# ruolin/strawberry

Hardware: NVIDIA B200
Metric: fragments*EM-iters/sec (higher is better)
Workload: dtype f64

## Files before the change

### include/sbq.h

```cpp
#ifndef SBQ_H_
#define SBQ_H_
#include <stddef.h>
#include <stdint.h>

#ifdef __cplusplus
extern "C" {
#endif

#define SBQ_ABI_VERSION 2

typedef enum {
   SBQ_SUCCESS = 0,
   SBQ_ERR_INVALID = -1,
   SBQ_ERR_NO_DEVICE = -2,
   SBQ_ERR_CUDA = -3,
   SBQ_ERR_NOMEM = -4,
   SBQ_ERR_STATE = -5,
   SBQ_ERR_UNSUPPORTED = -6
} sbq_error;

typedef enum { SBQ_LOCUS_OK = 0, SBQ_LOCUS_ITER_CAP = 1, SBQ_LOCUS_ZERO_DENOM = 2, SBQ_LOCUS_NO_ROWS = 3 } sbq_locus_status;

#define SBQ_MAX_ISO 3600

typedef struct {
   int32_t device;
   int32_t max_iter;
   double  theta_tol;
   double  row_eps;
   double  min_iso_frac;
   int32_t effective_len_norm;
   double  insert_mean;
   int32_t bias_mode;
   int32_t max_out_it;
   int32_t max_theta_it;
   int32_t max_bias_it;
   double  bias_tol;
   int32_t n_gpus;
} sbq_config;

typedef struct {
   int32_t n_iso;
   int32_t n_row;
   const int64_t* row_ptr;
   const int32_t* col;
   const double*  alpha;
   const int32_t* count;
   const int32_t* iso_len;
} sbq_locus;

typedef struct sbq_ctx sbq_ctx;

typedef struct {
   int64_t n_loci, n_row, n_iso, nnz;
   int64_t loci_warp, loci_cta, loci_grid;
   int64_t kernel_launches;
   int64_t h2d_bytes, d2h_bytes;
   double  upload_ms, solve_ms, download_ms;
   double  em_ms;
   double  grid_em_ms;
   int64_t em_iters_total;
   int64_t frag_iters;
   int64_t alg_bytes;
   int64_t grid_alg_bytes;
   double  weights_ms;
} sbq_stats;

int  sbq_abi_version(void);
const char* sbq_error_string(int err);
const char* sbq_last_error(const sbq_ctx*);

void sbq_config_default(sbq_config* cfg);

int  sbq_create(const sbq_config* cfg, sbq_ctx** out);
void sbq_destroy(sbq_ctx*);

int  sbq_submit(sbq_ctx*, const sbq_locus* loci, int64_t n_loci);

int  sbq_submit_flat(sbq_ctx*, int64_t n_loci, const int64_t* loc_row_off, const int64_t* loc_iso_off,
                     const int64_t* row_ptr, const int32_t* col, const double* alpha,
                     const int32_t* count, const int32_t* iso_len);

int  sbq_clear(sbq_ctx*);

int  sbq_validate(sbq_ctx*);

void* sbq_host_alloc(size_t bytes);
void  sbq_host_free(void* p);

int  sbq_upload(sbq_ctx*);
int  sbq_upload_begin(sbq_ctx*);
int  sbq_solve(sbq_ctx*, int64_t total_mapped_reads);
int  sbq_download(sbq_ctx*);

int  sbq_run(sbq_ctx*, int64_t total_mapped_reads);

int  sbq_fpkm_sum(sbq_ctx*, double* local_sum);
int  sbq_fpkm_sum_to_device(sbq_ctx*, void* dev_double);
int  sbq_finalize_tpm(sbq_ctx*, double global_fpkm_sum);

int  sbq_results(sbq_ctx*, double* theta, double* fpkm, double* frac, double* tpm, int32_t* keep,
                 int32_t* iters, int32_t* status);

int  sbq_get_stats(const sbq_ctx*, sbq_stats* out);
// ... 44 lines not shown
```

### strawberry_b200/api.py

```python
import ctypes
import os
import weakref

os.environ.setdefault("CUDA_DEVICE_MAX_CONNECTIONS", "32")

import numpy as np

_HERE = os.path.dirname(os.path.abspath(__file__))
LIB_PATH = os.environ.get("SBQ_LIB_PATH", os.path.join(_HERE, "libsbq.so"))

SBQ_SUCCESS, SBQ_ERR_INVALID, SBQ_ERR_NO_DEVICE, SBQ_ERR_CUDA, SBQ_ERR_NOMEM, SBQ_ERR_STATE, SBQ_ERR_UNSUPPORTED = 0, -1, -2, -3, -4, -5, -6
LOCUS_OK, LOCUS_ITER_CAP, LOCUS_ZERO_DENOM, LOCUS_NO_ROWS = 0, 1, 2, 3

ABI_SYMBOLS = [
    "sbq_abi_version", "sbq_error_string", "sbq_last_error", "sbq_config_default", "sbq_create", "sbq_destroy",
    "sbq_submit", "sbq_submit_flat", "sbq_clear", "sbq_validate", "sbq_host_alloc", "sbq_host_free",
    "sbq_upload", "sbq_upload_begin", "sbq_solve", "sbq_download", "sbq_run", "sbq_fpkm_sum", "sbq_fpkm_sum_to_device",
    "sbq_finalize_tpm", "sbq_results", "sbq_get_stats", "sbq_get_launch_stats", "sbq_em_solve", "sbq_set_plan",
    "sbq_set_covariates", "sbq_bias_results", "sbq_partition_lpt", "sbq_locus_devices", "sbq_synth_giant", "sbq_fetch_batch",
]


class SbqError(RuntimeError):
    def __init__(self, code, msg):
        super().__init__(f"sbq error {code}: {msg}")
        self.code = code


class Config(ctypes.Structure):
    _fields_ = [("device", ctypes.c_int32), ("max_iter", ctypes.c_int32), ("theta_tol", ctypes.c_double),
                ("row_eps", ctypes.c_double), ("min_iso_frac", ctypes.c_double),
                ("effective_len_norm", ctypes.c_int32), ("insert_mean", ctypes.c_double),
                ("bias_mode", ctypes.c_int32), ("max_out_it", ctypes.c_int32), ("max_theta_it", ctypes.c_int32),
                ("max_bias_it", ctypes.c_int32), ("bias_tol", ctypes.c_double), ("n_gpus", ctypes.c_int32)]


class Locus(ctypes.Structure):
    _fields_ = [("n_iso", ctypes.c_int32), ("n_row", ctypes.c_int32), ("row_ptr", ctypes.c_void_p),
                ("col", ctypes.c_void_p), ("alpha", ctypes.c_void_p), ("count", ctypes.c_void_p),
                ("iso_len", ctypes.c_void_p)]


class SynthGiantSpec(ctypes.Structure):
    _fields_ = [("seed", ctypes.c_uint64), ("n_loci", ctypes.c_int32), ("locus_ids", ctypes.c_void_p), ("rows_per_locus", ctypes.c_int64),
                ("iso_lo", ctypes.c_int32), ("iso_hi", ctypes.c_int32), ("mean_extra", ctypes.c_double)]


class Stats(ctypes.Structure):
    _fields_ = [(n, ctypes.c_int64) for n in ("n_loci", "n_row", "n_iso", "nnz", "loci_warp", "loci_cta", "loci_grid",
                                              "kernel_launches", "h2d_bytes", "d2h_bytes")] + \
               [(n, ctypes.c_double) for n in ("upload_ms", "solve_ms", "download_ms", "em_ms", "grid_em_ms")] + \
               [(n, ctypes.c_int64) for n in ("em_iters_total", "frag_iters", "alg_bytes", "grid_alg_bytes")] + \
               [("weights_ms", ctypes.c_double)]

    def as_dict(self):
        return {n: getattr(self, n) for n, _ in self._fields_}


class LaunchStat(ctypes.Structure):
    _fields_ = [("kind", ctypes.c_int32), ("cluster_size", ctypes.c_int32), ("lanes_per_row", ctypes.c_int32),
                ("variant", ctypes.c_int32), ("n_loci", ctypes.c_int64), ("nnz", ctypes.c_int64), ("ms", ctypes.c_double),
                ("alg_bytes", ctypes.c_int64), ("frag_iters", ctypes.c_int64), ("max_iters", ctypes.c_int64), ("start_ms", ctypes.c_double)]


_lib = None


def lib():
    global _lib
    if _lib is None:
        if not os.path.exists(LIB_PATH):
            raise RuntimeError(f"{LIB_PATH} is missing: build the CUDA extension first "
                               "(python -m strawberry_b200.build or __graft_entry__.build()); there is no CPU fallback")
        L = ctypes.CDLL(LIB_PATH)
        L.sbq_error_string.restype = ctypes.c_char_p
        L.sbq_last_error.restype = ctypes.c_char_p
        L.sbq_last_error.argtypes = [ctypes.c_void_p]
        L.sbq_host_alloc.restype = ctypes.c_void_p
        L.sbq_host_alloc.argtypes = [ctypes.c_size_t]
        L.sbq_host_free.argtypes = [ctypes.c_void_p]
        L.sbq_config_default.argtypes = [ctypes.POINTER(Config)]
        L.sbq_create.argtypes = [ctypes.POINTER(Config), ctypes.POINTER(ctypes.c_void_p)]
        L.sbq_destroy.argtypes = [ctypes.c_void_p]
        for name in ("sbq_clear", "sbq_validate", "sbq_upload", "sbq_upload_begin", "sbq_download"):
            getattr(L, name).argtypes = [ctypes.c_void_p]
        L.sbq_submit.argtypes = [ctypes.c_void_p, ctypes.POINTER(Locus), ctypes.c_int64]
        L.sbq_submit_flat.argtypes = [ctypes.c_void_p, ctypes.c_int64] + [ctypes.c_void_p] * 7
        L.sbq_solve.argtypes = [ctypes.c_void_p, ctypes.c_int64]
        L.sbq_run.argtypes = [ctypes.c_void_p, ctypes.c_int64]
        L.sbq_fpkm_sum.argtypes = [ctypes.c_void_p, ctypes.POINTER(ctypes.c_double)]
        L.sbq_fpkm_sum_to_device.argtypes = [ctypes.c_void_p, ctypes.c_void_p]
        L.sbq_finalize_tpm.argtypes = [ctypes.c_void_p, ctypes.c_double]
        L.sbq_results.argtypes = [ctypes.c_void_p] + [ctypes.c_void_p] * 7
        L.sbq_get_stats.argtypes = [ctypes.c_void_p, ctypes.POINTER(Stats)]
        L.sbq_get_launch_stats.argtypes = [ctypes.c_void_p, ctypes.POINTER(LaunchStat), ctypes.c_int]
# ... 98 lines not shown

    def submit(self, loci):
        arr, keep = [], []
        for n_iso, row_ptr, col, alpha, count, iso_len in loci:
            rp, c, a = _c(row_ptr, np.int64), _c(col, np.int32), _c(alpha, np.float64)
            n, il = _c(count, np.int32), _c(iso_len, np.int32)
            keep.append((rp, c, a, n, il))
            arr.append(Locus(int(n_iso), len(n), rp.ctypes.data, c.ctypes.data, a.ctypes.data, n.ctypes.data, il.ctypes.data))
        buf = (Locus * len(arr))(*arr)
        self._chk(self._L.sbq_submit(self._h, buf, len(arr)))

    def set_covariates(self, x):
        x = _c(x, np.float64)
        self._n_cov = x.shape[1] if x.ndim == 2 else 0
        self._chk(self._L.sbq_set_covariates(self._h, _ptr(x) if x.size else None, x.shape[0], self._n_cov))

    def bias_results(self):
        nl = self.stats()["n_loci"]
        beta = np.zeros((nl, max(self._n_cov, 1)))
        outer = np.zeros(nl, np.int32)
        self._chk(self._L.sbq_bias_results(self._h, _ptr(beta), _ptr(outer)))
        return beta[:, :self._n_cov], outer

    def set_insert_model(self, model, read_len):
        from . import builder
        builder._lib()
        self._model = model
        self._chk(self._L.sbq_set_insert_model(self._h, ctypes.byref(model.struct), int(read_len)))

    def submit_deferred(self, tables):
        from . import builder
        builder._lib()
        arr = (ctypes.c_void_p * len(tables))(*[t.handle for t in tables])
        self._keepalive.append(tables)
        self._chk(self._L.sbq_submit_deferred(self._h, arr, len(tables)))

    def fetch_alpha(self):
        out = np.empty(self.stats()["nnz"])
        self._chk(self._L.sbq_fetch_alpha(self._h, _ptr(out)))
        return out

    def validate(self):
        self._chk(self._L.sbq_validate(self._h))

    def upload(self):
        self._chk(self._L.sbq_upload(self._h))

    def upload_begin(self):
        self._chk(self._L.sbq_upload_begin(self._h))

    def solve(self, total_mapped_reads):
        self._chk(self._L.sbq_solve(self._h, int(total_mapped_reads)))

    def download(self):
        self._chk(self._L.sbq_download(self._h))

    def run(self, total_mapped_reads):
        self._chk(self._L.sbq_run(self._h, int(total_mapped_reads)))

    def fpkm_sum(self):
        s = ctypes.c_double(0)
        self._chk(self._L.sbq_fpkm_sum(self._h, ctypes.byref(s)))
        return s.value

    def fpkm_sum_to_device(self, dev_ptr):
        self._chk(self._L.sbq_fpkm_sum_to_device(self._h, ctypes.c_void_p(dev_ptr)))

    def finalize_tpm(self, global_fpkm_sum):
        self._chk(self._L.sbq_finalize_tpm(self._h, float(global_fpkm_sum)))

    def stats(self):
        s = Stats()
        self._chk(self._L.sbq_get_stats(self._h, ctypes.byref(s)))
        return s.as_dict()

    def launch_stats(self):
        cap = 32 * max(1, int(self.cfg.n_gpus))
        buf = (LaunchStat * cap)()
        n = self._chk(self._L.sbq_get_launch_stats(self._h, buf, cap))
        names = {1: "em_warp_kernel", 2: "em_cluster_kernel", 3: "em_grid_kernel"}
        grid = {1: "em_grid_kernel", 2: "em_grid_tma_kernel", 3: "em_grid_dual_kernel"}
        return [dict(kernel=grid.get(buf[i].variant, names[buf[i].kind]) if buf[i].kind == 3 else names[buf[i].kind], cluster_size=buf[i].cluster_size, lanes_per_row=buf[i].lanes_per_row,
                     n_loci=buf[i].n_loci, nnz=buf[i].nnz, ms=buf[i].ms, alg_bytes=buf[i].alg_bytes,
                     frag_iters=buf[i].frag_iters, max_iters=buf[i].max_iters, start_ms=buf[i].start_ms, threads=buf[i].lanes_per_row) for i in range(min(n, cap))]

    def synth_giant(self, locus_ids, rows_per_locus, seed=4, iso_lo=500, iso_hi=800, mean_extra=47.0):
        ids = _c(locus_ids, np.int32)
        spec = SynthGiantSpec(int(seed), len(ids), ids.ctypes.data, int(rows_per_locus), int(iso_lo), int(iso_hi), float(mean_extra))
        self._keepalive = []
        self._chk(self._L.sbq_synth_giant(self._h, ctypes.byref(spec)))

    def fetch_batch(self):
        st = self.stats()
        out = dict(loc_row_off=np.empty(st["n_loci"] + 1, np.int64), loc_iso_off=np.empty(st["n_loci"] + 1, np.int64),
                   row_ptr=np.empty(st["n_row"] + 1, np.int64), col=np.empty(st["nnz"], np.int32), alpha=np.empty(st["nnz"]),
                   count=np.empty(st["n_row"], np.int32), iso_len=np.empty(st["n_iso"], np.int32))
        self._chk(self._L.sbq_fetch_batch(self._h, *[_ptr(out[k]) for k in ("loc_row_off", "loc_iso_off", "row_ptr", "col", "alpha", "count", "iso_len")]))
        out["total_mapped_reads"] = int(out["count"].sum())
        return out

    def locus_devices(self):
        out = np.empty(self.stats()["n_loci"], np.int32)
        self._chk(self._L.sbq_locus_devices(self._h, _ptr(out)))
        return out

    def results(self):
        st = self.stats()
        ni, nl = st["n_iso"], st["n_loci"]
        out = dict(theta=np.empty(ni), fpkm=np.empty(ni), frac=np.empty(ni), tpm=np.empty(ni),
                   keep=np.empty(ni, np.int32), iters=np.empty(nl, np.int32), status=np.empty(nl, np.int32))
        self._chk(self._L.sbq_results(self._h, *[_ptr(out[k]) for k in ("theta", "fpkm", "frac", "tpm", "keep", "iters", "status")]))
        return out

    def em_solve(self, n_iso, row_ptr, col, alpha, count):
        rp, c, a, n = _c(row_ptr, np.int64), _c(col, np.int32), _c(alpha, np.float64), _c(count, np.int32)
        il = np.full(n_iso, 1000, np.int32)
        loc = Locus(int(n_iso), len(n), rp.ctypes.data, c.ctypes.data, a.ctypes.data, n.ctypes.data, il.ctypes.data)
        theta = np.empty(n_iso)
        iters = ctypes.c_int32(0)
        st = self._chk(self._L.sbq_em_solve(self._h, ctypes.byref(loc), _ptr(theta), ctypes.byref(iters)))
        return st, theta, iters.value


class EmSolver:

    def __init__(self, quantifier=None):
        self._q = quantifier or Quantifier()
        self._theta = []
        self._status = None
        self.iters = 0

    def init(self, num_iso, count, model):
        model = np.asarray(model, dtype=np.float64).reshape(len(count), num_iso)
        rows, cols = np.nonzero(model)
        row_ptr = np.zeros(len(count) + 1, np.int64)
        np.cumsum(np.bincount(rows, minlength=len(count)), out=row_ptr[1:])
        st, theta, it = self._q.em_solve(num_iso, row_ptr, cols.astype(np.int32), model[rows, cols], count)
        self._status, self._theta, self.iters = st, list(theta), it
        return st != LOCUS_NO_ROWS

    def run(self):
        if self._status is None or self._status == LOCUS_NO_ROWS:
            return False
        return self._status != LOCUS_ZERO_DENOM
```

### strawberry_b200/csrc/sbq.cu

```cuda
#include <algorithm>
#include <chrono>
#include <cstdarg>
#include <cstdio>
#include <cstdlib>
#include <cstring>
#include <dlfcn.h>
#include <mutex>
#include <string>
#include <thread>
#include <vector>

#include <nccl.h>

#include "../../include/sbq.h"
#include "../../include/sbq_builder.h"
#include "sbq_kernels.cuh"
#include "sbq_grid.cuh"
#include "sbq_grid_tma.cuh"
#include "sbq_grid_dual.cuh"
#include "sbq_bias.cuh"
#include "sbq_weights.cuh"
#include "sbq_synth.cuh"
#include "sbq_rawbuild.cuh"

using namespace sbq;

namespace {

constexpr size_t SMEM_CAP = CL_SMEM_CAP;
constexpr int N_SIDE_STREAMS = 12;
#ifndef SBQ_DEFAULT_WARP_CTAS
#define SBQ_DEFAULT_WARP_CTAS 0
#endif
#ifndef SBQ_DEFAULT_ORDER
#define SBQ_DEFAULT_ORDER 0
#endif

template <typename T>
struct PinnedVec {
   T* p = nullptr;
   size_t n = 0, cap = 0;
   bool reserve(size_t want) {
      if (want <= cap) return true;
      size_t ncap = std::max(want, cap + cap / 2 + 1024);
      T* q = nullptr;
      if (cudaMallocHost((void**)&q, ncap * sizeof(T)) != cudaSuccess) return false;
      if (n) memcpy(q, p, n * sizeof(T));
      if (p) cudaFreeHost(p);
      p = q;
      cap = ncap;
      return true;
   }
   bool append(const T* src, size_t k) {
      if (!reserve(n + k)) return false;
      if (k) memcpy(p + n, src, k * sizeof(T));
      n += k;
      return true;
   }
   void clear() { n = 0; }
   void release() {
      if (p) cudaFreeHost(p);
      p = nullptr;
      n = cap = 0;
   }
};

struct DevBuf {
   void* p = nullptr;
   size_t cap = 0;
   bool reserve(size_t bytes) {
      if (bytes <= cap) return true;
      if (p) cudaFree(p);
      p = nullptr;
      cap = 0;
      size_t want = bytes + bytes / 8 + 4096;
      if (cudaMalloc(&p, want) != cudaSuccess) return false;
      cap = want;
      return true;
   }
   void release() {
      if (p) cudaFree(p);
      p = nullptr;
      cap = 0;
   }
};

struct LaunchClass {
   int cs, lpr;
   std::vector<int32_t> loci;
   int max_iso = 0;
   size_t max_slice = 0;
   size_t list_off = 0;
   size_t smem = 0;
};

struct BiasClass {
   int cs = 1, max_iso = 1;
   size_t off = 0, n = 0;
};

struct LaunchTimer {
   cudaEvent_t e0 = nullptr, e1 = nullptr;
   bool used = false;
};

}

struct MultiState;

struct sbq_ctx {
   sbq_config cfg;
   MultiState* multi = nullptr;
   int device = 0;
   cudaDeviceProp prop;
   cudaStream_t stream = nullptr;
   cudaStream_t copy_st = nullptr;
   cudaEvent_t ev_class_ready[N_SIDE_STREAMS] = {};
   cudaEvent_t ev_grid_ready = nullptr;
   bool class_ready[N_SIDE_STREAMS] = {};
   bool grid_ready = false;
   bool upload_pending = false;
   cudaStream_t side[N_SIDE_STREAMS] = {};
   cudaEvent_t ev[10] = {};
   cudaEvent_t ev_fork = nullptr, ev_join[N_SIDE_STREAMS] = {};
   LaunchTimer lt[N_SIDE_STREAMS + 2];
   std::vector<sbq_launch_stat> launch_stats;
   std::vector<int32_t> locus_launch;
   std::mutex mu;
   std::string err;

   PinnedVec<int64_t> h_loc_row_off, h_loc_iso_off, h_row_ptr;
   PinnedVec<int32_t> h_col, h_count, h_iso_len;
   PinnedVec<double> h_alpha;
   bool borrowed = false;
   const int64_t *b_loc_row_off = nullptr, *b_loc_iso_off = nullptr, *b_row_ptr = nullptr;
   const int32_t *b_col = nullptr, *b_count = nullptr, *b_iso_len = nullptr;
   const double* b_alpha = nullptr;
   int64_t n_loci = 0, n_row = 0, n_iso = 0, nnz = 0;
   bool host_released = false;
   struct LocusMeta { int64_t nnz, frags; int32_t R, T; };
   std::vector<LocusMeta> meta;

   PinnedVec<double> h_cov;
   int n_cov = 0;
   bool have_cov = false;
   DevBuf d_bias;
   int32_t* d_bias_list = nullptr;
   std::vector<int32_t> bias_list;
   BiasClass bias_cls[6];
   int* d_bias_queue = nullptr;
   BiasParams bpar{};
   PinnedVec<double> r_beta;
   PinnedVec<int32_t> r_outer;
   int max_iso_all = 1;

   int deferred = 0;
   PinnedVec<int64_t> h_wseg, h_wpool_off;
   PinnedVec<uint8_t> h_wn;
   PinnedVec<uint32_t> h_wmask, h_wpool;
   PinnedVec<int32_t> h_wlen;
   std::vector<double> model_emp;
   sbq_insert_model model{};
   int model_read_len = 0;
   bool have_model = false;
   DevBuf d_weights;
   double weights_ms = 0.0;

   struct RawStage {
      std::vector<int32_t> hit_locus, hit_ref, iso_seg;
      std::vector<int64_t> hit_feat_ptr{0}, iso_feat_ptr{0}, loc_hit_off{0}, loc_seg_off{0}, iso_seg_ptr{0};
      std::vector<uint32_t> hf_off, hf_len, if_off, if_len, seg_left, seg_right;
      std::vector<uint8_t> hf_code, if_code;
      std::vector<float> hit_mass;
      int long_read = 0;
      void clear() { *this = RawStage(); }
   } raw;
   bool raw_mode = false;
   DevBuf d_raw, d_raw2;
   RawBatch rb{};

   int force_tier = 0, force_cluster = 0;
   std::vector<int32_t> warp_list, grid_list;
   std::vector<LaunchClass> classes;
   int warp_max_iso = 1;
   PinnedVec<int32_t> h_lists;
   size_t warp_list_off = 0, grid_list_off = 0;

   DevBuf d_in, d_out, d_lists, d_grid_scratch, d_col16, d_rowrec, d_csc, d_synth, d_pk;
   bool col16_ready = false, grid_tma_ok = false, grid_dual_ok = false;
   std::vector<int32_t> sgrid_list;
   std::vector<int64_t> sgrid_rec_off;
   size_t sgrid_list_off = 0, sgrid_n_dual = 0;
   int sgrid_max_iso = 1, sgrid_max_iso_dual = 1, sgrid_variant = 0;
   bool sgrid_tma_ok = false;
   DevBuf d_sgrid_scratch, d_srowrec, d_spk;
   cudaStream_t sgrid_st = nullptr;
   cudaEvent_t ev_sgrid_join = nullptr;
   LaunchTimer lt_sgrid;
   std::vector<int64_t> grid_rec_off;
   size_t grid_n_dual = 0;
   int grid_max_iso_dual = 1;
   int grid_max_iso = 1;
   int grid_variant = 0;
   DevParams dp{};
   double* d_tpm = nullptr;
   double* d_fpkm_sum = nullptr;
   int32_t* d_lists_p = nullptr;
   bool resident = false, solved = false, downloaded = false;

   PinnedVec<double> r_theta, r_fpkm, r_frac, r_tpm, r_locus_fpkm;
   PinnedVec<int32_t> r_keep, r_iters, r_status;
   PinnedVec<long long> r_frags;
   DevBuf d_frags;
   double r_fpkm_sum = 0.0;

   sbq_stats stats{};
   bool stats_stale = false;
};

namespace {

int fail(sbq_ctx* c, int code, const char* fmt, ...) {
   if (c) {
      char buf[512];
      va_list ap;
      va_start(ap, fmt);
      vsnprintf(buf, sizeof buf, fmt, ap);
      va_end(ap);
      c->err = buf;
   }
   return code;
}

#define CU(call)                                                                                   \
   do {                                                                                            \
      cudaError_t e_ = (call);                                                                     \
      if (e_ != cudaSuccess)                                                                       \
         return fail(c, SBQ_ERR_CUDA, "%s failed: %s (%s:%d)", #call, cudaGetErrorString(e_), __FILE__, __LINE__); \
   } while (0)

const int64_t* loc_row_off(const sbq_ctx* c) { return c->borrowed ? c->b_loc_row_off : c->h_loc_row_off.p; }
const int64_t* loc_iso_off(const sbq_ctx* c) { return c->borrowed ? c->b_loc_iso_off : c->h_loc_iso_off.p; }
const int64_t* row_ptr(const sbq_ctx* c) { return c->borrowed ? c->b_row_ptr : c->h_row_ptr.p; }
const int32_t* colp(const sbq_ctx* c) { return c->borrowed ? c->b_col : c->h_col.p; }
const int32_t* countp(const sbq_ctx* c) { return c->borrowed ? c->b_count : c->h_count.p; }
const int32_t* iso_lenp(const sbq_ctx* c) { return c->borrowed ? c->b_iso_len : c->h_iso_len.p; }
const double* alphap(const sbq_ctx* c) { return c->borrowed ? c->b_alpha : c->h_alpha.p; }

bool is_pinned(const void* p) {
   cudaPointerAttributes a;
   if (cudaPointerGetAttributes(&a, p) != cudaSuccess) {
      cudaGetLastError();
      return false;
   }
   return a.type == cudaMemoryTypeHost;
}

int materialise(sbq_ctx* c) {
   if (!c->borrowed) return SBQ_SUCCESS;
   if (c->host_released) return fail(c, SBQ_ERR_STATE, "the borrowed batch was released by sbq_upload: sbq_clear and submit again");
   bool ok = true;
   c->h_loc_row_off.clear(); c->h_loc_iso_off.clear(); c->h_row_ptr.clear();
   c->h_col.clear(); c->h_count.clear(); c->h_iso_len.clear(); c->h_alpha.clear();
   ok &= c->h_loc_row_off.append(c->b_loc_row_off, c->n_loci + 1);
   ok &= c->h_loc_iso_off.append(c->b_loc_iso_off, c->n_loci + 1);
   ok &= c->h_row_ptr.append(c->b_row_ptr, c->n_row + 1);
   ok &= c->h_col.append(c->b_col, c->nnz);
   ok &= c->h_alpha.append(c->b_alpha, c->nnz);
   ok &= c->h_count.append(c->b_count, c->n_row);
   ok &= c->h_iso_len.append(c->b_iso_len, c->n_iso);
   c->borrowed = false;
   return ok ? SBQ_SUCCESS : fail(c, SBQ_ERR_NOMEM, "pinned staging allocation failed");
}

void reset_batch(sbq_ctx* c) {
   c->borrowed = false;
   c->host_released = false;
   c->meta.clear();
   c->h_loc_row_off.clear(); c->h_loc_iso_off.clear(); c->h_row_ptr.clear();
   c->h_col.clear(); c->h_count.clear(); c->h_iso_len.clear(); c->h_alpha.clear();
   c->n_loci = c->n_row = c->n_iso = c->nnz = 0;
   c->have_cov = false;
   c->h_cov.clear();
   c->deferred = 0;
   c->raw.clear();
   c->raw_mode = false;
   c->h_wseg.clear(); c->h_wn.clear(); c->h_wmask.clear(); c->h_wpool.clear(); c->h_wlen.clear(); c->h_wpool_off.clear();
   c->resident = c->solved = c->downloaded = false;
}

int ensure_origin(sbq_ctx* c) {
   if (c->h_loc_row_off.n == 0) {
      int64_t z = 0;
      if (!c->h_loc_row_off.append(&z, 1) || !c->h_loc_iso_off.append(&z, 1) || !c->h_row_ptr.append(&z, 1))
         return fail(c, SBQ_ERR_NOMEM, "pinned staging allocation failed");
   }
   return SBQ_SUCCESS;
}

constexpr int N_BUCKETS = 5;
const int BUCKET_NT[N_BUCKETS] = {64, 128, 512, 512, 512};
int smem_bucket(size_t bytes) { return bytes <= 12 * 1024 ? 0 : bytes <= 24 * 1024 ? 1 : bytes <= 56 * 1024 ? 2 : bytes <= 112 * 1024 ? 3 : 4; }

constexpr int64_t SGRID_MAX_NNZ = 1000 * 1000;
constexpr int SGRID_CTAS_DEFAULT = 32;
inline int sgrid_ctas() {
   static const int v = getenv("SBQ_SGRID_CTAS") ? std::max(1, atoi(getenv("SBQ_SGRID_CTAS"))) : SGRID_CTAS_DEFAULT;
   return v;
}
#define SGRID_CTAS sgrid_ctas()

int cluster_size_for(int64_t nnz) {
   static int64_t th[4] = {16 * 1024, 32 * 1024, 64 * 1024, 150 * 1024};
   static bool init = false;
   if (!init) {
      init = true;
      if (const char* e = std::getenv("SBQ_CS_THRESH")) {
         long long a, b, c2, d;
         if (std::sscanf(e, "%lld,%lld,%lld,%lld", &a, &b, &c2, &d) == 4) { th[0] = a * 1024; th[1] = b * 1024; th[2] = c2 * 1024; th[3] = d * 1024; }
      }
   }
   if (nnz <= th[0]) return 1;
   if (nnz <= th[1]) return 2;
   if (nnz <= th[2]) return 4;
   if (nnz <= th[3]) return 8;
   return 16;
}

void capture_meta_host(sbq_ctx* c) {
   const int64_t *lro = loc_row_off(c), *lio = loc_iso_off(c), *rp = row_ptr(c);
   c->meta.resize((size_t)c->n_loci);
   for (int64_t l = 0; l < c->n_loci; ++l)
      c->meta[l] = {rp[lro[l + 1]] - rp[lro[l]], 0, (int32_t)(lro[l + 1] - lro[l]), (int32_t)(lio[l + 1] - lio[l])};
}

int plan(sbq_ctx* c) {
   c->warp_list.clear();
   c->grid_list.clear();
   c->sgrid_list.clear();
   c->sgrid_max_iso = c->sgrid_max_iso_dual = 1;
   c->sgrid_tma_ok = true;
   c->classes.clear();
   c->warp_max_iso = 1;
   c->max_iso_all = 1;
   c->grid_max_iso = 1;
   c->grid_max_iso_dual = 1;
   c->grid_tma_ok = true;
   c->grid_dual_ok = !getenv("SBQ_GRID_NO_DUAL");
   const bool force_dual = getenv("SBQ_GRID_DUAL") != nullptr;
   static const bool sgrid_enabled = !getenv("SBQ_NO_SGRID");
   std::vector<char> dual_locus(c->n_loci, 0);
   std::vector<int64_t> nnz_of(c->n_loci);
   LaunchClass* slot[5][N_BUCKETS] = {};
   std::vector<LaunchClass> tmp;
   tmp.reserve(20);
   static const int64_t grid_min_nnz = getenv("SBQ_GRID_MIN_NNZ") ? atoll(getenv("SBQ_GRID_MIN_NNZ")) : 300 * 1000;
   for (int64_t l = 0; l < c->n_loci; ++l) {
      const int64_t R = c->meta[l].R, T = c->meta[l].T, nnz = c->meta[l].nnz;
      nnz_of[l] = nnz;
      c->max_iso_all = std::max(c->max_iso_all, (int)T);
      if (T > SBQ_MAX_ISO) return fail(c, SBQ_ERR_UNSUPPORTED, "locus %lld has %lld isoforms (> SBQ_MAX_ISO)", (long long)l, (long long)T);
      int tier;
      if (c->force_tier) tier = c->force_tier;
      else if (T <= WT_MAX_ISO && R <= WT_MAX_ROWS && nnz <= WT_MAX_NNZ) tier = 1;
      else if (nnz >= grid_min_nnz) tier = 3;
      else tier = 2;
      if (tier == 1 && T > WT_MAX_ISO) tier = 2;
      if (tier == 3 && !grid_tier_supports((int)T)) tier = 2;
      if (tier == 2 && cluster_stream_groups((int)T, SMEM_CAP, CL_NT, 1, 0) <= 0) {
         if (!grid_tier_supports((int)T)) return fail(c, SBQ_ERR_UNSUPPORTED, "locus %lld: %lld isoforms fit no tier", (long long)l, (long long)T);
         tier = 3;
      }
      if (tier == 1) {
         c->warp_list.push_back((int32_t)l);
         c->warp_max_iso = std::max(c->warp_max_iso, (int)T);
      } else if (tier == 3) {
         const bool small = !c->force_tier && sgrid_enabled && nnz < SGRID_MAX_NNZ;
         (small ? c->sgrid_list : c->grid_list).push_back((int32_t)l);
         const bool dual = c->grid_dual_ok && (grid_dual_supports_iso((int)T) || (force_dual && grid_dual_possible((int)T))) &&
                           nnz < (1LL << 32) && nnz <= 56 * R;
         dual_locus[l] = dual;
         int& mx_dual = small ? c->sgrid_max_iso_dual : c->grid_max_iso_dual;
         int& mx_rest = small ? c->sgrid_max_iso : c->grid_max_iso;
         bool& tma_ok = small ? c->sgrid_tma_ok : c->grid_tma_ok;
         if (dual) {
            mx_dual = std::max(mx_dual, (int)T);
         } else {
            mx_rest = std::max(mx_rest, (int)T);
            if (!grid_tma_supports((int)T, (long long)R, small ? SGRID_CTAS : c->prop.multiProcessorCount)) tma_ok = false;
         }
      } else {
         int cs = c->force_cluster ? c->force_cluster : cluster_size_for(nnz);
         int csi = cs == 1 ? 0 : cs == 2 ? 1 : cs == 4 ? 2 : cs == 8 ? 3 : 4;
         const size_t slice = cluster_slice_estimate(nnz, R, (int)T, cs);
         const int bucket = cs == 1 ? smem_bucket(cluster_fixed_doubles((int)T, 1, slice) * sizeof(double) + slice + 256) : N_BUCKETS - 1;
         if (!slot[csi][bucket]) {
            tmp.push_back(LaunchClass{cs, BUCKET_NT[bucket], {}, 0, 0, 0, 0});
            slot[csi][bucket] = &tmp.back();
         }
         LaunchClass* lc = slot[csi][bucket];
         lc->loci.push_back((int32_t)l);
         lc->max_iso = std::max(lc->max_iso, (int)T);
         lc->max_slice = std::max(lc->max_slice, slice);
         lc->smem = std::max(lc->smem, cluster_class_smem((int)T, slice, lc->lpr, cs));
      }
   }
   auto by_size = [&](int32_t a, int32_t b) { return nnz_of[a] != nnz_of[b] ? nnz_of[a] > nnz_of[b] : a < b; };
   {
      bool small_keys = true;
      for (int32_t l : c->warp_list) small_keys &= nnz_of[l] <= WT_MAX_NNZ;
      if (small_keys) {
         std::vector<int32_t> first(WT_MAX_NNZ + 2, 0), sorted(c->warp_list.size());
         for (int32_t l : c->warp_list) ++first[WT_MAX_NNZ - (int)nnz_of[l] + 1];
         for (int k = 1; k <= WT_MAX_NNZ + 1; ++k) first[k] += first[k - 1];
         for (int32_t l : c->warp_list) sorted[first[WT_MAX_NNZ - (int)nnz_of[l]]++] = l;
         c->warp_list.swap(sorted);
      } else {
         std::sort(c->warp_list.begin(), c->warp_list.end(), by_size);
      }
   }
   auto order_grid = [&](std::vector<int32_t>& list, size_t& n_dual, std::vector<int64_t>& rec_off) {
      std::sort(list.begin(), list.end(), [&](int32_t a, int32_t b) {
         if (dual_locus[a] != dual_locus[b]) return dual_locus[a] > dual_locus[b];
         if (dual_locus[a]) {
            const int na = grid_dual_nc(c->meta[a].T), nb_ = grid_dual_nc(c->meta[b].T);
            if (na != nb_) return na > nb_;
         }
         return by_size(a, b);
      });
      n_dual = 0;
      for (int32_t l : list) n_dual += dual_locus[l];
      rec_off.assign(n_dual + 1, 0);
      for (size_t i = 0; i < n_dual; ++i) rec_off[i + 1] = rec_off[i] + c->meta[list[i]].R + 1;
   };
   order_grid(c->grid_list, c->grid_n_dual, c->grid_rec_off);
   order_grid(c->sgrid_list, c->sgrid_n_dual, c->sgrid_rec_off);
   for (auto& lc : tmp) {
      std::sort(lc.loci.begin(), lc.loci.end(), by_size);
      if (cluster_stream_groups(lc.max_iso, SMEM_CAP, lc.lpr, 1, 0) <= 0)
         return fail(c, SBQ_ERR_UNSUPPORTED, "locus with %d isoforms does not fit the cluster tier", lc.max_iso);
      c->classes.push_back(std::move(lc));
   }
   std::sort(c->classes.begin(), c->classes.end(), [](const LaunchClass& a, const LaunchClass& b) { return a.cs != b.cs ? a.cs > b.cs : a.max_slice > b.max_slice; });

   c->h_lists.clear();
   c->warp_list_off = 0;
   if (!c->h_lists.append(c->warp_list.data(), c->warp_list.size())) return fail(c, SBQ_ERR_NOMEM, "list staging");
   c->grid_list_off = c->h_lists.n;
   if (!c->h_lists.append(c->grid_list.data(), c->grid_list.size())) return fail(c, SBQ_ERR_NOMEM, "list staging");
   c->sgrid_list_off = c->h_lists.n;
   if (!c->h_lists.append(c->sgrid_list.data(), c->sgrid_list.size())) return fail(c, SBQ_ERR_NOMEM, "list staging");
   for (auto& lc : c->classes) {
      lc.list_off = c->h_lists.n;
      if (!c->h_lists.append(lc.loci.data(), lc.loci.size())) return fail(c, SBQ_ERR_NOMEM, "list staging");
   }
   c->stats.loci_warp = (int64_t)c->warp_list.size();
   c->stats.loci_grid = (int64_t)(c->grid_list.size() + c->sgrid_list.size());
   c->stats.loci_cta = c->n_loci - c->stats.loci_warp - c->stats.loci_grid;
   return SBQ_SUCCESS;
}

size_t align_up(size_t x, size_t a = 256) { return (x + a - 1) / a * a; }

int alloc_device(sbq_ctx* c) {
   const size_t sz_lro = align_up((c->n_loci + 1) * sizeof(int64_t)), sz_rp = align_up((c->n_row + 1) * sizeof(int64_t) + 64);
   const size_t sz_col = align_up(c->nnz * sizeof(int32_t) + 64), sz_al = align_up(c->nnz * sizeof(double) + 64);
   const size_t sz_cnt = align_up(c->n_row * sizeof(int32_t) + 64), sz_il = align_up(c->n_iso * sizeof(int32_t));
   const size_t in_bytes = 2 * sz_lro + sz_rp + sz_col + sz_al + 2 * sz_cnt + sz_il;
   const size_t sz_iso_d = align_up(c->n_iso * sizeof(double)), sz_iso_i = align_up(c->n_iso * sizeof(int32_t));
   const size_t sz_loc_i = align_up(c->n_loci * sizeof(int32_t)), sz_loc_d = align_up(c->n_loci * sizeof(double));
   const size_t out_bytes = 4 * sz_iso_d + sz_iso_i + 2 * sz_loc_i + sz_loc_d + 256;
   if (!c->d_in.reserve(in_bytes) || !c->d_out.reserve(out_bytes) || !c->d_lists.reserve(align_up((size_t)c->n_loci * sizeof(int32_t)) + 256))
      return fail(c, SBQ_ERR_NOMEM, "device allocation failed (%zu MB)", (in_bytes + out_bytes) >> 20);

   char* p = (char*)c->d_in.p;
   DevParams& dp = c->dp;
   auto carve = [&](size_t bytes) { char* q = p; p += bytes; return q; };
   int64_t* d_lro = (int64_t*)carve(sz_lro);
   int64_t* d_lio = (int64_t*)carve(sz_lro);
   int64_t* d_rp = (int64_t*)carve(sz_rp);
   int32_t* d_col = (int32_t*)carve(sz_col);
   double* d_al = (double*)carve(sz_al);
   int32_t* d_cnt = (int32_t*)carve(sz_cnt);
   dp.neff = (int32_t*)carve(sz_cnt);
   int32_t* d_il = (int32_t*)carve(sz_il);
   dp.csc = nullptr;
   dp.loc_row_off = d_lro; dp.loc_iso_off = d_lio; dp.row_ptr = d_rp; dp.col = d_col; dp.alpha = d_al;
   dp.count = d_cnt; dp.iso_len = d_il;
   p = (char*)c->d_out.p;
   dp.theta = (double*)carve(sz_iso_d);
   dp.fpkm = (double*)carve(sz_iso_d);
   dp.frac = (double*)carve(sz_iso_d);
   c->d_tpm = (double*)carve(sz_iso_d);
   dp.keep = (int32_t*)carve(sz_iso_i);
   dp.iters = (int32_t*)carve(sz_loc_i);
   dp.status = (int32_t*)carve(sz_loc_i);
   dp.locus_fpkm = (double*)carve(sz_loc_d);
   c->d_fpkm_sum = (double*)carve(256);
   c->d_lists_p = (int32_t*)c->d_lists.p;
   return SBQ_SUCCESS;
}

template <typename K>
int set_kernel_attrs(sbq_ctx* c, K kernel, size_t smem, bool nonportable) {
   CU(cudaFuncSetAttribute(kernel, cudaFuncAttributeMaxDynamicSharedMemorySize, (int)smem));
   if (nonportable) CU(cudaFuncSetAttribute(kernel, cudaFuncAttributeNonPortableClusterSizeAllowed, 1));
   return SBQ_SUCCESS;
}

template <int NT, int NCACHE, int MINB>
int launch_cluster_class_nt(sbq_ctx* c, const LaunchClass& lc, cudaStream_t st) {
   auto kernel = em_cluster_kernel<NT, NCACHE, MINB>;
   int rc = set_kernel_attrs(c, kernel, lc.smem, lc.cs > 8);
   if (rc) return rc;
   cudaLaunchConfig_t cfg{};
   cfg.gridDim = dim3((unsigned)(lc.loci.size() * lc.cs));
   cfg.blockDim = dim3(NT);
   cfg.dynamicSmemBytes = lc.smem;
   cfg.stream = st;
   cudaLaunchAttribute attr[1];
   attr[0].id = cudaLaunchAttributeClusterDimension;
   attr[0].val.clusterDim.x = (unsigned)lc.cs;
   attr[0].val.clusterDim.y = 1;
   attr[0].val.clusterDim.z = 1;
   cfg.attrs = attr;
   cfg.numAttrs = 1;
   const int32_t* list = c->d_lists_p + lc.list_off;
   CU(cudaLaunchKernelEx(&cfg, kernel, c->dp, list, (int)lc.loci.size(), (unsigned)lc.smem));
   return SBQ_SUCCESS;
}

struct StagingMark {
   size_t lro, lio, rp, col, al, cnt, il, wseg, wn, wmask, wlen, wpool, wpoff;
   int64_t n_loci, n_row, n_iso, nnz;
   explicit StagingMark(const sbq_ctx* c)
       : lro(c->h_loc_row_off.n), lio(c->h_loc_iso_off.n), rp(c->h_row_ptr.n), col(c->h_col.n), al(c->h_alpha.n), cnt(c->h_count.n), il(c->h_iso_len.n),
         wseg(c->h_wseg.n), wn(c->h_wn.n), wmask(c->h_wmask.n), wlen(c->h_wlen.n), wpool(c->h_wpool.n), wpoff(c->h_wpool_off.n),
         n_loci(c->n_loci), n_row(c->n_row), n_iso(c->n_iso), nnz(c->nnz) {}
   void restore(sbq_ctx* c) const {
      c->h_loc_row_off.n = lro; c->h_loc_iso_off.n = lio; c->h_row_ptr.n = rp; c->h_col.n = col; c->h_alpha.n = al; c->h_count.n = cnt; c->h_iso_len.n = il;
      c->h_wseg.n = wseg; c->h_wn.n = wn; c->h_wmask.n = wmask; c->h_wlen.n = wlen; c->h_wpool.n = wpool; c->h_wpool_off.n = wpoff;
      c->n_loci = n_loci; c->n_row = n_row; c->n_iso = n_iso; c->nnz = nnz;
   }
};

int submit_locked(sbq_ctx* c, const sbq_locus* loci, int64_t n_loci) {
   if (c->host_released) return fail(c, SBQ_ERR_STATE, "the borrowed batch was released by sbq_upload: sbq_clear and submit again");
   for (int64_t l = 0; l < n_loci; ++l) {
      const sbq_locus& L = loci[l];
      if (L.n_iso < 1 || L.n_row < 0 || !L.row_ptr || !L.iso_len || (L.n_row > 0 && !L.count))
         return fail(c, SBQ_ERR_INVALID, "locus %lld: bad shape or null pointer", (long long)l);
      if (L.n_iso > SBQ_MAX_ISO) return fail(c, SBQ_ERR_UNSUPPORTED, "locus %lld: %d isoforms > SBQ_MAX_ISO", (long long)l, L.n_iso);
      for (int32_t i = 1; i <= L.n_row; ++i)
         if (L.row_ptr[i] < L.row_ptr[i - 1]) return fail(c, SBQ_ERR_INVALID, "locus %lld: row_ptr not monotone", (long long)l);
      if (L.row_ptr[L.n_row] > L.row_ptr[0] && (!L.col || !L.alpha)) return fail(c, SBQ_ERR_INVALID, "locus %lld: null col / alpha", (long long)l);
   }
   cudaSetDevice(c->device);
   int rc = materialise(c);
   if (rc) return rc;
   if ((rc = ensure_origin(c))) return rc;
   const StagingMark mark(c);
   for (int64_t l = 0; l < n_loci; ++l) {
      const sbq_locus& L = loci[l];
      const int64_t k0 = L.row_ptr[0], k1 = L.row_ptr[L.n_row];
      const int64_t base = c->nnz - k0;
      bool ok = c->h_row_ptr.reserve(c->h_row_ptr.n + L.n_row);
      if (ok) {
         for (int32_t i = 1; i <= L.n_row; ++i) c->h_row_ptr.p[c->h_row_ptr.n++] = L.row_ptr[i] + base;
         ok = c->h_col.append(L.col + k0, k1 - k0) && c->h_alpha.append(L.alpha + k0, k1 - k0) &&
              c->h_count.append(L.count, L.n_row) && c->h_iso_len.append(L.iso_len, L.n_iso);
      }
      c->nnz += k1 - k0;
      c->n_row += L.n_row;
      c->n_iso += L.n_iso;
      c->n_loci += 1;
      ok = ok && c->h_loc_row_off.append(&c->n_row, 1) && c->h_loc_iso_off.append(&c->n_iso, 1);
      if (!ok) {
         mark.restore(c);
         return fail(c, SBQ_ERR_NOMEM, "pinned staging");
      }
   }
   c->resident = c->solved = c->downloaded = false;
   return SBQ_SUCCESS;
}

}

#include "sbq_multi.cuh"

extern "C" {

int sbq_abi_version(void) { return SBQ_ABI_VERSION; }

const char* sbq_error_string(int err) {
   switch (err) {
      case SBQ_SUCCESS: return "success";
      case SBQ_ERR_INVALID: return "invalid argument";
      case SBQ_ERR_NO_DEVICE: return "no CUDA device (libsbq has no CPU path)";
      case SBQ_ERR_CUDA: return "CUDA runtime error";
      case SBQ_ERR_NOMEM: return "out of memory";
      case SBQ_ERR_STATE: return "invalid call sequence";
      case SBQ_ERR_UNSUPPORTED: return "shape outside supported limits";
      default: return "unknown error";
   }
}

const char* sbq_last_error(const sbq_ctx* c) { return c ? c->err.c_str() : ""; }

void sbq_config_default(sbq_config* cfg) {
   if (!cfg) return;
   memset(cfg, 0, sizeof *cfg);
   cfg->device = -1;
   cfg->max_iter = 1000;
   cfg->theta_tol = 1e-2;
   cfg->row_eps = 1e-5;
   cfg->min_iso_frac = 0.0;
   cfg->effective_len_norm = 0;
   cfg->insert_mean = 0.0;
   cfg->bias_mode = 0;
   cfg->max_out_it = 100;
   cfg->max_theta_it = 5000;
   cfg->max_bias_it = 10;
   cfg->bias_tol = 1e-2;
   cfg->n_gpus = 1;
}

int sbq_create(const sbq_config* cfg, sbq_ctx** out) {
   if (!cfg || !out) return SBQ_ERR_INVALID;
   *out = nullptr;
   if (cfg->max_iter < 1 || !(cfg->theta_tol >= 0) || cfg->bias_mode < 0 || cfg->bias_mode > 1) return SBQ_ERR_INVALID;
   if (cfg->bias_mode == 1 && (cfg->max_out_it < 1 || cfg->max_theta_it < 1 || cfg->max_bias_it < 1 || !(cfg->bias_tol >= 0))) return SBQ_ERR_INVALID;
   if (cfg->n_gpus < 0 || cfg->n_gpus > 64) return SBQ_ERR_INVALID;
   setenv("CUDA_DEVICE_MAX_CONNECTIONS", "32", 0);
   int ndev = 0;
   if (cudaGetDeviceCount(&ndev) != cudaSuccess || ndev == 0) {
      cudaGetLastError();
      return SBQ_ERR_NO_DEVICE;
   }
   int dev = cfg->device;
   if (dev < 0) {
      if (cfg->n_gpus > 1) dev = 0;
      else if (cudaGetDevice(&dev) != cudaSuccess) return SBQ_ERR_NO_DEVICE;
   }
   if (dev >= ndev) return SBQ_ERR_INVALID;
   if (cfg->n_gpus > 1 && dev + cfg->n_gpus > ndev) return SBQ_ERR_NO_DEVICE;
   sbq_ctx* c = new sbq_ctx();
   c->cfg = *cfg;
   c->device = dev;
   auto bail = [&](int code) { sbq_destroy(c); return code; };
   if (cudaSetDevice(dev) != cudaSuccess) return bail(SBQ_ERR_CUDA);
   if (cudaGetDeviceProperties(&c->prop, dev) != cudaSuccess) return bail(SBQ_ERR_CUDA);
   if (c->prop.major < 10) return bail(SBQ_ERR_NO_DEVICE);
   if (cudaStreamCreateWithFlags(&c->stream, cudaStreamNonBlocking) != cudaSuccess) return bail(SBQ_ERR_CUDA);
   if (cudaStreamCreateWithFlags(&c->copy_st, cudaStreamNonBlocking) != cudaSuccess) return bail(SBQ_ERR_CUDA);
   if (cudaEventCreateWithFlags(&c->ev_grid_ready, cudaEventDisableTiming) != cudaSuccess) return bail(SBQ_ERR_CUDA);
   for (auto& e : c->ev_class_ready)
      if (cudaEventCreateWithFlags(&e, cudaEventDisableTiming) != cudaSuccess) return bail(SBQ_ERR_CUDA);
   for (auto& s : c->side)
      if (cudaStreamCreateWithFlags(&s, cudaStreamNonBlocking) != cudaSuccess) return bail(SBQ_ERR_CUDA);
   for (auto& e : c->ev)
      if (cudaEventCreate(&e) != cudaSuccess) return bail(SBQ_ERR_CUDA);
   if (cudaEventCreateWithFlags(&c->ev_fork, cudaEventDisableTiming) != cudaSuccess) return bail(SBQ_ERR_CUDA);
   for (auto& e : c->ev_join)
      if (cudaEventCreateWithFlags(&e, cudaEventDisableTiming) != cudaSuccess) return bail(SBQ_ERR_CUDA);
   for (auto& t : c->lt)
      if (cudaEventCreate(&t.e0) != cudaSuccess || cudaEventCreate(&t.e1) != cudaSuccess) return bail(SBQ_ERR_CUDA);
   if (cudaStreamCreateWithFlags(&c->sgrid_st, cudaStreamNonBlocking) != cudaSuccess) return bail(SBQ_ERR_CUDA);
   if (cudaEventCreateWithFlags(&c->ev_sgrid_join, cudaEventDisableTiming) != cudaSuccess) return bail(SBQ_ERR_CUDA);
   if (cudaEventCreate(&c->lt_sgrid.e0) != cudaSuccess || cudaEventCreate(&c->lt_sgrid.e1) != cudaSuccess) return bail(SBQ_ERR_CUDA);
   if (cfg->n_gpus > 1) {
      const int rc = multi_create(c, ndev);
      if (rc) {
         fprintf(stderr, "libsbq: %s\n", c->err.c_str());
         return bail(rc);
      }
   }
   *out = c;
   return SBQ_SUCCESS;
}

void sbq_destroy(sbq_ctx* c) {
   if (!c) return;
   multi_destroy(c);
   cudaSetDevice(c->device);
   if (c->copy_st) cudaStreamSynchronize(c->copy_st);
   if (c->stream) cudaStreamSynchronize(c->stream);
   c->h_loc_row_off.release(); c->h_loc_iso_off.release(); c->h_row_ptr.release();
   c->h_col.release(); c->h_count.release(); c->h_iso_len.release(); c->h_alpha.release();
   c->h_lists.release();
   c->r_theta.release(); c->r_fpkm.release(); c->r_frac.release(); c->r_tpm.release();
   c->r_locus_fpkm.release(); c->r_keep.release(); c->r_iters.release(); c->r_status.release(); c->r_frags.release(); c->d_frags.release();
   c->d_in.release(); c->d_out.release(); c->d_lists.release(); c->d_grid_scratch.release(); c->d_col16.release(); c->d_rowrec.release(); c->d_csc.release(); c->d_synth.release(); c->d_pk.release(); c->d_raw.release(); c->d_raw2.release(); c->d_bias.release();
   c->d_sgrid_scratch.release(); c->d_srowrec.release(); c->d_spk.release();
   c->h_cov.release(); c->r_beta.release(); c->r_outer.release();
   c->h_wseg.release(); c->h_wn.release(); c->h_wmask.release(); c->h_wpool.release(); c->h_wlen.release(); c->h_wpool_off.release(); c->d_weights.release();
   for (auto& e : c->ev) if (e) cudaEventDestroy(e);
   if (c->ev_fork) cudaEventDestroy(c->ev_fork);
   for (auto& e : c->ev_join) if (e) cudaEventDestroy(e);
   for (auto& t : c->lt) { if (t.e0) cudaEventDestroy(t.e0); if (t.e1) cudaEventDestroy(t.e1); }
   for (auto& s : c->side) if (s) cudaStreamDestroy(s);
   if (c->lt_sgrid.e0) cudaEventDestroy(c->lt_sgrid.e0);
   if (c->lt_sgrid.e1) cudaEventDestroy(c->lt_sgrid.e1);
   if (c->ev_sgrid_join) cudaEventDestroy(c->ev_sgrid_join);
   if (c->sgrid_st) cudaStreamSynchronize(c->sgrid_st), cudaStreamDestroy(c->sgrid_st);
   if (c->ev_grid_ready) cudaEventDestroy(c->ev_grid_ready);
   for (auto& e : c->ev_class_ready) if (e) cudaEventDestroy(e);
   if (c->copy_st) cudaStreamDestroy(c->copy_st);
   if (c->stream) cudaStreamDestroy(c->stream);
   delete c;
}

int sbq_set_plan(sbq_ctx* c, int force_tier, int force_cluster) {
   if (!c) return SBQ_ERR_INVALID;
   if (force_tier < 0 || force_tier > 3) return fail(c, SBQ_ERR_INVALID, "force_tier must be 0..3");
   if (force_cluster != 0 && force_cluster != 1 && force_cluster != 2 && force_cluster != 4 && force_cluster != 8 && force_cluster != 16)
      return fail(c, SBQ_ERR_INVALID, "force_cluster must be 0, 1, 2, 4, 8 or 16");
   if (c->force_tier != force_tier || c->force_cluster != force_cluster) c->resident = c->solved = c->downloaded = false;
   c->force_tier = force_tier;
   c->force_cluster = force_cluster;
   return SBQ_SUCCESS;
}

int sbq_clear(sbq_ctx* c) {
   if (!c) return SBQ_ERR_INVALID;
   std::lock_guard<std::mutex> lk(c->mu);
   if (c->upload_pending) {
      cudaSetDevice(c->device);
      cudaStreamSynchronize(c->copy_st);
      c->upload_pending = false;
   }
   if (c->multi && c->raw_mode)
      for (sbq_ctx* ch : c->multi->child) sbq_clear(ch);
   reset_batch(c);
   return SBQ_SUCCESS;
}

int sbq_submit(sbq_ctx* c, const sbq_locus* loci, int64_t n_loci) {
   if (!c || (!loci && n_loci > 0) || n_loci < 0) return SBQ_ERR_INVALID;
   std::lock_guard<std::mutex> lk(c->mu);
   if (c->deferred == 1) return fail(c, SBQ_ERR_STATE, "a batch is either all deferred-weight or all host-weighted");
   const int rc = submit_locked(c, loci, n_loci);
   if (rc == SBQ_SUCCESS && n_loci > 0) c->deferred = 2;
   return rc;
}

int sbq_submit_flat(sbq_ctx* c, int64_t n_loci, const int64_t* lro, const int64_t* lio, const int64_t* rp,
                    const int32_t* col, const double* alpha, const int32_t* count, const int32_t* iso_len) {
   if (!c || n_loci < 0) return SBQ_ERR_INVALID;
   if (n_loci == 0) return SBQ_SUCCESS;
   if (!lro || !lio || !rp || !iso_len) return fail(c, SBQ_ERR_INVALID, "null offset array");
   std::lock_guard<std::mutex> lk(c->mu);
   cudaSetDevice(c->device);
   if (c->deferred == 1) return fail(c, SBQ_ERR_STATE, "a batch is either all deferred-weight or all host-weighted");
   const int64_t rows = lro[n_loci] - lro[0], isos = lio[n_loci] - lio[0];
   if (rows < 0 || isos < n_loci) return fail(c, SBQ_ERR_INVALID, "bad locus offsets");
   const int64_t k0 = rp[lro[0]], k1 = rp[lro[n_loci]];
   if (k1 < k0 || (k1 > k0 && (!col || !alpha)) || (rows > 0 && !count)) return fail(c, SBQ_ERR_INVALID, "bad CSR arrays");
   for (int64_t l = 0; l < n_loci; ++l) {
      const int64_t T = lio[l + 1] - lio[l];
      if (lro[l + 1] < lro[l] || T < 1) return fail(c, SBQ_ERR_INVALID, "locus %lld: bad shape", (long long)l);
      if (T > SBQ_MAX_ISO) return fail(c, SBQ_ERR_UNSUPPORTED, "locus %lld: %lld isoforms > SBQ_MAX_ISO", (long long)l, (long long)T);
   }
   if (c->n_loci == 0 && lro[0] == 0 && lio[0] == 0 && k0 == 0 && is_pinned(lro) && is_pinned(lio) && is_pinned(rp) &&
       is_pinned(iso_len) && (rows == 0 || is_pinned(count)) && (k1 == 0 || (is_pinned(col) && is_pinned(alpha)))) {
      c->borrowed = true;
      c->b_loc_row_off = lro; c->b_loc_iso_off = lio; c->b_row_ptr = rp;
      c->b_col = col; c->b_alpha = alpha; c->b_count = count; c->b_iso_len = iso_len;
      c->n_loci = n_loci; c->n_row = rows; c->n_iso = isos; c->nnz = k1;
      c->deferred = 2;
      c->resident = c->solved = c->downloaded = false;
      return SBQ_SUCCESS;
   }
   if (c->host_released) return fail(c, SBQ_ERR_STATE, "the borrowed batch was released by sbq_upload: sbq_clear and submit again");
   for (int64_t i = lro[0]; i < lro[n_loci]; ++i)
      if (rp[i + 1] < rp[i]) return fail(c, SBQ_ERR_INVALID, "row %lld: row_ptr not monotone", (long long)i);
   int rc = materialise(c);
   if (rc) return rc;
   if ((rc = ensure_origin(c))) return rc;
   const bool ok = c->h_loc_row_off.reserve(c->h_loc_row_off.n + n_loci) && c->h_loc_iso_off.reserve(c->h_loc_iso_off.n + n_loci) &&
                   c->h_row_ptr.reserve(c->h_row_ptr.n + rows) && c->h_col.reserve(c->h_col.n + (k1 - k0)) && c->h_alpha.reserve(c->h_alpha.n + (k1 - k0)) &&
                   c->h_count.reserve(c->h_count.n + rows) && c->h_iso_len.reserve(c->h_iso_len.n + isos);
   if (!ok) return fail(c, SBQ_ERR_NOMEM, "pinned staging");
   for (int64_t l = 1; l <= n_loci; ++l) {
      c->h_loc_row_off.p[c->h_loc_row_off.n++] = c->n_row + (lro[l] - lro[0]);
      c->h_loc_iso_off.p[c->h_loc_iso_off.n++] = c->n_iso + (lio[l] - lio[0]);
   }
   const int64_t base = c->nnz - k0;
   for (int64_t i = 1; i <= rows; ++i) c->h_row_ptr.p[c->h_row_ptr.n++] = rp[lro[0] + i] + base;
   c->h_col.append(col + k0, k1 - k0);
   c->h_alpha.append(alpha + k0, k1 - k0);
   c->h_count.append(count + lro[0], rows);
   c->h_iso_len.append(iso_len + lio[0], isos);
   c->n_loci += n_loci; c->n_row += rows; c->n_iso += isos; c->nnz += k1 - k0;
   c->deferred = 2;
   c->resident = c->solved = c->downloaded = false;
   return SBQ_SUCCESS;
}

int sbq_validate(sbq_ctx* c) {
   if (!c) return SBQ_ERR_INVALID;
   std::lock_guard<std::mutex> lk(c->mu);
   if (c->host_released) return fail(c, SBQ_ERR_STATE, "the borrowed batch was released by sbq_upload");
   const int64_t *lro = loc_row_off(c), *lio = loc_iso_off(c), *rp = row_ptr(c);
   const int32_t* col = colp(c);
   for (int64_t l = 0; l < c->n_loci; ++l) {
      const int64_t T = lio[l + 1] - lio[l];
      for (int64_t i = lro[l]; i < lro[l + 1]; ++i) {
         if (rp[i + 1] < rp[i]) return fail(c, SBQ_ERR_INVALID, "locus %lld row %lld: row_ptr not monotone", (long long)l, (long long)(i - lro[l]));
         for (int64_t k = rp[i]; k < rp[i + 1]; ++k) {
            if (col[k] < 0 || col[k] >= T) return fail(c, SBQ_ERR_INVALID, "locus %lld: column %d out of range", (long long)l, col[k]);
            if (k > rp[i] && col[k] <= col[k - 1]) return fail(c, SBQ_ERR_INVALID, "locus %lld row %lld: columns not strictly ascending", (long long)l, (long long)(i - lro[l]));
         }
      }
   }
   return SBQ_SUCCESS;
}

}

static int raw_upload(sbq_ctx* c);

static int upload_begin(sbq_ctx* c) {
   CU(cudaSetDevice(c->device));
   if (c->upload_pending) {
      CU(cudaStreamSynchronize(c->copy_st));
      c->upload_pending = false;
   }
   if (c->n_loci == 0) return fail(c, SBQ_ERR_STATE, "nothing submitted");
   if (c->host_released) return fail(c, SBQ_ERR_STATE, "the borrowed batch was released by the previous sbq_upload: sbq_clear and submit again");
   {
      const int rc = alloc_device(c);
      if (rc) return rc;
   }
   DevParams& dp = c->dp;
   int64_t *d_lro = const_cast<int64_t*>(dp.loc_row_off), *d_lio = const_cast<int64_t*>(dp.loc_iso_off), *d_rp = const_cast<int64_t*>(dp.row_ptr);
   int32_t *d_col = const_cast<int32_t*>(dp.col), *d_cnt = const_cast<int32_t*>(dp.count), *d_il = const_cast<int32_t*>(dp.iso_len);
   double* d_al = const_cast<double*>(dp.alpha);

   cudaStream_t st = c->copy_st;
   c->upload_pending = true;
   c->resident = c->solved = c->downloaded = false;
   CU(cudaEventRecord(c->ev[0], st));
   CU(cudaMemcpyAsync(d_lro, loc_row_off(c), (c->n_loci + 1) * sizeof(int64_t), cudaMemcpyHostToDevice, st));
   CU(cudaMemcpyAsync(d_lio, loc_iso_off(c), (c->n_loci + 1) * sizeof(int64_t), cudaMemcpyHostToDevice, st));
   CU(cudaMemcpyAsync(d_rp, row_ptr(c), (c->n_row + 1) * sizeof(int64_t), cudaMemcpyHostToDevice, st));
   if (c->n_row) CU(cudaMemcpyAsync(d_cnt, countp(c), c->n_row * sizeof(int32_t), cudaMemcpyHostToDevice, st));
   CU(cudaMemcpyAsync(d_il, iso_lenp(c), c->n_iso * sizeof(int32_t), cudaMemcpyHostToDevice, st));
   if (!c->r_frags.reserve((size_t)c->n_loci) || !c->d_frags.reserve(align_up((size_t)c->n_loci * 8))) return fail(c, SBQ_ERR_NOMEM, "fragment-total buffers");
   locus_frags_kernel<<<std::max(1, std::min<int>((int)((c->n_loci + 7) / 8), c->prop.multiProcessorCount * 8)), 256, 0, st>>>(d_lro, d_cnt, c->n_loci, (long long*)c->d_frags.p);
   CU(cudaGetLastError());
   CU(cudaMemcpyAsync(c->r_frags.p, c->d_frags.p, (size_t)c->n_loci * 8, cudaMemcpyDeviceToHost, st));
   if (c->nnz) CU(cudaMemcpyAsync(d_col, colp(c), c->nnz * sizeof(int32_t), cudaMemcpyHostToDevice, st));
   const bool timing = getenv("SBQ_TIMING") != nullptr;
   const auto t_plan0 = std::chrono::steady_clock::now();
   {
      capture_meta_host(c);
      const int rc = plan(c);
      if (rc) {
         cudaStreamSynchronize(st);
         c->upload_pending = false;
         return rc;
      }
   }
   if (timing) fprintf(stderr, "SBQ_TIMING plan_ms %.3f\n", std::chrono::duration<double, std::milli>(std::chrono::steady_clock::now() - t_plan0).count());
   if (c->h_lists.n) CU(cudaMemcpyAsync(c->d_lists_p, c->h_lists.p, c->h_lists.n * sizeof(int32_t), cudaMemcpyHostToDevice, st));
   const int64_t* lro = loc_row_off(c);
   const int64_t* rp = row_ptr(c);
   const double* al = alphap(c);
   std::vector<std::pair<int64_t, int64_t>> done;
   auto copy_loci = [&](const std::vector<int32_t>& loci) -> int {
      for (int32_t l : loci) {
         const int64_t k0 = rp[lro[l]], k1 = rp[lro[l + 1]];
         if (k1 > k0) {
            CU(cudaMemcpyAsync(d_al + k0, al + k0, (size_t)(k1 - k0) * sizeof(double), cudaMemcpyHostToDevice, st));
            done.emplace_back(k0, k1);
         }
      }
      return SBQ_SUCCESS;
   };
   for (auto& r : c->class_ready) r = false;
   c->grid_ready = false;
   if (!(c->grid_list.empty() && c->sgrid_list.empty()) && c->grid_list.size() + c->sgrid_list.size() <= 16) {
      int rc = copy_loci(c->grid_list);
      if (rc) return rc;
      rc = copy_loci(c->sgrid_list);
      if (rc) return rc;
      CU(cudaEventRecord(c->ev_grid_ready, st));
      c->grid_ready = true;
   }
   size_t n_prio = 0;
   for (size_t i = 0; i < c->classes.size() && i < (size_t)N_SIDE_STREAMS; ++i) {
      if (c->classes[i].cs < 8 || n_prio + c->classes[i].loci.size() > 48) continue;
      n_prio += c->classes[i].loci.size();
      const int rc = copy_loci(c->classes[i].loci);
      if (rc) return rc;
      CU(cudaEventRecord(c->ev_class_ready[i], st));
      c->class_ready[i] = true;
   }
   std::sort(done.begin(), done.end());
   int64_t pos = 0;
   for (size_t i = 0; i <= done.size(); ++i) {
      const int64_t end = i < done.size() ? done[i].first : c->nnz;
      if (end > pos) CU(cudaMemcpyAsync(d_al + pos, al + pos, (size_t)(end - pos) * sizeof(double), cudaMemcpyHostToDevice, st));
      if (i < done.size()) pos = std::max(pos, done[i].second);
   }
   CU(cudaEventRecord(c->ev[1], st));
   if (!c->classes.empty()) {
      if (!c->d_csc.reserve(align_up(c->nnz * 4 + 16))) return fail(c, SBQ_ERR_NOMEM, "device allocation failed (transposed-index scratch)");
      dp.csc = (unsigned*)c->d_csc.p;
   }
   c->stats.h2d_bytes = 2 * (c->n_loci + 1) * 8 + (c->n_row + 1) * 8 + c->nnz * 12 + c->n_row * 4 + c->n_iso * 4 + (int64_t)c->h_lists.n * 4;
   c->stats.n_loci = c->n_loci; c->stats.n_row = c->n_row; c->stats.n_iso = c->n_iso; c->stats.nnz = c->nnz;
   c->stats.weights_ms = 0.0;
   c->col16_ready = false;
   c->resident = true;
   return SBQ_SUCCESS;
}

static int upload_wait(sbq_ctx* c) {
   if (!c->upload_pending) return SBQ_SUCCESS;
   CU(cudaSetDevice(c->device));
   CU(cudaStreamSynchronize(c->copy_st));
   c->upload_pending = false;
   if (c->borrowed) c->host_released = true;
   for (size_t l = 0; l < c->meta.size(); ++l) c->meta[l].frags = c->r_frags.p[l];
   float ms = 0;
   CU(cudaEventElapsedTime(&ms, c->ev[0], c->ev[1]));
   c->stats.upload_ms = ms;
   return SBQ_SUCCESS;
}

extern "C" {

int sbq_upload_begin(sbq_ctx* c) {
   if (!c) return SBQ_ERR_INVALID;
   if (c->multi || c->deferred == 1 || c->raw_mode || c->cfg.bias_mode == 1) return sbq_upload(c);
   std::lock_guard<std::mutex> lk(c->mu);
   return upload_begin(c);
}

int sbq_upload(sbq_ctx* c) {
   if (!c) return SBQ_ERR_INVALID;
   if (c->multi) return multi_upload(c);
   std::lock_guard<std::mutex> lk(c->mu);
   if (c->raw_mode) {
      if (c->n_loci == 0) return fail(c, SBQ_ERR_STATE, "nothing submitted");
      return raw_upload(c);
   }
   {
      int rc = upload_begin(c);
      if (!rc) rc = upload_wait(c);
      if (rc) return rc;
   }
   if (c->deferred == 1) {
      if (!c->have_model) return fail(c, SBQ_ERR_STATE, "deferred weights need sbq_set_insert_model()");
      if ((int64_t)c->h_wseg.n != c->nnz) return fail(c, SBQ_ERR_STATE, "deferred-weight descriptors do not cover the batch");
      const size_t b_seg = align_up(c->nnz * 8 + 8), b_n = align_up(c->nnz + 8), b_m = align_up(c->nnz * 4 + 8), b_l = align_up(c->nnz * 4 + 8);
      const size_t b_pool = align_up(c->h_wpool.n * 4 + 8), b_emp = align_up(c->model_emp.size() * 8 + 8);
      if (!c->d_weights.reserve(b_seg + b_n + b_m + b_l + b_pool + b_emp)) return fail(c, SBQ_ERR_NOMEM, "device allocation failed (weight descriptors)");
      char* q = (char*)c->d_weights.p;
      int64_t* d_seg = (int64_t*)q; q += b_seg;
      uint8_t* d_n = (uint8_t*)q; q += b_n;
      uint32_t* d_m = (uint32_t*)q; q += b_m;
      int32_t* d_l = (int32_t*)q; q += b_l;
      uint32_t* d_pool = (uint32_t*)q; q += b_pool;
      double* d_emp = (double*)q;
      cudaStream_t st = c->stream;
      CU(cudaEventRecord(c->ev[5], st));
      CU(cudaMemcpyAsync(d_seg, c->h_wseg.p, c->nnz * 8, cudaMemcpyHostToDevice, st));
      CU(cudaMemcpyAsync(d_n, c->h_wn.p, c->nnz, cudaMemcpyHostToDevice, st));
      CU(cudaMemcpyAsync(d_m, c->h_wmask.p, c->nnz * 4, cudaMemcpyHostToDevice, st));
      CU(cudaMemcpyAsync(d_l, c->h_wlen.p, c->nnz * 4, cudaMemcpyHostToDevice, st));
      if (c->h_wpool.n) CU(cudaMemcpyAsync(d_pool, c->h_wpool.p, c->h_wpool.n * 4, cudaMemcpyHostToDevice, st));
      if (!c->model_emp.empty()) CU(cudaMemcpyAsync(d_emp, c->model_emp.data(), c->model_emp.size() * 8, cudaMemcpyHostToDevice, st));
      WeightModel wm{c->model.use_emp, c->model.start_offset, c->model.end_offset, c->model.total_reads, d_emp, c->model.mean, c->model.sd, c->model_read_len};
      const int blocks = std::max(1, std::min<int>((int)((c->nnz + 7) / 8), c->prop.multiProcessorCount * 16));
      weights_kernel<<<blocks, 256, 0, st>>>(c->nnz, d_seg, d_n, d_m, d_l, d_pool, wm, const_cast<double*>(c->dp.alpha));
      CU(cudaGetLastError());
      CU(cudaEventRecord(c->ev[6], st));
      CU(cudaStreamSynchronize(st));
      float wms = 0;
      CU(cudaEventElapsedTime(&wms, c->ev[5], c->ev[6]));
      c->weights_ms = wms;
      c->stats.weights_ms = wms;
      c->stats.h2d_bytes += (int64_t)(c->nnz * 17 + c->h_wpool.n * 4 + c->model_emp.size() * 8);
   }
   if (c->cfg.bias_mode == 1) {
      if (!c->have_cov) return fail(c, SBQ_ERR_STATE, "bias_mode = 1 needs sbq_set_covariates() after the last submit");
      const size_t K = (size_t)c->n_cov;
      const size_t bx = align_up(c->n_row * K * 8 + 8), bw = align_up(c->n_row * 8 + 8), bb = align_up(c->n_loci * K * 8 + 8), bo = align_up(c->n_loci * 4 + 8);
      if (!c->d_bias.reserve(bx + 2 * bw + bb + 2 * bo + 64)) return fail(c, SBQ_ERR_NOMEM, "device allocation failed (bias scratch)");
      char* q = (char*)c->d_bias.p;
      c->bpar.x = (const double*)q; q += bx;
// ... 44 lines not shown
   dp.max_iter = c->cfg.max_iter;
   dp.tol = c->cfg.theta_tol;
   dp.row_eps = c->cfg.row_eps;
   dp.min_frac = c->cfg.min_iso_frac;
   dp.eff_len_norm = c->cfg.effective_len_norm;
   dp.insert_mean = c->cfg.insert_mean;
   dp.rpm = 1e6 / (double)(int)total_mapped_reads;

   cudaStream_t st = c->stream;
   int64_t launches = 0;
   if (c->cfg.bias_mode == 1) {
      const size_t smem = bias_smem_bytes(c->max_iso_all);
      if (smem > SMEM_CAP) return fail(c, SBQ_ERR_UNSUPPORTED, "bias mode supports up to %d isoforms per locus", (int)((SMEM_CAP / 8 - 8) / (5 + BI_W)));
      c->bpar.max_out_it = c->cfg.max_out_it;
      c->bpar.max_theta_it = c->cfg.max_theta_it;
      c->bpar.max_bias_it = c->cfg.max_bias_it;
      c->bpar.bias_tol = c->cfg.bias_tol;
      int rc_attr = set_kernel_attrs(c, em_bias_kernel, smem, c->bias_cls[0].n > 0);
      if (rc_attr) return rc_attr;
      CU(cudaEventRecord(c->ev[2], st));
      CU(cudaEventRecord(c->ev_fork, st));
      int n_side = 0;
      if (c->bias_cls[5].n) {
         const BiasClass& bc = c->bias_cls[5];
         cudaStream_t ss = c->side[n_side];
         CU(cudaStreamWaitEvent(ss, c->ev_fork, 0));
         ++n_side;
         const size_t wsmem = bias_warp_smem_bytes();
         CU(cudaFuncSetAttribute(em_bias_warp_kernel, cudaFuncAttributeMaxDynamicSharedMemorySize, (int)wsmem));
         int occ = 1;
         CU(cudaOccupancyMaxActiveBlocksPerMultiprocessor(&occ, em_bias_warp_kernel, BW_WARPS * 32, wsmem));
         const long long want = ((long long)bc.n + BW_WARPS - 1) / BW_WARPS;
         const unsigned grid = (unsigned)std::max(1LL, std::min(want, (long long)c->prop.multiProcessorCount * std::max(1, occ)));
         CU(cudaMemsetAsync(c->d_bias_queue, 0, sizeof(int), ss));
         em_bias_warp_kernel<<<grid, BW_WARPS * 32, wsmem, ss>>>(c->dp, c->bpar, (const int32_t*)(c->d_bias_list + bc.off), (int)bc.n, c->d_bias_queue);
         CU(cudaGetLastError());
         ++launches;
      }
      for (int k = 0; k < 5; ++k) {
         const BiasClass& bc = c->bias_cls[k];
         if (!bc.n) continue;
         cudaStream_t ss = c->side[n_side % N_SIDE_STREAMS];
         if (n_side < N_SIDE_STREAMS) CU(cudaStreamWaitEvent(ss, c->ev_fork, 0));
         ++n_side;
         cudaLaunchConfig_t cfg{};
         cfg.gridDim = dim3((unsigned)(bc.n * bc.cs));
         cfg.blockDim = dim3(BI_NT);
         cfg.dynamicSmemBytes = bias_smem_bytes(bc.max_iso);
         cfg.stream = ss;
         cudaLaunchAttribute attr[1];
         attr[0].id = cudaLaunchAttributeClusterDimension;
         attr[0].val.clusterDim.x = (unsigned)bc.cs;
         attr[0].val.clusterDim.y = 1;
         attr[0].val.clusterDim.z = 1;
         cfg.attrs = attr;
         cfg.numAttrs = 1;
         CU(cudaLaunchKernelEx(&cfg, em_bias_kernel, c->dp, c->bpar, (const int32_t*)(c->d_bias_list + bc.off), (int)bc.n));
         ++launches;
      }
      for (int i = 0; i < std::min(n_side, N_SIDE_STREAMS); ++i) {
         CU(cudaEventRecord(c->ev_join[i], c->side[i]));
         CU(cudaStreamWaitEvent(st, c->ev_join[i], 0));
      }
      CU(cudaEventRecord(c->ev[3], st));
      fpkm_sum_kernel<<<1, 1024, 0, st>>>(dp.locus_fpkm, c->n_loci, c->d_fpkm_sum);
      CU(cudaGetLastError());
      CU(cudaEventRecord(c->ev[4], st));
      CU(cudaStreamSynchronize(st));
      float ms_ = 0;
      CU(cudaEventElapsedTime(&ms_, c->ev[2], c->ev[4]));
      c->stats.solve_ms = ms_;
      CU(cudaEventElapsedTime(&ms_, c->ev[2], c->ev[3]));
      c->stats.em_ms = ms_;
      c->stats.grid_em_ms = 0;
      c->stats.kernel_launches = launches + 1;
      c->launch_stats.clear();
      c->locus_launch.assign(c->n_loci, -1);
      c->solved = true;
      c->downloaded = false;
      return SBQ_SUCCESS;
   }
   CU(cudaEventRecord(c->ev[2], st));
   CU(cudaEventRecord(c->ev_fork, st));
   int used_side = 0;
   c->stats.grid_em_ms = 0;
   for (auto& t : c->lt) t.used = false;
   const bool pending = c->upload_pending;
   auto launch_grid_part = [&](const std::vector<int32_t>& list, size_t list_off, size_t n_dual_, const std::vector<int64_t>& rec_off, int max_iso_rest,
                               bool tma_ok, const cudaDeviceProp& prop_, DevBuf& scratch, DevBuf& rowrec, DevBuf& pkbuf, cudaStream_t gs_, int& variant,
                               int& n_launch) -> int {
      int rc = 0;
      variant = 0;
      const int32_t* d_grid = c->d_lists_p + list_off;
      const int n_dual = (int)n_dual_, n_rest = (int)list.size() - n_dual;
      if (n_dual) {
         GridDualBufs bf{&scratch.p, &scratch.cap, &c->d_col16.p, &c->d_col16.cap, &rowrec.p, &rowrec.cap, &pkbuf.p, &pkbuf.cap};
         int nl = 0;
         std::vector<int> h_iso((size_t)n_dual);
         for (int i = 0; i < n_dual; ++i) h_iso[i] = c->meta[list[i]].T;
         rc = grid_dual_launch(c->dp, c->nnz, d_grid, n_dual, h_iso.data(), rec_off.data(), prop_, bf, c->col16_ready, gs_, &nl);
         n_launch += nl;
         variant = 3;
      }
      if (rc == 0 && n_rest) {
         int nl = 0;
         if (tma_ok && !getenv("SBQ_GRID_NO_TMA")) {
            if (!variant) variant = 2;
            rc = grid_tma_launch(c->dp, c->nnz, d_grid + n_dual, n_rest, max_iso_rest, prop_, &scratch.p, &scratch.cap,
                                 &c->d_col16.p, &c->d_col16.cap, c->col16_ready, gs_, &nl);
         } else {
            if (!variant) variant = 1;
            rc = grid_tier_launch(c->dp, d_grid + n_dual, n_rest, prop_, &scratch.p, &scratch.cap, gs_, &nl);
         }
         n_launch += nl;
      }
      return rc;
   };
   auto grid_failed = [&](int rc) -> int {
      c->resident = false;
      c->col16_ready = false;
      return fail(c, rc < -6 ? SBQ_ERR_CUDA : rc, "grid tier launch failed: %s", cudaGetErrorString(cudaGetLastError()));
   };
   if (!(c->grid_list.empty() && c->sgrid_list.empty())) {
      const size_t need16 = (size_t)c->nnz * 2 + 256;
      if (need16 > c->d_col16.cap) {
         if (!c->d_col16.reserve(need16)) return fail(c, SBQ_ERR_NOMEM, "device allocation failed (16-bit slots)");
         c->col16_ready = false;
      }
   }
   if (!c->grid_list.empty()) {
      if (pending) CU(cudaStreamWaitEvent(st, c->grid_ready ? c->ev_grid_ready : c->ev[1], 0));
      CU(cudaEventRecord(c->ev[6], st));
      int n_launch = 0;
      const int rc = launch_grid_part(c->grid_list, c->grid_list_off, c->grid_n_dual, c->grid_rec_off, c->grid_max_iso, c->grid_tma_ok, c->prop,
                                      c->d_grid_scratch, c->d_rowrec, c->d_pk, st, c->grid_variant, n_launch);
      if (rc != 0) return grid_failed(rc);
      launches += n_launch;
      CU(cudaEventRecord(c->ev[7], st));
   }
   c->lt_sgrid.used = false;
   if (!c->sgrid_list.empty()) {
      cudaDeviceProp prop_sg = c->prop;
      prop_sg.multiProcessorCount = std::min(SGRID_CTAS, c->prop.multiProcessorCount);
      cudaStream_t gs_ = c->sgrid_st;
      CU(cudaStreamWaitEvent(gs_, c->ev_fork, 0));
      if (pending) CU(cudaStreamWaitEvent(gs_, c->grid_ready ? c->ev_grid_ready : c->ev[1], 0));
      if (!c->grid_list.empty()) {
         CU(cudaStreamWaitEvent(gs_, c->ev[7], 0));
      }
      CU(cudaEventRecord(c->lt_sgrid.e0, gs_));
      int n_launch = 0;
      const int rc = launch_grid_part(c->sgrid_list, c->sgrid_list_off, c->sgrid_n_dual, c->sgrid_rec_off, c->sgrid_max_iso, c->sgrid_tma_ok, prop_sg,
                                      c->d_sgrid_scratch, c->d_srowrec, c->d_spk, gs_, c->sgrid_variant, n_launch);
      if (rc != 0) return grid_failed(rc);
      launches += n_launch;
      CU(cudaEventRecord(c->lt_sgrid.e1, gs_));
      CU(cudaEventRecord(c->ev_sgrid_join, gs_));
      c->lt_sgrid.used = true;
   }
   if (!(c->grid_list.empty() && c->sgrid_list.empty())) c->col16_ready = true;
   const bool serialize = getenv("SBQ_SERIALIZE") != nullptr;
   static const int order_mode = getenv("SBQ_ORDER") ? atoi(getenv("SBQ_ORDER")) : SBQ_DEFAULT_ORDER;
   const int ncls = (int)c->classes.size();
   std::vector<int> ord;
   int warp_pos = ncls;
   {
      std::vector<int> big, small, rest;
      for (int i = 0; i < ncls; ++i) {
         const LaunchClass& lc = c->classes[i];
         if (lc.lpr < CL_NT) small.push_back(i);
         else if (lc.cs >= (order_mode == 3 ? 16 : 8)) big.push_back(i);
         else rest.push_back(i);
      }
      if (order_mode == 1) { ord = small; ord.insert(ord.end(), big.begin(), big.end()); ord.insert(ord.end(), rest.begin(), rest.end()); warp_pos = 0; }
      else if (order_mode == 2 || order_mode == 3) { ord = big; warp_pos = (int)ord.size(); ord.insert(ord.end(), small.begin(), small.end()); ord.insert(ord.end(), rest.begin(), rest.end()); }
      else { for (int i = 0; i < ncls; ++i) ord.push_back(i); }
   }
   auto launch_warp = [&]() -> int {
      if (c->warp_list.empty()) return SBQ_SUCCESS;
      const size_t smem = warp_tier_smem_bytes(c->warp_max_iso);
      CU(cudaFuncSetAttribute(em_warp_kernel, cudaFuncAttributeMaxDynamicSharedMemorySize, (int)smem));
      const int n = (int)c->warp_list.size();
      int per_sm = 1;
      CU(cudaOccupancyMaxActiveBlocksPerMultiprocessor(&per_sm, em_warp_kernel, WT_WARPS * 32, smem));
      int grid = std::max(1, std::min((n + WT_WARPS - 1) / WT_WARPS, per_sm * c->prop.multiProcessorCount));
      static const int warp_cta_cap = getenv("SBQ_WARP_CTAS") ? atoi(getenv("SBQ_WARP_CTAS")) : SBQ_DEFAULT_WARP_CTAS;
      if (warp_cta_cap > 0) grid = std::min(grid, warp_cta_cap);
      int* queue = (int*)((char*)c->d_fpkm_sum + 64);
      if (pending) CU(cudaStreamWaitEvent(st, c->ev[1], 0));
      CU(cudaMemsetAsync(queue, 0, sizeof(int), st));
      CU(cudaEventRecord(c->lt[0].e0, st));
      em_warp_kernel<<<grid, WT_WARPS * 32, smem, st>>>(c->dp, c->d_lists_p + c->warp_list_off, n, c->warp_max_iso, queue);
      CU(cudaGetLastError());
      CU(cudaEventRecord(c->lt[0].e1, st));
      c->lt[0].used = true;
      ++launches;
      return SBQ_SUCCESS;
   };
   for (int pos = 0; pos <= ncls; ++pos) {
      if (pos == warp_pos) {
         const int rcw = launch_warp();
         if (rcw) return rcw;
      }
      if (pos == ncls) break;
      const int i = ord[pos];
      const LaunchClass& lc = c->classes[i];
      cudaStream_t ss = serialize ? st : c->side[i % N_SIDE_STREAMS];
      if (!serialize && i < N_SIDE_STREAMS) CU(cudaStreamWaitEvent(ss, c->ev_fork, 0));
      if (pending) CU(cudaStreamWaitEvent(ss, (i < N_SIDE_STREAMS && c->class_ready[i]) ? c->ev_class_ready[i] : c->ev[1], 0));
      LaunchTimer& t = c->lt[2 + i % N_SIDE_STREAMS];
      CU(cudaEventRecord(t.e0, ss));
      int rc = lc.lpr == 64 ? launch_cluster_class_nt<64, 0, 8>(c, lc, ss) : lc.lpr == 128 ? launch_cluster_class_nt<128, 0, 4>(c, lc, ss) :
               lc.lpr == 256 ? launch_cluster_class_nt<256, 0, 2>(c, lc, ss) : launch_cluster_class_nt<CL_NT, 0, 1>(c, lc, ss);
      if (rc) return rc;
      CU(cudaEventRecord(t.e1, ss));
      t.used = true;
      ++launches;
   }
   used_side = ncls;
   for (int i = 0; i < std::min(used_side, N_SIDE_STREAMS) && !serialize; ++i) {
      CU(cudaEventRecord(c->ev_join[i], c->side[i]));
      CU(cudaStreamWaitEvent(st, c->ev_join[i], 0));
   }
   if (c->lt_sgrid.used) CU(cudaStreamWaitEvent(st, c->ev_sgrid_join, 0));
   CU(cudaEventRecord(c->ev[3], st));
   fpkm_sum_kernel<<<1, 1024, 0, st>>>(dp.locus_fpkm, c->n_loci, c->d_fpkm_sum);
   CU(cudaGetLastError());
   ++launches;
   CU(cudaEventRecord(c->ev[4], st));
   CU(cudaStreamSynchronize(st));
   if (pending) {
      const int rcw = upload_wait(c);
      if (rcw) return rcw;
   }
   float ms = 0;
   CU(cudaEventElapsedTime(&ms, c->ev[2], c->ev[4]));
   c->stats.solve_ms = ms;
   CU(cudaEventElapsedTime(&ms, c->ev[2], c->ev[3]));
   c->stats.em_ms = ms;
   if (!c->grid_list.empty()) {
      CU(cudaEventElapsedTime(&ms, c->ev[6], c->ev[7]));
      c->stats.grid_em_ms = ms;
   }
   c->launch_stats.clear();
   c->locus_launch.assign(c->n_loci, -1);
   auto add_stat = [&](int kind, int cs, int lpr, const std::vector<int32_t>& loci, double ms_, cudaEvent_t e0 = nullptr) {
      sbq_launch_stat ls{};
      ls.kind = kind; ls.cluster_size = cs; ls.lanes_per_row = lpr; ls.n_loci = (int64_t)loci.size(); ls.ms = ms_;
      float st_ms = 0;
      if (e0 && cudaEventElapsedTime(&st_ms, c->ev[2], e0) == cudaSuccess) ls.start_ms = st_ms;
      for (int32_t l : loci) c->locus_launch[l] = (int32_t)c->launch_stats.size();
      c->launch_stats.push_back(ls);
   };
   if (c->lt[0].used) { CU(cudaEventElapsedTime(&ms, c->lt[0].e0, c->lt[0].e1)); add_stat(1, 1, 1, c->warp_list, ms, c->lt[0].e0); }
   if (!c->grid_list.empty()) { add_stat(3, 0, 32, c->grid_list, c->stats.grid_em_ms, c->ev[6]); c->launch_stats.back().variant = c->grid_variant; }
   if (c->lt_sgrid.used) {
      CU(cudaEventElapsedTime(&ms, c->lt_sgrid.e0, c->lt_sgrid.e1));
      add_stat(3, std::min(SGRID_CTAS, c->prop.multiProcessorCount), 32, c->sgrid_list, ms, c->lt_sgrid.e0);
      c->launch_stats.back().variant = c->sgrid_variant;
   }
   for (size_t i = 0; i < c->classes.size(); ++i) {
      LaunchTimer& t = c->lt[2 + i % N_SIDE_STREAMS];
      CU(cudaEventElapsedTime(&ms, t.e0, t.e1));
      add_stat(2, c->classes[i].cs, c->classes[i].lpr, c->classes[i].loci, ms, t.e0);
   }
   c->stats.kernel_launches = launches;
   c->solved = true;
   c->downloaded = false;
   return SBQ_SUCCESS;
}

int sbq_fpkm_sum(sbq_ctx* c, double* local_sum) {
   if (!c || !local_sum) return SBQ_ERR_INVALID;
   if (c->multi) {
      std::lock_guard<std::mutex> lk(c->mu);
      if (!c->solved) return fail(c, SBQ_ERR_STATE, "sbq_fpkm_sum before sbq_solve");
      const int rc = multi_allreduce_locked(c);
      if (!rc) *local_sum = c->multi->global_sum;
      return rc;
   }
   std::lock_guard<std::mutex> lk(c->mu);
   CU(cudaSetDevice(c->device));
   if (!c->solved) return fail(c, SBQ_ERR_STATE, "sbq_fpkm_sum before sbq_solve");
   CU(cudaMemcpyAsync(local_sum, c->d_fpkm_sum, sizeof(double), cudaMemcpyDeviceToHost, c->stream));
   CU(cudaStreamSynchronize(c->stream));
   return SBQ_SUCCESS;
}

int sbq_fpkm_sum_to_device(sbq_ctx* c, void* dev_double) {
   if (!c || !dev_double) return SBQ_ERR_INVALID;
   if (c->multi) {
      std::lock_guard<std::mutex> lk(c->mu);
      if (!c->solved) return fail(c, SBQ_ERR_STATE, "sbq_fpkm_sum_to_device before sbq_solve");
      const int rc = multi_allreduce_locked(c);
      if (rc) return rc;
      CU(cudaMemcpy(dev_double, c->multi->d_sum[0] + 1, sizeof(double), cudaMemcpyDefault));
      return SBQ_SUCCESS;
   }
   std::lock_guard<std::mutex> lk(c->mu);
   CU(cudaSetDevice(c->device));
   if (!c->solved) return fail(c, SBQ_ERR_STATE, "sbq_fpkm_sum_to_device before sbq_solve");
   CU(cudaMemcpyAsync(dev_double, c->d_fpkm_sum, sizeof(double), cudaMemcpyDeviceToDevice, c->stream));
   CU(cudaStreamSynchronize(c->stream));
   return SBQ_SUCCESS;
}

int sbq_finalize_tpm(sbq_ctx* c, double global_fpkm_sum) {
   if (!c) return SBQ_ERR_INVALID;
   if (c->multi) return multi_finalize_tpm(c, global_fpkm_sum);
   std::lock_guard<std::mutex> lk(c->mu);
   CU(cudaSetDevice(c->device));
   if (!c->solved) return fail(c, SBQ_ERR_STATE, "sbq_finalize_tpm before sbq_solve");
   const int64_t n = c->n_iso;
   tpm_kernel<<<(unsigned)((n + 255) / 256), 256, 0, c->stream>>>(c->dp.fpkm, c->d_tpm, n, global_fpkm_sum);
   CU(cudaGetLastError());
   c->stats.kernel_launches += 1;
   c->downloaded = false;
   return SBQ_SUCCESS;
}

int sbq_download(sbq_ctx* c) {
   if (!c) return SBQ_ERR_INVALID;
   if (c->multi) return multi_download(c);
   std::lock_guard<std::mutex> lk(c->mu);
   CU(cudaSetDevice(c->device));
   if (!c->solved) return fail(c, SBQ_ERR_STATE, "sbq_download before sbq_solve");
   const size_t ni = c->n_iso, nl = c->n_loci;
   bool ok = c->r_theta.reserve(ni) && c->r_fpkm.reserve(ni) && c->r_frac.reserve(ni) && c->r_tpm.reserve(ni) &&
             c->r_keep.reserve(ni) && c->r_iters.reserve(nl) && c->r_status.reserve(nl) && c->r_locus_fpkm.reserve(nl);
   if (!ok) return fail(c, SBQ_ERR_NOMEM, "pinned result buffers");
   cudaStream_t st = c->stream;
   CU(cudaEventRecord(c->ev[8], st));
   CU(cudaMemcpyAsync(c->r_theta.p, c->dp.theta, ni * 8, cudaMemcpyDeviceToHost, st));
   CU(cudaMemcpyAsync(c->r_fpkm.p, c->dp.fpkm, ni * 8, cudaMemcpyDeviceToHost, st));
   CU(cudaMemcpyAsync(c->r_frac.p, c->dp.frac, ni * 8, cudaMemcpyDeviceToHost, st));
   CU(cudaMemcpyAsync(c->r_tpm.p, c->d_tpm, ni * 8, cudaMemcpyDeviceToHost, st));
   CU(cudaMemcpyAsync(c->r_keep.p, c->dp.keep, ni * 4, cudaMemcpyDeviceToHost, st));
   CU(cudaMemcpyAsync(c->r_iters.p, c->dp.iters, nl * 4, cudaMemcpyDeviceToHost, st));
   CU(cudaMemcpyAsync(c->r_status.p, c->dp.status, nl * 4, cudaMemcpyDeviceToHost, st));
   CU(cudaMemcpyAsync(&c->r_fpkm_sum, c->d_fpkm_sum, 8, cudaMemcpyDeviceToHost, st));
   CU(cudaEventRecord(c->ev[9], st));
   CU(cudaStreamSynchronize(st));
   float ms = 0;
   CU(cudaEventElapsedTime(&ms, c->ev[8], c->ev[9]));
   c->stats.download_ms = ms;
   c->stats.d2h_bytes = (int64_t)ni * 36 + (int64_t)nl * 8 + 8;

   c->stats_stale = true;
   c->downloaded = true;
   return SBQ_SUCCESS;
}

int sbq_run(sbq_ctx* c, int64_t total_mapped_reads) {
   int rc = sbq_upload_begin(c);
   if (rc) return rc;
   if ((rc = sbq_solve(c, total_mapped_reads))) return rc;
   if (c->multi) {
      if ((rc = multi_tpm(c))) return rc;
      return sbq_download(c);
   }
   double s = 0.0;
   if ((rc = sbq_fpkm_sum(c, &s))) return rc;
   if ((rc = sbq_finalize_tpm(c, s))) return rc;
   return sbq_download(c);
}

}

static void account(sbq_ctx* c) {
   if (!c->stats_stale || !c->downloaded) return;
   const size_t nl = (size_t)c->n_loci;
   std::vector<char> is_grid(nl, 0);
   for (int32_t l : c->grid_list) is_grid[l] = 1;
   int64_t it_total = 0, frag_iters = 0, alg = 0, galg = 0;
   for (auto& ls : c->launch_stats) ls.nnz = ls.alg_bytes = ls.frag_iters = ls.max_iters = 0;
   for (size_t l = 0; l < nl && l < c->meta.size(); ++l) {
      const int64_t it = c->r_iters.p[l];
      const sbq_ctx::LocusMeta& m = c->meta[l];
      it_total += it;
      frag_iters += m.frags * it;
      const int64_t b = (12 * m.nnz + 12 * (int64_t)m.R + 16 * (int64_t)m.T) * it;
      alg += b;
      if (is_grid[l]) galg += b;
      const int32_t li = l < c->locus_launch.size() ? c->locus_launch[l] : -1;
      if (li >= 0) {
         c->launch_stats[li].nnz += m.nnz;
         c->launch_stats[li].alg_bytes += b;
         c->launch_stats[li].frag_iters += m.frags * it;
         c->launch_stats[li].max_iters = std::max<int64_t>(c->launch_stats[li].max_iters, it);
      }
   }
   c->stats.em_iters_total = it_total;
   c->stats.frag_iters = frag_iters;
   c->stats.alg_bytes = alg;
   c->stats.grid_alg_bytes = galg;
   c->stats_stale = false;
}

extern "C" {

int sbq_results(sbq_ctx* c, double* theta, double* fpkm, double* frac, double* tpm, int32_t* keep, int32_t* iters, int32_t* status) {
   if (!c) return SBQ_ERR_INVALID;
   std::lock_guard<std::mutex> lk(c->mu);
   if (!c->downloaded) return fail(c, SBQ_ERR_STATE, "sbq_results before sbq_download / sbq_run");
   const size_t ni = c->n_iso, nl = c->n_loci;
   if (theta) memcpy(theta, c->r_theta.p, ni * 8);
   if (fpkm) memcpy(fpkm, c->r_fpkm.p, ni * 8);
   if (frac) memcpy(frac, c->r_frac.p, ni * 8);
   if (tpm) memcpy(tpm, c->r_tpm.p, ni * 8);
   if (keep) memcpy(keep, c->r_keep.p, ni * 4);
   if (iters) memcpy(iters, c->r_iters.p, nl * 4);
   if (status) memcpy(status, c->r_status.p, nl * 4);
   return SBQ_SUCCESS;
}

int sbq_get_stats(const sbq_ctx* cc, sbq_stats* out) {
   if (!cc || !out) return SBQ_ERR_INVALID;
   sbq_ctx* c = const_cast<sbq_ctx*>(cc);
   std::lock_guard<std::mutex> lk(c->mu);
   if (c->multi) {
      multi_stats(c, out);
      return SBQ_SUCCESS;
   }
   account(c);
   *out = c->stats;
   return SBQ_SUCCESS;
}

int sbq_set_insert_model(sbq_ctx* c, const sbq_insert_model* model, int32_t read_len) {
   if (!c || !model || read_len < 1) return SBQ_ERR_INVALID;
   std::lock_guard<std::mutex> lk(c->mu);
   c->model = *model;
// ... 204 lines not shown
   }
   if (rb_scan(st, b.is_rep, H, d_bs, b.cls_prefix)) return fail(c, SBQ_ERR_CUDA, "scan failed");
   rb_gather_kernel<<<(unsigned)((L + 1 + 255) / 256), 256, 0, st>>>(b.cls_prefix, b.loc_hit_off, L + 1, d_gather);
   std::vector<int64_t> cls_off(L + 1);
   CU(cudaMemcpyAsync(cls_off.data(), d_gather, (L + 1) * 8, cudaMemcpyDeviceToHost, st));
   if ((rc = check_flags("hits"))) return rc;
   const int64_t R = cls_off[L];
   std::vector<int64_t> cmask_off(L + 1, 0);
   std::vector<int32_t> class_locus((size_t)R);
   for (int64_t l = 0; l < L; ++l) {
      const int64_t W = (lio[l + 1] - lio[l] + 31) / 32;
      cmask_off[l + 1] = cmask_off[l] + (cls_off[l + 1] - cls_off[l]) * W;
      for (int64_t x = cls_off[l]; x < cls_off[l + 1]; ++x) class_locus[x] = (int32_t)l;
   }
   size_t need2 = 0;
   auto sz2 = [&](size_t bytes) { const size_t o = need2; need2 += align_up(bytes + 16); return o; };
   const int n_scan2 = (int)((std::max<int64_t>(R, 1) + RB_SCAN_BLOCK - 1) / RB_SCAN_BLOCK);
   const size_t p_co = sz2((L + 1) * 8), p_mo = sz2((L + 1) * 8), p_cl = sz2(R * 4), p_rep = sz2(R * 8), p_ms = sz2(R * 4), p_nf = sz2(R * 4), p_cmk = sz2(cmask_off[L] * 4),
                p_nz = sz2(R * 4), p_rp = sz2((R + 1) * 8), p_bs = sz2((size_t)n_scan2 * 8 + 8), p_g = sz2((L + 1) * 8);
   if (!c->d_raw2.reserve(need2)) return fail(c, SBQ_ERR_NOMEM, "device allocation failed (class arrays)");
   char* base2 = (char*)c->d_raw2.p;
   CU(cudaMemcpyAsync(base2 + p_co, cls_off.data(), (L + 1) * 8, cudaMemcpyHostToDevice, st));
   CU(cudaMemcpyAsync(base2 + p_mo, cmask_off.data(), (L + 1) * 8, cudaMemcpyHostToDevice, st));
   if (R) CU(cudaMemcpyAsync(base2 + p_cl, class_locus.data(), R * 4, cudaMemcpyHostToDevice, st));
   CU(cudaMemsetAsync(base2 + p_ms, 0, align_up(R * 4 + 16), st));
   CU(cudaMemsetAsync(base2 + p_nf, 0, align_up(R * 4 + 16), st));
   CU(cudaMemsetAsync(base2 + p_cmk, 0, align_up(cmask_off[L] * 4 + 16), st));
   b.loc_cls_off = (const int64_t*)(base2 + p_co); b.loc_cmask_off = (const int64_t*)(base2 + p_mo); b.class_rep = (int64_t*)(base2 + p_rep);
   b.class_mass = (float*)(base2 + p_ms); b.class_nfrag = (int32_t*)(base2 + p_nf); b.cmask = (uint32_t*)(base2 + p_cmk); b.class_nnz = (int32_t*)(base2 + p_nz);
   const int32_t* d_class_locus = (const int32_t*)(base2 + p_cl);
   int64_t* d_rp_tmp = (int64_t*)(base2 + p_rp);
   const int nbc = std::max(1, std::min<int>((int)((R + 127) / 128), c->prop.multiProcessorCount * 16));
   if (H) {
      raw_member_kernel<<<nbk, 256, 0, st>>>(b);
      raw_mass_kernel<<<nbk, 256, 0, st>>>(b);
   }
   if (R) raw_nnz_kernel<<<nbc, 256, 0, st>>>(b, R, d_class_locus);
   CU(cudaGetLastError());
   if (rb_scan(st, b.class_nnz, R, (long long*)(base2 + p_bs), d_rp_tmp)) return fail(c, SBQ_ERR_CUDA, "scan failed");
   rb_gather_kernel<<<(unsigned)((L + 1 + 255) / 256), 256, 0, st>>>(d_rp_tmp, b.loc_cls_off, L + 1, (int64_t*)(base2 + p_g));
   std::vector<int64_t> nz_off(L + 1);
   CU(cudaMemcpyAsync(nz_off.data(), base2 + p_g, (L + 1) * 8, cudaMemcpyDeviceToHost, st));
   if ((rc = check_flags("classes"))) return rc;
   c->n_row = R;
   c->nnz = nz_off[L];
   if ((rc = alloc_device(c))) return rc;
   DevParams& dp = c->dp;
   CU(cudaMemcpyAsync(const_cast<int64_t*>(dp.loc_row_off), cls_off.data(), (L + 1) * 8, cudaMemcpyHostToDevice, st));
   CU(cudaMemcpyAsync(const_cast<int64_t*>(dp.loc_iso_off), lio, (L + 1) * 8, cudaMemcpyHostToDevice, st));
   CU(cudaMemcpyAsync(const_cast<int64_t*>(dp.row_ptr), d_rp_tmp, (R + 1) * 8, cudaMemcpyDeviceToDevice, st));
   CU(cudaMemcpyAsync(const_cast<int32_t*>(dp.iso_len), c->h_iso_len.p, T * 4, cudaMemcpyHostToDevice, st));
   const int64_t nnz = c->nnz;
   const size_t b_seg = align_up(nnz * 8 + 8), b_n = align_up(nnz + 8), b_m = align_up(nnz * 4 + 8), b_l = align_up(nnz * 4 + 8), b_pool = align_up((size_t)nnz * RB_POOL * 4 + 8),
                b_emp = align_up(c->model_emp.size() * 8 + 8);
   if (!c->d_weights.reserve(b_seg + b_n + b_m + b_l + b_pool + b_emp)) return fail(c, SBQ_ERR_NOMEM, "device allocation failed (weight descriptors)");
   char* q = (char*)c->d_weights.p;
   int64_t* d_seg = (int64_t*)q; q += b_seg;
   uint8_t* d_n = (uint8_t*)q; q += b_n;
   uint32_t* d_m = (uint32_t*)q; q += b_m;
   int32_t* d_l = (int32_t*)q; q += b_l;
   uint32_t* d_pool = (uint32_t*)q; q += b_pool;
   double* d_emp = (double*)q;
   if (R) raw_fill_kernel<<<nbc, 128, 0, st>>>(b, R, d_class_locus, dp.row_ptr, const_cast<int32_t*>(dp.col), const_cast<double*>(dp.alpha), const_cast<int32_t*>(dp.count),
                                               d_seg, d_n, d_m, d_l, d_pool);
   CU(cudaGetLastError());
   if ((rc = check_flags("weights"))) return rc;
   CU(cudaEventRecord(c->ev[5], st));
   if (!r.long_read && nnz) {
      if (!c->model_emp.empty()) CU(cudaMemcpyAsync(d_emp, c->model_emp.data(), c->model_emp.size() * 8, cudaMemcpyHostToDevice, st));
      WeightModel wm{c->model.use_emp, c->model.start_offset, c->model.end_offset, c->model.total_reads, d_emp, c->model.mean, c->model.sd, c->model_read_len};
      const int blocks = std::max(1, std::min<int>((int)((nnz + 7) / 8), c->prop.multiProcessorCount * 16));
      weights_kernel<<<blocks, 256, 0, st>>>(nnz, d_seg, d_n, d_m, d_l, d_pool, wm, const_cast<double*>(dp.alpha));
      CU(cudaGetLastError());
   }
   CU(cudaEventRecord(c->ev[6], st));
   if (!c->r_frags.reserve((size_t)L) || !c->d_frags.reserve(align_up((size_t)L * 8))) return fail(c, SBQ_ERR_NOMEM, "fragment-total buffers");
   locus_frags_kernel<<<std::max(1, std::min<int>((int)((L + 7) / 8), c->prop.multiProcessorCount * 8)), 256, 0, st>>>(dp.loc_row_off, dp.count, L, (long long*)c->d_frags.p);
   CU(cudaMemcpyAsync(c->r_frags.p, c->d_frags.p, (size_t)L * 8, cudaMemcpyDeviceToHost, st));
   CU(cudaStreamSynchronize(st));
   c->meta.resize((size_t)L);
   for (int64_t l = 0; l < L; ++l) c->meta[l] = {nz_off[l + 1] - nz_off[l], c->r_frags.p[l], (int32_t)(cls_off[l + 1] - cls_off[l]), (int32_t)(lio[l + 1] - lio[l])};
   if ((rc = plan(c))) return rc;
   if (c->h_lists.n) CU(cudaMemcpyAsync(c->d_lists_p, c->h_lists.p, c->h_lists.n * sizeof(int32_t), cudaMemcpyHostToDevice, st));
   if (!c->classes.empty()) {
      if (!c->d_csc.reserve(align_up(c->nnz * 4 + 16))) return fail(c, SBQ_ERR_NOMEM, "device allocation failed (transposed-index scratch)");
      dp.csc = (unsigned*)c->d_csc.p;
   }
   CU(cudaEventRecord(c->ev[1], st));
   CU(cudaStreamSynchronize(st));
   float ms = 0;
   CU(cudaEventElapsedTime(&ms, c->ev[0], c->ev[1]));
   c->stats.upload_ms = ms;
   CU(cudaEventElapsedTime(&ms, c->ev[5], c->ev[6]));
   c->stats.weights_ms = ms;
   c->weights_ms = ms;
   c->stats.h2d_bytes = (int64_t)(H * 20 + r.hf_off.size() * 9 + r.if_off.size() * 9 + S * 8 + r.iso_seg.size() * 4 + T * 20 + L * 40);
   c->stats.n_loci = c->n_loci; c->stats.n_row = c->n_row; c->stats.n_iso = c->n_iso; c->stats.nnz = c->nnz;
   c->resident = true;
   c->col16_ready = false;
   c->solved = c->downloaded = false;
   return SBQ_SUCCESS;
}

extern "C" {

int sbq_fetch_raw_classes(sbq_ctx* c, int32_t* hit_class, uint8_t* hit_ncoord, uint16_t* hit_coords, int64_t* class_rep, float* class_mass, int32_t* class_nfrag) {
   if (!c) return SBQ_ERR_INVALID;
   std::lock_guard<std::mutex> lk(c->mu);
   if (c->multi) return fail(c, SBQ_ERR_UNSUPPORTED, "sbq_fetch_raw_classes is single-device (a test aid)");
   CU(cudaSetDevice(c->device));
   if (!c->resident || !c->raw_mode) return fail(c, SBQ_ERR_STATE, "sbq_fetch_raw_classes needs an uploaded raw batch");
   const RawBatch& b = c->rb;
   cudaStream_t st = c->stream;
   if (hit_class && b.n_hit) CU(cudaMemcpyAsync(hit_class, b.hit_class, b.n_hit * 4, cudaMemcpyDeviceToHost, st));
   if (hit_ncoord && b.n_hit) CU(cudaMemcpyAsync(hit_ncoord, b.ncoord, b.n_hit, cudaMemcpyDeviceToHost, st));
   if (hit_coords && b.n_hit) CU(cudaMemcpyAsync(hit_coords, b.coords, b.n_hit * RB_MAXC * 2, cudaMemcpyDeviceToHost, st));
   if (class_rep && c->n_row) CU(cudaMemcpyAsync(class_rep, b.class_rep, c->n_row * 8, cudaMemcpyDeviceToHost, st));
   if (class_mass && c->n_row) CU(cudaMemcpyAsync(class_mass, b.class_mass, c->n_row * 4, cudaMemcpyDeviceToHost, st));
   if (class_nfrag && c->n_row) CU(cudaMemcpyAsync(class_nfrag, b.class_nfrag, c->n_row * 4, cudaMemcpyDeviceToHost, st));
   CU(cudaStreamSynchronize(st));
   return SBQ_SUCCESS;
}

int sbq_synth_giant(sbq_ctx* c, const sbq_synth_giant_spec* sp) {
   if (!c || !sp || sp->n_loci < 1 || sp->rows_per_locus < 1 || sp->iso_lo < 1 || sp->iso_hi < sp->iso_lo || sp->iso_hi > SBQ_MAX_ISO ||
       !(sp->mean_extra >= 0) || sp->mean_extra > 200.0)
      return SBQ_ERR_INVALID;
   if (c->multi) return fail(c, SBQ_ERR_UNSUPPORTED, "sbq_synth_giant is per device: give every device of a partition its own locus ids");
   if (c->cfg.bias_mode) return fail(c, SBQ_ERR_UNSUPPORTED, "sbq_synth_giant generates no covariates");
   std::lock_guard<std::mutex> lk(c->mu);
   CU(cudaSetDevice(c->device));
   reset_batch(c);
   const int L = sp->n_loci;
   const int64_t rows = sp->rows_per_locus, n_row = (int64_t)L * rows;
   std::vector<SynthLocus> hl((size_t)L);
   std::vector<int64_t> h_lro((size_t)L + 1), h_lio((size_t)L + 1, 0);
   for (int l = 0; l < L; ++l) {
      const uint64_t id = sp->locus_ids ? (uint64_t)(uint32_t)sp->locus_ids[l] : (uint64_t)l;
      hl[l].key_deg = synth_key(sp->seed, id, 1);
      hl[l].key_ent = synth_key(sp->seed, id, 2);
      hl[l].key_len = synth_key(sp->seed, id, 3);
      hl[l].T = sp->iso_lo + (int32_t)(sm64(synth_key(sp->seed, id, 0)) % (uint64_t)(sp->iso_hi - sp->iso_lo + 1));
      hl[l].pad = 0;
      h_lro[l] = (int64_t)l * rows;
      h_lio[l + 1] = h_lio[l] + hl[l].T;
   }
   h_lro[L] = n_row;
   double cdf[SYN_CDF];
   {
      double pk = std::exp(-sp->mean_extra);
      cdf[0] = pk;
      for (int k = 1; k < SYN_CDF; ++k) {
         pk = pk * (sp->mean_extra / (double)k);
         cdf[k] = cdf[k - 1] + pk;
      }
   }
   const int n_scan = (int)((n_row + SYN_SCAN_BLOCK - 1) / SYN_SCAN_BLOCK);
   const size_t b_loci = align_up(L * sizeof(SynthLocus)), b_cdf = align_up(sizeof cdf), b_deg = align_up((size_t)n_row), b_sum = align_up((size_t)n_scan * 8 + 8);
   if (!c->d_synth.reserve(b_loci + b_cdf + b_deg + b_sum + 256)) return fail(c, SBQ_ERR_NOMEM, "device allocation failed (generator scratch)");
   char* q = (char*)c->d_synth.p;
   SynthLocus* d_loci = (SynthLocus*)q; q += b_loci;
   double* d_cdf = (double*)q; q += b_cdf;
   unsigned char* d_deg = (unsigned char*)q; q += b_deg;
   long long* d_bsum = (long long*)q; q += b_sum;
   unsigned long long* d_total = (unsigned long long*)q;
   cudaStream_t st = c->stream;
   CU(cudaEventRecord(c->ev[0], st));
   CU(cudaMemcpyAsync(d_loci, hl.data(), L * sizeof(SynthLocus), cudaMemcpyHostToDevice, st));
   CU(cudaMemcpyAsync(d_cdf, cdf, sizeof cdf, cudaMemcpyHostToDevice, st));
   CU(cudaMemsetAsync(d_total, 0, 8, st));
   const int nb = c->prop.multiProcessorCount * 8;
   synth_degree_kernel<<<nb, 256, 0, st>>>(d_loci, L, rows, d_cdf, d_deg, d_total);
   CU(cudaGetLastError());
   unsigned long long total = 0;
   CU(cudaMemcpyAsync(&total, d_total, 8, cudaMemcpyDeviceToHost, st));
   CU(cudaStreamSynchronize(st));
   c->n_loci = L; c->n_row = n_row; c->n_iso = h_lio[L]; c->nnz = (int64_t)total;
   {
      const int rc = alloc_device(c);
      if (rc) { reset_batch(c); return rc; }
   }
   DevParams& dp = c->dp;
   CU(cudaMemcpyAsync(const_cast<int64_t*>(dp.loc_row_off), h_lro.data(), (L + 1) * 8, cudaMemcpyHostToDevice, st));
   CU(cudaMemcpyAsync(const_cast<int64_t*>(dp.loc_iso_off), h_lio.data(), (L + 1) * 8, cudaMemcpyHostToDevice, st));
   synth_scan_sums_kernel<<<n_scan, 1024, 0, st>>>(d_deg, n_row, d_bsum);
   synth_scan_blocks_kernel<<<1, 1024, 0, st>>>(d_bsum, n_scan);
   synth_scan_fill_kernel<<<n_scan, 1024, 0, st>>>(d_deg, n_row, d_bsum, const_cast<int64_t*>(dp.row_ptr), const_cast<int32_t*>(dp.count));
   synth_fill_kernel<<<nb, 256, 0, st>>>(d_loci, L, rows, dp.row_ptr, const_cast<int32_t*>(dp.col), const_cast<double*>(dp.alpha));
   synth_len_kernel<<<std::min(L, 1024), 256, 0, st>>>(d_loci, L, dp.loc_iso_off, const_cast<int32_t*>(dp.iso_len));
   CU(cudaGetLastError());
   std::vector<int64_t> bound((size_t)L + 1);
   CU(cudaMemcpy2DAsync(bound.data(), 8, dp.row_ptr, (size_t)rows * 8, 8, (size_t)L + 1, cudaMemcpyDeviceToHost, st));
   CU(cudaStreamSynchronize(st));
   c->meta.resize((size_t)L);
   for (int l = 0; l < L; ++l) c->meta[l] = {bound[l + 1] - bound[l], rows, (int32_t)rows, hl[l].T};
   if (rows > INT32_MAX) return fail(c, SBQ_ERR_INVALID, "rows_per_locus too large");
   {
      const int rc = plan(c);
      if (rc) { reset_batch(c); return rc; }
   }
   if (c->h_lists.n) CU(cudaMemcpyAsync(c->d_lists_p, c->h_lists.p, c->h_lists.n * sizeof(int32_t), cudaMemcpyHostToDevice, st));
   if (!c->classes.empty()) {
      if (!c->d_csc.reserve(align_up(c->nnz * 4 + 16))) return fail(c, SBQ_ERR_NOMEM, "device allocation failed (transposed-index scratch)");
      dp.csc = (unsigned*)c->d_csc.p;
   }
   CU(cudaEventRecord(c->ev[1], st));
   CU(cudaStreamSynchronize(st));
   float ms = 0;
   CU(cudaEventElapsedTime(&ms, c->ev[0], c->ev[1]));
   c->stats.upload_ms = ms;
   c->stats.h2d_bytes = 0;
   c->stats.n_loci = c->n_loci; c->stats.n_row = c->n_row; c->stats.n_iso = c->n_iso; c->stats.nnz = c->nnz;
   c->stats.weights_ms = 0.0;
   c->deferred = 2;
   c->host_released = true;
   c->resident = true;
   c->col16_ready = false;
   c->solved = c->downloaded = false;
   return SBQ_SUCCESS;
}

int sbq_fetch_batch(sbq_ctx* c, int64_t* loc_row_off_, int64_t* loc_iso_off_, int64_t* row_ptr_, int32_t* col, double* alpha, int32_t* count, int32_t* iso_len) {
   if (!c) return SBQ_ERR_INVALID;
   if (c->multi) return fail(c, SBQ_ERR_UNSUPPORTED, "sbq_fetch_batch is single-device");
   std::lock_guard<std::mutex> lk(c->mu);
   CU(cudaSetDevice(c->device));
   if (!c->resident) return fail(c, SBQ_ERR_STATE, "sbq_fetch_batch before sbq_upload / sbq_synth_giant");
   { const int rcw = upload_wait(c); if (rcw) return rcw; }
   cudaStream_t st = c->stream;
   if (loc_row_off_) CU(cudaMemcpyAsync(loc_row_off_, c->dp.loc_row_off, (c->n_loci + 1) * 8, cudaMemcpyDeviceToHost, st));
   if (loc_iso_off_) CU(cudaMemcpyAsync(loc_iso_off_, c->dp.loc_iso_off, (c->n_loci + 1) * 8, cudaMemcpyDeviceToHost, st));
   if (row_ptr_) CU(cudaMemcpyAsync(row_ptr_, c->dp.row_ptr, (c->n_row + 1) * 8, cudaMemcpyDeviceToHost, st));
   if (col) CU(cudaMemcpyAsync(col, c->dp.col, c->nnz * 4, cudaMemcpyDeviceToHost, st));
   if (alpha) CU(cudaMemcpyAsync(alpha, c->dp.alpha, c->nnz * 8, cudaMemcpyDeviceToHost, st));
   if (count) CU(cudaMemcpyAsync(count, c->dp.count, c->n_row * 4, cudaMemcpyDeviceToHost, st));
   if (iso_len) CU(cudaMemcpyAsync(iso_len, c->dp.iso_len, c->n_iso * 4, cudaMemcpyDeviceToHost, st));
   CU(cudaStreamSynchronize(st));
   return SBQ_SUCCESS;
}

int sbq_fetch_alpha(sbq_ctx* c, double* alpha) {
   if (!c || !alpha) return SBQ_ERR_INVALID;
   if (c->multi) return fail(c, SBQ_ERR_UNSUPPORTED, "sbq_fetch_alpha is single-device");
   std::lock_guard<std::mutex> lk(c->mu);
   CU(cudaSetDevice(c->device));
   if (!c->resident) return fail(c, SBQ_ERR_STATE, "sbq_fetch_alpha before sbq_upload");
   { const int rcw = upload_wait(c); if (rcw) return rcw; }
   CU(cudaMemcpyAsync(alpha, c->dp.alpha, c->nnz * 8, cudaMemcpyDeviceToHost, c->stream));
   CU(cudaStreamSynchronize(c->stream));
   return SBQ_SUCCESS;
}

int sbq_set_covariates(sbq_ctx* c, const double* x, int64_t n_row, int32_t n_cov) {
   if (!c || n_cov < 0 || n_cov > BI_MAX_COV || (n_cov > 0 && !x)) return SBQ_ERR_INVALID;
   std::lock_guard<std::mutex> lk(c->mu);
   if (n_row != c->n_row) return fail(c, SBQ_ERR_INVALID, "covariates for %lld rows, %lld rows queued", (long long)n_row, (long long)c->n_row);
   cudaSetDevice(c->device);
   c->h_cov.clear();
   if (!c->h_cov.append(x, (size_t)n_row * n_cov)) return fail(c, SBQ_ERR_NOMEM, "pinned staging");
   c->n_cov = n_cov;
   c->have_cov = true;
   c->resident = c->solved = c->downloaded = false;
   return SBQ_SUCCESS;
}

int sbq_bias_results(sbq_ctx* c, double* beta, int32_t* outer_iters) {
   if (!c) return SBQ_ERR_INVALID;
   std::lock_guard<std::mutex> lk(c->mu);
   CU(cudaSetDevice(c->device));
   if (c->cfg.bias_mode != 1 || !c->solved) return fail(c, SBQ_ERR_STATE, "sbq_bias_results needs a solved bias-mode batch");
   if (c->multi) {
      MultiState& m = *c->multi;
      const size_t K = (size_t)c->n_cov;
      for (size_t i = 0; i < m.child.size(); ++i) {
         const size_t n = m.loci_of[i].size();
         if (!n) continue;
         std::vector<double> b(n * K + 1);
         std::vector<int32_t> o(n);
         const int rc = sbq_bias_results(m.child[i], b.data(), o.data());
         if (rc) return fail(c, rc, "device %d: %s", m.devices[i], m.child[i]->err.c_str());
         for (size_t x = 0; x < n; ++x) {
            const int32_t l = m.loci_of[i][x];
            if (beta && K) memcpy(beta + (size_t)l * K, b.data() + x * K, K * 8);
            if (outer_iters) outer_iters[l] = o[x];
         }
      }
      return SBQ_SUCCESS;
   }
// ... 92 lines not shown
```

### strawberry_b200/csrc/sbq_kernels.cuh

```cuda
#pragma once
#include <cooperative_groups.h>
#include <cuda_runtime.h>
#include <stdint.h>

namespace sbq {
namespace cg = cooperative_groups;

enum : int { LOCUS_OK = 0, LOCUS_ITER_CAP = 1, LOCUS_ZERO_DENOM = 2, LOCUS_NO_ROWS = 3 };

struct DevParams {
   const int64_t* loc_row_off;
   const int64_t* loc_iso_off;
   const int64_t* row_ptr;
   const int32_t* col;
   const double* alpha;
   const int32_t* count;
   const int32_t* iso_len;
   int32_t* neff;
   unsigned* csc;
   double* theta;
   double* fpkm;
   double* frac;
   int32_t* keep;
   int32_t* iters;
   int32_t* status;
   double* locus_fpkm;
   int max_iter;
   double tol;
   double row_eps;
   double min_frac;
   int eff_len_norm;
   double insert_mean;
   double rpm;
};

__device__ __forceinline__ double warp_sum(double v) {
#pragma unroll
   for (int o = 16; o > 0; o >>= 1) v += __shfl_xor_sync(0xffffffffu, v, o);
   return v;
}
__device__ __forceinline__ long long warp_sum_ll(long long v) {
#pragma unroll
   for (int o = 16; o > 0; o >>= 1) v += __shfl_xor_sync(0xffffffffu, v, o);
   return v;
}
template <int W>
__device__ __forceinline__ double group_sum(double v) {
#pragma unroll
   for (int o = W / 2; o > 0; o >>= 1) v += __shfl_xor_sync(0xffffffffu, v, o);
   return v;
}

__device__ __forceinline__ double iso_fpkm(const DevParams& p, double theta, int len, bool& na) {
   double kb;
   na = false;
   if (p.eff_len_norm) {
      kb = (double)len - p.insert_mean;
      if (kb < 0) { na = true; return 0.0; }
      kb = 1e3 / kb;
   } else {
      kb = 1e3 / (double)len;
   }
   return theta * p.rpm * kb;
}

#ifdef SBQ_TRACE
constexpr unsigned TRACE_CAP = 1u << 18;
__device__ unsigned long long g_trace[TRACE_CAP * 4];
__device__ unsigned g_trace_n;
__device__ __forceinline__ unsigned long long trace_now() { unsigned long long t; asm volatile("mov.u64 %0, %%globaltimer;" : "=l"(t)); return t; }
__device__ __forceinline__ unsigned trace_smid() { unsigned s; asm volatile("mov.u32 %0, %%smid;" : "=r"(s)); return s; }
__device__ __forceinline__ void trace_emit(unsigned cs, unsigned nt, int locus, unsigned rank, unsigned long long t0, int iters) {
   const unsigned i = atomicAdd(&g_trace_n, 1u);
   if (i < TRACE_CAP) {
      g_trace[4 * i] = ((unsigned long long)cs << 48) | ((unsigned long long)nt << 32) | (unsigned)locus;
      g_trace[4 * i + 1] = ((unsigned long long)rank << 48) | ((unsigned long long)trace_smid() << 32) | (unsigned)iters;
      g_trace[4 * i + 2] = t0;
      g_trace[4 * i + 3] = trace_now();
   }
}
#endif
constexpr int WT_WARPS = 8;
constexpr int WT_MAX_ISO = 32;
constexpr int WT_MAX_ROWS = 64;
constexpr int WT_MAX_NNZ = 256;
constexpr int WT_STRIDE = 33;

__host__ __device__ inline size_t warp_tier_smem_bytes(int max_iso) {
   return (size_t)WT_WARPS * ((size_t)max_iso * WT_STRIDE + WT_MAX_ISO) * sizeof(double);
}

// ... 118 lines not shown
               int x = 0;
               for (; x + 1 < nl; x += 2) {
                  n0 += acc[lane * WT_STRIDE + x];
                  n1 += acc[lane * WT_STRIDE + x + 1];
                  acc[lane * WT_STRIDE + x] = 0.0;
                  acc[lane * WT_STRIDE + x + 1] = 0.0;
               }
               if (x < nl) { n0 += acc[lane * WT_STRIDE + x]; acc[lane * WT_STRIDE + x] = 0.0; }
               nw = n0 + n1;
            }
            const double diff = lane < T ? nw - cur : 0.0;
            const double d2 = warp_sum(diff * diff);
            if (d2 < tol2) { status = LOCUS_OK; break; }
            cur = nw;
            __syncwarp();
            if (lane < T) th[lane] = (s != 0) ? cur / s : 0.0;
            __syncwarp();
         }
      }

      const double theta_out = (status == LOCUS_ZERO_DENOM || status == LOCUS_NO_ROWS) ? theta0 : cur;
      bool na = false;
      double f = 0.0;
      if (lane < T && status != LOCUS_NO_ROWS) f = iso_fpkm(p, theta_out, p.iso_len[t0 + lane], na);
      const double sum = warp_sum(f);
      double fr = 0.0;
      int kp = 0;
      if (lane < T && status != LOCUS_NO_ROWS) {
         if (!na) fr = f / sum;
         kp = !(fr < p.min_frac) ? (na ? -1 : 1) : 0;
      }
      const double kept_sum = warp_sum(kp != 0 ? f : 0.0);
      if (lane < T) {
         p.theta[t0 + lane] = theta_out;
         p.fpkm[t0 + lane] = f;
         p.frac[t0 + lane] = fr;
         p.keep[t0 + lane] = kp;
      }
      if (lane == 0) {
         p.iters[l] = iters;
         p.status[l] = status;
         p.locus_fpkm[l] = kept_sum;
      }
      __syncwarp();
   }
}

constexpr int CL_NT = 512;
constexpr int CL_NT_SMALL = 128;
constexpr int CL_LPR_STREAM = 32;

constexpr int CL_A2A_MAX = 4096;
constexpr size_t CL_SMEM_CAP = 220 * 1024;
__host__ __device__ inline int cluster_a2a_stride(int T) { return (T + 1) & ~1; }
__host__ __device__ inline bool cluster_a2a(int T, int cs, size_t slice_bytes) {
   if (cs <= 1 || (long long)cs * cluster_a2a_stride(T) > CL_A2A_MAX) return false;
   return ((size_t)4 * T + (size_t)cs * cluster_a2a_stride(T) + 64) * sizeof(double) + slice_bytes + 256 <= CL_SMEM_CAP;
}
__host__ __device__ inline size_t cluster_fixed_doubles(int T, int cs, size_t slice_bytes) {
   return (size_t)4 * T + (cluster_a2a(T, cs, slice_bytes) ? (size_t)cs * cluster_a2a_stride(T) + 64 : (size_t)2 * T + 64);
}

__host__ __device__ inline int cluster_stream_groups(int T, size_t smem_bytes, int nt, int cs, size_t slice_bytes) {
   const long long budget = (long long)(smem_bytes / sizeof(double)) - (long long)cluster_fixed_doubles(T, cs, slice_bytes);
   long long G = budget / (T > 0 ? T : 1);
   if (G > nt / CL_LPR_STREAM) G = nt / CL_LPR_STREAM;
   return (int)G;
}
__host__ __device__ inline int cluster_diag_slots(int T) { return (T + 7) & ~3; }
__host__ __device__ inline size_t cluster_resident_csr_bytes(size_t nnz_c, size_t nrows, int T) {
   const size_t npos = nnz_c + (size_t)T;
   return (npos + 1) * 8 + (nrows + 2) * 8 + (size_t)cluster_diag_slots(T) * 4 + nrows * 4 + ((size_t)T + 1) * 4 + nrows * 2 + npos * 2 + 64;
}
__host__ __device__ inline size_t cluster_resident_bytes(size_t nnz_c, size_t nrows, int T) {
   return cluster_resident_csr_bytes(nnz_c, nrows, T) + nnz_c * 4 + 4;
}

__host__ __device__ inline size_t cluster_class_smem(int max_iso, size_t slice_bytes, int nt, int cs) {
   const size_t fixed = cluster_fixed_doubles(max_iso, cs, slice_bytes) * sizeof(double);
   const size_t stream = (size_t)(nt / CL_LPR_STREAM) * max_iso * sizeof(double);
   const size_t want = fixed + (slice_bytes > stream ? slice_bytes : stream) + 256;
   return want < CL_SMEM_CAP ? want : CL_SMEM_CAP;
}
__host__ __device__ inline size_t cluster_slice_estimate(long long nnz, long long R, int T, int cs) {
   return (size_t)(1.12 * (double)cluster_resident_bytes((size_t)(nnz / cs + 1), (size_t)(R / cs + 1), T)) + 512;
}

template <int NT>
__device__ __forceinline__ double block_sum(double v, double* red) {
   v = warp_sum(v);
   if ((threadIdx.x & 31) == 0) red[threadIdx.x >> 5] = v;
   __syncthreads();
   double t = 0.0;
#pragma unroll
   for (int w = 0; w < NT / 32; ++w) t += red[w];
   __syncthreads();
   return t;
}

struct GlobalRows {
   const int64_t* rp;
   const double* al;
   const int32_t* col;
   int32_t* ne;
   int64_t k_a;
   __device__ __forceinline__ unsigned start(int i) const { return (unsigned)(rp[i] - k_a); }
   __device__ __forceinline__ double a(unsigned k) const { return al[k]; }
   __device__ __forceinline__ int c(unsigned k) const { return col[k]; }
   __device__ __forceinline__ int get_ne(int i) const { return ne[i]; }
   __device__ __forceinline__ void set_ne(int i, int v) const { ne[i] = v; }
};

template <int LPR, typename Rows>
__device__ __forceinline__ void cluster_setup_pass(const Rows& rows, const int32_t* __restrict__ cnt, int nrows, int G, int g, int lg,
                                                   double row_eps, double* my_acc, long long& tot, int& kept) {
   for (int base = 0; base < nrows; base += G) {
      const int i = base + g;
      const bool valid = i < nrows;
      unsigned k0 = 0, k1 = 0;
      int n = 0;
      if (valid) { k0 = rows.start(i); k1 = rows.start(i + 1); n = cnt[i]; }
      bool keep = false;
      for (unsigned k = k0 + lg; k < k1; k += LPR) keep |= rows.a(k) > row_eps;
#pragma unroll
      for (int o = LPR / 2; o > 0; o >>= 1) keep |= (bool)__shfl_xor_sync(0xffffffffu, (int)keep, o);
      if (valid && lg == 0) { rows.set_ne(i, keep ? n : -1); tot += n; kept += keep; }
      if (keep)
         for (unsigned k = k0 + lg; k < k1; k += LPR) my_acc[rows.c(k)] += rows.a(k);
      __syncwarp();
   }
}

template <int LPR, typename Rows>
__device__ __forceinline__ void cluster_em_pass(const Rows& rows, int nrows, int G, int g, int lg, const double* th, double* my_acc, int& zero) {
   for (int base = 0; base < nrows; base += 2 * G) {
      const int i0 = base + g, i1 = base + G + g;
      int ne0 = -1, ne1 = -1;
      unsigned a0 = 0, b0 = 0, a1 = 0, b1 = 0;
      if (i0 < nrows) { ne0 = rows.get_ne(i0); if (ne0 >= 0) { a0 = rows.start(i0); b0 = rows.start(i0 + 1); } }
      if (i1 < nrows) { ne1 = rows.get_ne(i1); if (ne1 >= 0) { a1 = rows.start(i1); b1 = rows.start(i1 + 1); } }
      double d0 = 0.0, d1 = 0.0;
      for (unsigned k = a0 + lg; k < b0; k += LPR) d0 += rows.a(k) * th[rows.c(k)];
      for (unsigned k = a1 + lg; k < b1; k += LPR) d1 += rows.a(k) * th[rows.c(k)];
#pragma unroll
      for (int o = LPR / 2; o > 0; o >>= 1) {
         d0 += __shfl_xor_sync(0xffffffffu, d0, o);
         d1 += __shfl_xor_sync(0xffffffffu, d1, o);
      }
      if (ne0 >= 0) {
         if (d0 == 0) zero = 1;
         else {
            const double r = (double)ne0 / d0;
            for (unsigned k = a0 + lg; k < b0; k += LPR) { const int c = rows.c(k); my_acc[c] += rows.a(k) * th[c] * r; }
         }
      }
      __syncwarp();
      if (ne1 >= 0) {
         if (d1 == 0) zero = 1;
         else {
            const double r = (double)ne1 / d1;
            for (unsigned k = a1 + lg; k < b1; k += LPR) { const int c = rows.c(k); my_acc[c] += rows.a(k) * th[c] * r; }
         }
      }
      __syncwarp();
   }
}

struct ResidentSlice {
// ... 261 lines not shown
   double d0 = 0.0, d1 = 0.0;
   int k = 4 * rs.q;
   for (; k + step + 4 <= len; k += 2 * step) {
      const uint4 o = *reinterpret_cast<const uint4*>(S.jd + k);
      const uint4 q = *reinterpret_cast<const uint4*>(S.jd + k + step);
      const unsigned p0 = o.x + s, p1 = o.y + s, p2 = o.z + s, p3 = o.w + s;
      const unsigned p4 = q.x + s, p5 = q.y + s, p6 = q.z + s, p7 = q.w + s;
      const int c0 = S.col[p0], c1 = S.col[p1], c2 = S.col[p2], c3 = S.col[p3];
      const int c4 = S.col[p4], c5 = S.col[p5], c6 = S.col[p6], c7 = S.col[p7];
      const double a0 = S.al[p0], a1 = S.al[p1], a2 = S.al[p2], a3 = S.al[p3];
      const double a4 = S.al[p4], a5 = S.al[p5], a6 = S.al[p6], a7 = S.al[p7];
      const double t0 = th[c0], t1 = th[c1], t2 = th[c2], t3 = th[c3];
      const double t4 = th[c4], t5 = th[c5], t6 = th[c6], t7 = th[c7];
      d0 += a0 * t0;
      d1 += a1 * t1;
      d0 += a2 * t2;
      d1 += a3 * t3;
      d0 += a4 * t4;
      d1 += a5 * t5;
      d0 += a6 * t6;
      d1 += a7 * t7;
   }
   for (; k < len; k += step) {
      const uint4 o = *reinterpret_cast<const uint4*>(S.jd + k);
      const bool v1 = k + 1 < len, v2 = k + 2 < len, v3 = k + 3 < len;
      const unsigned p0 = o.x + s, p1 = v1 ? o.y + s : S.npos, p2 = v2 ? o.z + s : S.npos, p3 = v3 ? o.w + s : S.npos;
      const double a0 = S.al[p0], a1 = S.al[p1], a2 = S.al[p2], a3 = S.al[p3];
      const int c0 = S.col[p0], c1 = S.col[p1], c2 = S.col[p2], c3 = S.col[p3];
      const double t0 = a0 * th[c0], t1 = a1 * th[c1], t2 = a2 * th[c2], t3 = a3 * th[c3];
      d0 += t0;
      d1 += v1 ? t1 : 0.0;
      d0 += v2 ? t2 : 0.0;
      d1 += v3 ? t3 : 0.0;
   }
   const double d = row_sum(d0 + d1, rs.q, rs.lanes, rs.n);
   if (rs.s >= 0 && rs.q == 0) {
      double r = 0.0;
      if (rs.ne >= 0) {
         if (d == 0) zero = 1; else r = (double)rs.ne / d;
      }
      S.r[s] = r;
   }
}

template <int NCACHE>
__device__ __forceinline__ void slot_col_pass(const ResidentSlice& S, const ColSlot<NCACHE>& cs, const double* scale) {
   double s0 = 0.0, s1 = 0.0;
   if (NCACHE > 0) {
#pragma unroll
      for (int u0 = 0; u0 < NCACHE; u0 += 8) {
         if (u0 < cs.ncache) {
#pragma unroll
            for (int u = u0; u < u0 + 8; u += 2) {
               s0 += S.al[cs.e[u] & 0xffffu] * S.r[cs.e[u] >> 16];
               s1 += S.al[cs.e[u + 1] & 0xffffu] * S.r[cs.e[u + 1] >> 16];
            }
         }
      }
   }
   if (cs.x_tail < cs.x1) {
      const unsigned pad = ((unsigned)S.nrows << 16) | S.npos;
      for (unsigned x = cs.x_tail; x < cs.x1; x += 8 * cs.lanes) {
         unsigned e[8];
#pragma unroll
         for (int u = 0; u < 8; ++u) e[u] = (x + u * cs.lanes < cs.x1) ? S.get_ent(x + u * cs.lanes) : pad;
         double a[8], r[8];
#pragma unroll
         for (int u = 0; u < 8; ++u) { a[u] = S.al[e[u] & 0xffffu]; r[u] = S.r[e[u] >> 16]; }
#pragma unroll
         for (int u = 0; u < 8; u += 2) {
            s0 += a[u] * r[u];
            s1 += a[u + 1] * r[u + 1];
         }
      }
   }
   const double sum = group_sum(s0 + s1, cs.q, cs.lanes, cs.wl);
   if (cs.j >= 0 && cs.q == 0) *cs.out = scale ? scale[cs.j] * sum : sum;
}

__device__ __forceinline__ void cluster_arrive_release() { asm volatile("barrier.cluster.arrive.release.aligned;" ::: "memory"); }
__device__ __forceinline__ void cluster_arrive_relaxed() { asm volatile("barrier.cluster.arrive.relaxed.aligned;" ::: "memory"); }
__device__ __forceinline__ void cluster_wait() { asm volatile("barrier.cluster.wait.acquire.aligned;" ::: "memory"); }

struct OwnerMap {
   cg::cluster_group* cluster;
   double* stage;
   int B;
   unsigned rank, CS;
   __device__ __forceinline__ double* ptr(int j) const {
      const int o = j / B;
      double* base = CS > 1 ? cluster->map_shared_rank(stage, (unsigned)o) : stage;
      return base + (size_t)rank * B + (j - o * B);
   }
};
struct LocalOut {
   double* out;
   __device__ __forceinline__ double* ptr(int j) const { return out + j; }
};

template <int NT, int NCACHE, int MINB>
__global__ void __launch_bounds__(NT, MINB)
em_cluster_kernel(DevParams p, const int32_t* __restrict__ list, int n_list, unsigned smem_launch) {
   cg::cluster_group cluster = cg::this_cluster();
   const unsigned CS = cluster.num_blocks();
   const unsigned rank = cluster.block_rank();
   const int item = blockIdx.x / CS;
   const int l = list[item];
   const int tid = threadIdx.x, lane = tid & 31;
#ifdef SBQ_TRACE
   const unsigned long long trace_t0 = trace_now();
#endif

   const int64_t r0 = p.loc_row_off[l];
   const int R = (int)(p.loc_row_off[l + 1] - r0);
   const int64_t t0 = p.loc_iso_off[l];
   const int T = (int)(p.loc_iso_off[l + 1] - t0);

   extern __shared__ double smem[];
   double* th = smem;
   double* bufA = th + T;
   double* bufB = bufA + T;
   double* sdiv = bufB + T;
   double* part = sdiv + T;
   const int64_t* __restrict__ rp = p.row_ptr + r0;
   const size_t slice_est = cluster_slice_estimate((long long)(rp[R] - rp[0]), R, T, (int)CS);
   double* dyn = smem + cluster_fixed_doubles(T, (int)CS, slice_est);
   __shared__ double red[NT / 32];
   __shared__ int s_rows[2];
   double* cur = bufA;
   double* nxt = bufB;

   const unsigned smem_bytes = min(smem_launch, (unsigned)cluster_class_smem(T, slice_est, NT, (int)CS));

   if (tid < 2) {
      const int64_t base = rp[0], nnz = rp[R] - base;
      const int64_t target = base + (nnz * (int64_t)(rank + tid)) / CS;
      int lo = 0, hi = R;
      if (rank + tid >= CS) lo = R;
      else if (rank + tid == 0) hi = 0;
      while (lo < hi) {
         const int mid = (lo + hi) >> 1;
         if (rp[mid] < target) lo = mid + 1; else hi = mid;
      }
      s_rows[tid] = lo;
   }
   __syncthreads();
   const int ra = s_rows[0], rb = s_rows[1], nrows = rb - ra;
   const int64_t k_a = rp[ra];
   const unsigned nnz_c = (unsigned)(rp[rb] - k_a);

   const size_t used = (size_t)((char*)dyn - (char*)smem);
   const int lpr = lanes_for(nrows, NT), lpc = lanes_for(T, NT);
   int too_long = 0;
   for (int i = tid; i < nrows; i += NT) too_long |= (rp[ra + i + 1] - rp[ra + i]) > (int64_t)T;
   too_long = __syncthreads_or(too_long);
   const bool small_idx = (uint64_t)nnz_c + (uint64_t)T <= 65535u && nrows <= 65535 && !too_long;
   const unsigned npos = nnz_c + (unsigned)T;
   const bool csc_in_smem = small_idx && used + cluster_resident_bytes(nnz_c, (size_t)nrows, T) <= smem_bytes;
   const bool resident = small_idx && used + cluster_resident_csr_bytes(nnz_c, (size_t)nrows, T) <= smem_bytes;
   const int jdn = cluster_diag_slots(T);
   ResidentSlice S;
   S.al = dyn;
   S.r = S.al + npos + 1;
   S.jd = (unsigned*)(S.r + nrows + 1 + ((npos + nrows) & 1u));
   S.ne = (int*)(S.jd + jdn);
   S.cp = (unsigned*)(S.ne + nrows);
   S.rlen = (unsigned short*)(S.cp + T + 1);
   S.col = S.rlen + nrows;
   S.ent = (unsigned*)(S.col + npos + 1 + ((npos + 1 + nrows) & 1u));
   S.ent_g = p.csc + (size_t)k_a;
   S.n_ent_s = 0;
   if (csc_in_smem) S.n_ent_s = nnz_c;
   else if (resident) S.n_ent_s = (unsigned)min((size_t)nnz_c, (smem_bytes - used - cluster_resident_csr_bytes(nnz_c, (size_t)nrows, T)) / 4);
   S.nrows = nrows; S.T = T; S.nnz = nnz_c; S.npos = npos;
   GlobalRows grows{rp + ra, p.alpha + k_a, p.col + k_a, p.neff + r0 + ra, k_a};
   const int G = resident ? 0 : cluster_stream_groups(T, smem_bytes, NT, (int)CS, slice_est);
   double* acc = dyn;
   const int g32 = tid / CL_LPR_STREAM, lg32 = tid % CL_LPR_STREAM;
   double* my_acc = acc + (size_t)(g32 < G ? g32 : 0) * T;
   const bool use_slots = resident && T <= NT;
   const bool use_row_slots = resident && nrows <= NT;
   ColSlot<NCACHE> slot;
   slot.j = -1; slot.q = 0; slot.lanes = 1; slot.wl = 1; slot.x_tail = slot.x1 = 0; slot.ncache = 0; slot.out = part;
   RowSlot rslot;
   rslot.s = -1; rslot.q = 0; rslot.lanes = 1; rslot.n = 1; rslot.len = 0; rslot.ne = -1;

#ifdef SBQ_PHASE_TIMING
   long long ph[8] = {0, 0, 0, 0, 0, 0, 0, 0};
#define SBQ_TICK(k) { const long long t_ = clock64(); ph[k] += t_ - t_prev; t_prev = t_; }
#define SBQ_STICK(k) { const long long t_ = clock64(); st[k] += t_ - t_prev; t_prev = t_; }
   long long st[8] = {0, 0, 0, 0, 0, 0, 0, 0};
   long long t_prev = clock64();
   const long long t_start = t_prev;
#else
#define SBQ_TICK(k)
#define SBQ_STICK(k)
#endif
   long long tot = 0;
   int kept = 0;
   if (resident) {
      unsigned* keys = (unsigned*)S.al;
      int P = 1;
      while (P < nrows) P <<= 1;
      for (int i = tid; i < P; i += NT)
         keys[i] = i < nrows ? ((65535u - (unsigned)(rp[ra + i + 1] - rp[ra + i])) << 16) | (unsigned)i : 0xffffffffu;
      __syncthreads();
      for (int kk = 2; kk <= P; kk <<= 1) {
         for (int jj = kk >> 1; jj > 0; jj >>= 1) {
            for (int i = tid; i < P; i += NT) {
               const int x = i ^ jj;
               if (x > i) {
                  const unsigned a = keys[i], b = keys[x];
                  if (((i & kk) == 0) ? (a > b) : (a < b)) { keys[i] = b; keys[x] = a; }
               }
            }
            __syncthreads();
         }
      }
      SBQ_STICK(0)
      for (int i = tid; i < nrows; i += NT) {
         const unsigned key = keys[i];
         S.rlen[i] = (unsigned short)(65535u - (key >> 16));
         S.ne[i] = (int)(key & 0xffffu);
      }
      for (int j = tid; j <= T; j += NT) S.cp[j] = 0;
      __syncthreads();
      for (int k = tid; k < jdn; k += NT) {
         unsigned v = 0;
         if (k > 0) {
            int lo = 0, hi = nrows;
            while (lo < hi) {
               const int mid = (lo + hi) >> 1;
               if ((int)S.rlen[mid] > k - 1) lo = mid + 1; else hi = mid;
            }
            v = (unsigned)lo | (lo > 0 ? 1u : 0u);
         }
         S.jd[k] = v;
      }
      __syncthreads();
      if (tid < 32) {
         const int chunk = (jdn + 31) / 32, k0 = lane * chunk, k1 = min(jdn, k0 + chunk);
         unsigned sum = 0;
         for (int k = k0; k < k1; ++k) sum += S.jd[k];
         unsigned incl = sum;
         for (int o = 1; o < 32; o <<= 1) {
            const unsigned v = __shfl_up_sync(0xffffffffu, incl, o);
            if (lane >= o) incl += v;
         }
         unsigned run = incl - sum;
         for (int k = k0; k < k1; ++k) { run += S.jd[k]; S.jd[k] = run; }
      }
      __syncthreads();
      SBQ_STICK(1)
      {
         const int32_t* __restrict__ cnt = p.count + r0 + ra;
         int lf = 1;
         while (lf < 32 && (long long)lf * nrows < (long long)nnz_c) lf <<= 1;
         const int g = tid / lf, lg = tid % lf, par = NT / lf;
         for (int base = 0; base < nrows; base += 2 * par) {
            int sv[2], iv[2], lenv[2], keepv[2];
            unsigned g0v[2];
            double a[2][4];
            int c[2][4];
#pragma unroll
            for (int r = 0; r < 2; ++r) {
               sv[r] = base + r * par + g;
               iv[r] = 0; lenv[r] = 0; g0v[r] = 0; keepv[r] = 0;
               if (sv[r] < nrows) {
                  iv[r] = S.ne[sv[r]];
                  lenv[r] = S.rlen[sv[r]];
               }
// ... 107 lines not shown
      __shared__ unsigned s_slot[NT];
      __shared__ int s_lanes[NT];
      __shared__ int s_total;
      if (use_row_slots) {
         const unsigned info = assign_row_slots<NT>(S.rlen, nrows, nnz_c, s_slot);
         if (info != 0xffffffffu) {
            const int first = (int)(info & 0xffffu), n = (int)((info >> 16) & 0xffu), L = (int)(info >> 24);
            rslot.lanes = L;
            rslot.n = n;
            rslot.q = lane / n;
            const int row = first + lane % n;
            if (rslot.q < L && row < nrows) {
               rslot.s = row;
               rslot.ne = S.ne[row];
               rslot.len = rslot.ne >= 0 ? (int)S.rlen[row] : 0;
            } else {
               rslot.q = L;
            }
         }
      }
      SBQ_STICK(4)
      if (use_slots) {
         const int len_j = tid < T ? (int)(S.cp[tid + 1] - S.cp[tid]) : 0;
         const unsigned sl = assign_slots<NT>(T, len_j, nnz_c, s_slot, s_lanes, &s_total);
         const unsigned pad = ((unsigned)nrows << 16) | npos;
         if (sl != 0xffffffffu) {
            slot.j = (int)(sl & 0xffffu);
            slot.lanes = (int)(sl >> 24);
            slot.q = (int)((sl >> 16) & 0xffu);
            const unsigned x0 = S.cp[slot.j] + (unsigned)slot.q;
            slot.x1 = S.cp[slot.j + 1];
            slot.x_tail = x0 + (unsigned)NCACHE * slot.lanes;
            if (NCACHE > 0) {
#pragma unroll
               for (int u = 0; u < NCACHE; ++u) {
                  const unsigned x = x0 + (unsigned)u * slot.lanes;
                  const bool v = x < slot.x1;
                  slot.e[u] = v ? S.get_ent(x) : pad;
                  slot.ncache += v;
               }
            }
            slot.out = part + slot.j;
         } else if (NCACHE > 0) {
#pragma unroll
            for (int u = 0; u < NCACHE; ++u) slot.e[u] = pad;
         }
         slot.wl = __reduce_max_sync(0xffffffffu, slot.lanes);
         SBQ_STICK(5)
         slot_col_pass(S, slot, nullptr);
      } else {
         resident_col_pass<NT>(S, nullptr, LocalOut{part}, lpc);
      }
   } else {
      for (int x = tid; x < G * T; x += NT) acc[x] = 0.0;
      __syncthreads();
      if (g32 < G) cluster_setup_pass<CL_LPR_STREAM>(grows, p.count + r0 + ra, nrows, G, g32, lg32, p.row_eps, my_acc, tot, kept);
      __syncthreads();
      for (int j = tid; j < T; j += NT) {
         double sj = 0.0;
         for (int gg = 0; gg < G; ++gg) { sj += acc[(size_t)gg * T + j]; acc[(size_t)gg * T + j] = 0.0; }
         part[j] = sj;
      }
   }
   {
      const double tot_b = block_sum<NT>((double)tot, red);
      const double kept_b = block_sum<NT>((double)kept, red);
      if (tid == 0) { part[T + 1] = tot_b; part[T + 2] = kept_b; }
   }
   cluster.sync();
   double total = 0.0, kept_all = 0.0;
   for (unsigned r = 0; r < CS; ++r) {
      const double* rp_part = CS > 1 ? cluster.map_shared_rank(part, r) : part;
      total += rp_part[T + 1];
      kept_all += rp_part[T + 2];
   }
   for (int j = tid; j < T; j += NT) {
      double sj = 0.0;
      for (unsigned r = 0; r < CS; ++r) {
         const double* rp_part = CS > 1 ? cluster.map_shared_rank(part, r) : part;
         sj += rp_part[j];
      }
      sdiv[j] = sj;
   }
   const double theta0 = total / (double)T;
   for (int j = tid; j < T; j += NT) { cur[j] = theta0; th[j] = theta0; }
   cluster.sync();

   const double tol2 = p.tol * p.tol;
   int status = LOCUS_ITER_CAP, iters = 0;
#ifdef SBQ_PHASE_TIMING
   const long long t_setup = clock64() - t_start;
   t_prev = clock64();
#endif
   const bool a2a = cluster_a2a(T, (int)CS, slice_est);
   const int Tp = cluster_a2a_stride(T);
   const int B = a2a ? Tp : (T + (int)CS - 1) / (int)CS;
   double* stage = part;
   double* dsq = a2a ? part + (size_t)CS * Tp : part + T + 16;
   double* flags = a2a ? dsq + 16 : part + 2 * T + 32;
   double* d2p = flags + 16;
   const OwnerMap own{&cluster, a2a ? stage + (size_t)rank * Tp : stage, a2a ? T : B, a2a ? 0u : rank, a2a ? 1u : CS};
   if (slot.j >= 0) slot.out = own.ptr(slot.j);
   const int nb = max(0, min(B, T - (int)rank * B));
   bool pend_b = false;
   if (kept_all == 0) {
      status = LOCUS_NO_ROWS;
   } else {
      for (int it = 0; it < p.max_iter; ++it) {
         iters = it + 1;
         int zero = 0;
         if (resident) {
            if (use_row_slots) slot_e_pass(S, rslot, th, zero);
            else if (lpr == 1) resident_e_pass_rows4<NT>(S, th, zero);
            else resident_e_pass<NT>(S, th, lpr, zero);
            SBQ_TICK(0)
            zero = __syncthreads_or(zero);
            SBQ_TICK(1)
            if (use_slots) slot_col_pass(S, slot, th);
            else resident_col_pass<NT>(S, th, own, lpc);
            SBQ_TICK(2)
         } else {
            if (g32 < G) cluster_em_pass<CL_LPR_STREAM>(grows, nrows, G, g32, lg32, th, my_acc, zero);
            zero = __syncthreads_or(zero);
            for (int j = tid; j < T; j += NT) {
               double sj = 0.0;
               for (int gg = 0; gg < G; ++gg) { sj += acc[(size_t)gg * T + j]; acc[(size_t)gg * T + j] = 0.0; }
               *own.ptr(j) = sj;
            }
         }
         double d2 = 0.0;
         if (CS == 1) {
            __syncthreads();
            SBQ_TICK(3)
            if (zero) { status = LOCUS_ZERO_DENOM; break; }
            double dd = 0.0;
            for (int j = tid; j < T; j += NT) {
               const double v = stage[j], sj = sdiv[j];
               nxt[j] = v;
               th[j] = (sj != 0) ? v / sj : 0.0;
               const double diff = v - cur[j];
               dd += diff * diff;
            }
            if ((tid & ~31) < T) dd = warp_sum(dd);
            if (lane == 0) dsq[tid >> 5] = dd;
            SBQ_TICK(4)
            __syncthreads();
            SBQ_TICK(6)
#pragma unroll
            for (int w = 0; w < NT / 32; ++w) d2 += dsq[w];
         } else if (a2a) {
            __syncthreads();
            if (pend_b) { cluster_wait(); pend_b = false; }
            {
               const int half = Tp >> 1, items = ((int)CS - 1) * half;
               const double2* mine = reinterpret_cast<const double2*>(stage + (size_t)rank * Tp);
               for (int x = tid; x < items; x += NT) {
                  const int pr = x / half, jj = x - pr * half;
                  const unsigned peer = (rank + 1u + (unsigned)pr) & (CS - 1u);
                  reinterpret_cast<double2*>(cluster.map_shared_rank(stage, peer) + (size_t)rank * Tp)[jj] = mine[jj];
               }
               if (tid < (int)CS) cluster.map_shared_rank(flags, (unsigned)tid)[rank] = (double)zero;
            }
            SBQ_TICK(3)
            cluster_arrive_release();
            cluster_wait();
            SBQ_TICK(4)
            double zf = 0.0;
            for (unsigned r = 0; r < CS; ++r) zf += flags[r];
            if (zf != 0.0) { status = LOCUS_ZERO_DENOM; break; }
            double dd = 0.0;
            for (int j = tid; j < T; j += NT) {
               double a[16];
#pragma unroll
               for (int r = 0; r < 16; ++r) a[r] = r < (int)CS ? stage[(size_t)r * Tp + j] : 0.0;
#pragma unroll
               for (int o = 8; o > 0; o >>= 1)
#pragma unroll
                  for (int r = 0; r < o; ++r) a[r] += a[r + o];
               const double v = a[0], sj = sdiv[j];
               nxt[j] = v;
               th[j] = (sj != 0) ? v / sj : 0.0;
               const double diff = v - cur[j];
               dd += diff * diff;
            }
            if ((tid & ~31) < T) dd = warp_sum(dd);
            if (lane == 0) dsq[tid >> 5] = dd;
            SBQ_TICK(5)
            __syncthreads();
            cluster_arrive_relaxed();
            pend_b = true;
            SBQ_TICK(6)
#pragma unroll
            for (int w = 0; w < NT / 32; ++w) d2 += dsq[w];
         } else {
            if (tid < (int)CS) cluster.map_shared_rank(flags, (unsigned)tid)[rank] = (double)zero;
            cluster.sync();
            SBQ_TICK(3)
            double zf = 0.0;
            for (unsigned r = 0; r < CS; ++r) zf += flags[r];
            if (zf != 0.0) { status = LOCUS_ZERO_DENOM; break; }
            {
               const int items = nb * (int)CS;
               const unsigned r = (unsigned)tid % CS;
               double* peer_nxt = cluster.map_shared_rank(nxt, r);
               double* peer_th = cluster.map_shared_rank(th, r);
               for (int base = 0; base < items; base += NT) {
                  const int x = base + tid, jj = x / (int)CS;
                  double v = x < items ? stage[(size_t)r * B + jj] : 0.0;
                  for (unsigned o = CS >> 1; o > 0; o >>= 1) v += __shfl_xor_sync(0xffffffffu, v, o);
                  if (x < items) {
                     const int j = (int)rank * B + jj;
                     const double sj = sdiv[j];
                     peer_nxt[j] = v;
                     peer_th[j] = (sj != 0) ? v / sj : 0.0;
                     if (r == 0) { const double diff = v - cur[j]; dsq[jj] = diff * diff; }
                  }
               }
            }
            SBQ_TICK(4)
            __syncthreads();
            if (tid < 32) {
               double d = 0.0;
               for (int jj = lane; jj < nb; jj += 32) d += dsq[jj];
               d = warp_sum(d);
               if (lane < (int)CS) cluster.map_shared_rank(d2p, (unsigned)lane)[rank] = d;
            }
            SBQ_TICK(5)
            cluster.sync();
            SBQ_TICK(6)
            for (unsigned r = 0; r < CS; ++r) d2 += d2p[r];
         }
         if (d2 < tol2) { status = LOCUS_OK; break; }
         { double* t_ = cur; cur = nxt; nxt = t_; }
         SBQ_TICK(7)
      }
   }
#ifdef SBQ_PHASE_TIMING
   if (rank == 0 && (tid == 0 || tid == NT - 32))
      printf("setup: sort %lld jd %lld fill %lld csc %lld rowslots %lld colslots %lld\n", st[0], st[1], st[2], st[3], st[4], st[5]);
   if (rank == 0 && (tid == 0 || tid == NT - 32))
      printf("locus %d tid %d iters %d resident %d csc_smem %d slots %d/%d lanes %d/%d ncache %d lpr %d lpc %d nrows %d nnz %u setup %lld | E %lld or %lld col %lld csync1 %lld own %lld d2 %lld csync2 %lld chk %lld (cycles/iter)\n", l, tid, iters,
             (int)resident, (int)csc_in_smem, (int)use_row_slots, (int)use_slots, rslot.lanes, slot.lanes, slot.ncache, lpr, lpc, nrows, nnz_c, t_setup, ph[0] / iters, ph[1] / iters, ph[2] / iters, ph[3] / iters, ph[4] / iters, ph[5] / iters, ph[6] / iters, ph[7] / iters);
#endif
   if (pend_b) cluster_wait();
   cluster.sync();
#ifdef SBQ_TRACE
   if (tid == 0) trace_emit(CS, NT, l, rank, trace_t0, iters);
#endif

   if (rank != 0) return;
   const bool uniform = status == LOCUS_ZERO_DENOM || status == LOCUS_NO_ROWS;
   double fsum = 0.0;
   for (int j = tid; j < T; j += NT) {
      const double tj = uniform ? theta0 : cur[j];
      bool na = false;
      double f = 0.0;
      if (status != LOCUS_NO_ROWS) f = iso_fpkm(p, tj, p.iso_len[t0 + j], na);
      p.theta[t0 + j] = tj;
      p.fpkm[t0 + j] = f;
      th[j] = na ? -1.0 : 0.0;
      fsum += f;
   }
   fsum = block_sum<NT>(fsum, red);
   double ksum = 0.0;
   for (int j = tid; j < T; j += NT) {
      const bool na = th[j] < 0;
      const double f = p.fpkm[t0 + j];
      double fr = 0.0;
      int kp = 0;
      if (status != LOCUS_NO_ROWS) {
         if (!na) fr = f / fsum;
         kp = !(fr < p.min_frac) ? (na ? -1 : 1) : 0;
      }
      p.frac[t0 + j] = fr;
      p.keep[t0 + j] = kp;
      if (kp != 0) ksum += f;
   }
   ksum = block_sum<NT>(ksum, red);
   if (tid == 0) {
      p.iters[l] = iters;
      p.status[l] = status;
      p.locus_fpkm[l] = ksum;
   }
}

__global__ void __launch_bounds__(1024) fpkm_sum_kernel(const double* __restrict__ locus_fpkm, int64_t n, double* out) {
   __shared__ double red[32];
   double v = 0.0;
   for (int64_t i = threadIdx.x; i < n; i += 1024) v += locus_fpkm[i];
   v = block_sum<1024>(v, red);
   if (threadIdx.x == 0) *out = v;
}

__global__ void tpm_kernel(const double* __restrict__ fpkm, double* __restrict__ tpm, int64_t n, double total) {
   const int64_t i = (int64_t)blockIdx.x * blockDim.x + threadIdx.x;
   if (i < n) tpm[i] = 1e6 * fpkm[i] / total;
}

__global__ void __launch_bounds__(256) locus_frags_kernel(const int64_t* __restrict__ loc_row_off, const int32_t* __restrict__ count, int64_t n_loci, long long* __restrict__ out) {
   const int lane = threadIdx.x & 31;
   const int64_t nw = ((int64_t)gridDim.x * blockDim.x) >> 5;
   for (int64_t l = ((int64_t)blockIdx.x * blockDim.x + threadIdx.x) >> 5; l < n_loci; l += nw) {
      long long v = 0;
      for (int64_t i = loc_row_off[l] + lane; i < loc_row_off[l + 1]; i += 32) v += count[i];
      v = warp_sum_ll(v);
      if (lane == 0) out[l] = v;
   }
}

__global__ void tpm_dev_kernel(const double* __restrict__ fpkm, double* __restrict__ tpm, int64_t n, const double* __restrict__ total) {
   const int64_t i = (int64_t)blockIdx.x * blockDim.x + threadIdx.x;
   const double tot = *total;
   if (i < n) tpm[i] = 1e6 * fpkm[i] / tot;
}

}
```

Baseline: 51.17 billion.

## Span giant loci across multiple thread-block clusters with global-memory cross-cluster reduction

Adds a multi-cluster path for loci too large to fit a 16-CTA cluster: each locus is split across several clusters (32 CTAs total) launched cooperatively. Per-iteration partial sums go to global scratch and the clusters meet at an epoch-tagged flag barrier with a timeout. This lets the data stay resident in shared memory across more SMs instead of spilling. The cost is a global-memory handshake every EM iteration, extra scratch allocation, and a fallback to the single-cluster path if the cooperative launch fails.

```diff
diff --git a/include/sbq.h b/include/sbq.h
--- a/include/sbq.h
+++ b/include/sbq.h
@@ -19,7 +19,7 @@
    SBQ_ERR_UNSUPPORTED = -6
 } sbq_error;
 
-typedef enum { SBQ_LOCUS_OK = 0, SBQ_LOCUS_ITER_CAP = 1, SBQ_LOCUS_ZERO_DENOM = 2, SBQ_LOCUS_NO_ROWS = 3 } sbq_locus_status;
+typedef enum { SBQ_LOCUS_OK = 0, SBQ_LOCUS_ITER_CAP = 1, SBQ_LOCUS_ZERO_DENOM = 2, SBQ_LOCUS_NO_ROWS = 3, SBQ_LOCUS_SYNC_TIMEOUT = 4 } sbq_locus_status;
 
 #define SBQ_MAX_ISO 3600
 
diff --git a/strawberry_b200/api.py b/strawberry_b200/api.py
--- a/strawberry_b200/api.py
+++ b/strawberry_b200/api.py
@@ -10,7 +10,7 @@
 LIB_PATH = os.environ.get("SBQ_LIB_PATH", os.path.join(_HERE, "libsbq.so"))
 
 SBQ_SUCCESS, SBQ_ERR_INVALID, SBQ_ERR_NO_DEVICE, SBQ_ERR_CUDA, SBQ_ERR_NOMEM, SBQ_ERR_STATE, SBQ_ERR_UNSUPPORTED = 0, -1, -2, -3, -4, -5, -6
-LOCUS_OK, LOCUS_ITER_CAP, LOCUS_ZERO_DENOM, LOCUS_NO_ROWS = 0, 1, 2, 3
+LOCUS_OK, LOCUS_ITER_CAP, LOCUS_ZERO_DENOM, LOCUS_NO_ROWS, LOCUS_SYNC_TIMEOUT = 0, 1, 2, 3, 4
 
 ABI_SYMBOLS = [
     "sbq_abi_version", "sbq_error_string", "sbq_last_error", "sbq_config_default", "sbq_create", "sbq_destroy",
@@ -275,7 +275,8 @@
         grid = {1: "em_grid_kernel", 2: "em_grid_tma_kernel", 3: "em_grid_dual_kernel"}
         return [dict(kernel=grid.get(buf[i].variant, names[buf[i].kind]) if buf[i].kind == 3 else names[buf[i].kind], cluster_size=buf[i].cluster_size, lanes_per_row=buf[i].lanes_per_row,
                      n_loci=buf[i].n_loci, nnz=buf[i].nnz, ms=buf[i].ms, alg_bytes=buf[i].alg_bytes,
-                     frag_iters=buf[i].frag_iters, max_iters=buf[i].max_iters, start_ms=buf[i].start_ms, threads=buf[i].lanes_per_row) for i in range(min(n, cap))]
+                     frag_iters=buf[i].frag_iters, max_iters=buf[i].max_iters, start_ms=buf[i].start_ms, threads=buf[i].lanes_per_row,
+                     variant=buf[i].variant) for i in range(min(n, cap))]
 
     def synth_giant(self, locus_ids, rows_per_locus, seed=4, iso_lo=500, iso_hi=800, mean_extra=47.0):
         ids = _c(locus_ids, np.int32)
diff --git a/strawberry_b200/csrc/sbq.cu b/strawberry_b200/csrc/sbq.cu
--- a/strawberry_b200/csrc/sbq.cu
+++ b/strawberry_b200/csrc/sbq.cu
@@ -92,6 +92,10 @@
    size_t max_slice = 0;
    size_t list_off = 0;
    size_t smem = 0;
+   int kc = 1;
+   size_t fb_smem = 0;
+   size_t xc_off = 0;
+   bool fell_back = false;
 };
 
 struct BiasClass {
@@ -187,6 +191,8 @@
    size_t warp_list_off = 0, grid_list_off = 0;
 
    DevBuf d_in, d_out, d_lists, d_grid_scratch, d_col16, d_rowrec, d_csc, d_synth, d_pk;
+   DevBuf d_xc;
+   unsigned long long xc_epoch = 0;
    bool col16_ready = false, grid_tma_ok = false, grid_dual_ok = false;
    std::vector<int32_t> sgrid_list;
    std::vector<int64_t> sgrid_rec_off;
@@ -310,6 +316,12 @@
 }
 #define SGRID_CTAS sgrid_ctas()
 
+constexpr int XC_CTAS = 32;
+inline int xc_cs() {
+   static const int v = getenv("SBQ_XC_CS") && atoi(getenv("SBQ_XC_CS")) == 8 ? 8 : 16;
+   return v;
+}
+
 int cluster_size_for(int64_t nnz) {
    static int64_t th[4] = {16 * 1024, 32 * 1024, 64 * 1024, 150 * 1024};
    static bool init = false;
@@ -351,7 +363,7 @@
    static const bool sgrid_enabled = !getenv("SBQ_NO_SGRID");
    std::vector<char> dual_locus(c->n_loci, 0);
    std::vector<int64_t> nnz_of(c->n_loci);
-   LaunchClass* slot[5][N_BUCKETS] = {};
+   LaunchClass* slot[6][N_BUCKETS] = {};
    std::vector<LaunchClass> tmp;
    tmp.reserve(20);
    static const int64_t grid_min_nnz = getenv("SBQ_GRID_MIN_NNZ") ? atoll(getenv("SBQ_GRID_MIN_NNZ")) : 300 * 1000;
@@ -390,12 +402,18 @@
             if (!grid_tma_supports((int)T, (long long)R, small ? SGRID_CTAS : c->prop.multiProcessorCount)) tma_ok = false;
          }
       } else {
-         int cs = c->force_cluster ? c->force_cluster : cluster_size_for(nnz);
-         int csi = cs == 1 ? 0 : cs == 2 ? 1 : cs == 4 ? 2 : cs == 8 ? 3 : 4;
-         const size_t slice = cluster_slice_estimate(nnz, R, (int)T, cs);
+         int cs = c->force_cluster ? c->force_cluster : cluster_size_for(nnz), kc = 1;
+         if (cs == XC_CTAS || (cs == 16 && !c->force_cluster && !cluster_slice_fits(nnz, R, (int)T, 16, 16))) {
+            const int xcs = xc_cs();
+            if (xc_shape_ok(nnz, R, (int)T, XC_CTAS / xcs, xcs)) { kc = XC_CTAS / xcs; cs = xcs; }
+            else cs = 16;
+         }
+         const int csi = kc > 1 ? 5 : cs == 1 ? 0 : cs == 2 ? 1 : cs == 4 ? 2 : cs == 8 ? 3 : 4;
+         const size_t slice = cluster_slice_estimate(nnz, R, (int)T, cs * kc);
          const int bucket = cs == 1 ? smem_bucket(cluster_fixed_doubles((int)T, 1, slice) * sizeof(double) + slice + 256) : N_BUCKETS - 1;
          if (!slot[csi][bucket]) {
             tmp.push_back(LaunchClass{cs, BUCKET_NT[bucket], {}, 0, 0, 0, 0});
+            tmp.back().kc = kc;
             slot[csi][bucket] = &tmp.back();
          }
          LaunchClass* lc = slot[csi][bucket];
@@ -403,6 +421,7 @@
          lc->max_iso = std::max(lc->max_iso, (int)T);
          lc->max_slice = std::max(lc->max_slice, slice);
          lc->smem = std::max(lc->smem, cluster_class_smem((int)T, slice, lc->lpr, cs));
+         if (kc > 1) lc->fb_smem = std::max(lc->fb_smem, cluster_class_smem((int)T, cluster_slice_estimate(nnz, R, (int)T, 16), lc->lpr, 16));
       }
    }
    auto by_size = [&](int32_t a, int32_t b) { return nnz_of[a] != nnz_of[b] ? nnz_of[a] > nnz_of[b] : a < b; };
@@ -441,7 +460,9 @@
          return fail(c, SBQ_ERR_UNSUPPORTED, "locus with %d isoforms does not fit the cluster tier", lc.max_iso);
       c->classes.push_back(std::move(lc));
    }
-   std::sort(c->classes.begin(), c->classes.end(), [](const LaunchClass& a, const LaunchClass& b) { return a.cs != b.cs ? a.cs > b.cs : a.max_slice > b.max_slice; });
+   std::sort(c->classes.begin(), c->classes.end(), [](const LaunchClass& a, const LaunchClass& b) {
+      return a.cs * a.kc != b.cs * b.kc ? a.cs * a.kc > b.cs * b.kc : a.max_slice > b.max_slice;
+   });
 
    c->h_lists.clear();
    c->warp_list_off = 0;
@@ -526,7 +547,66 @@
    cfg.attrs = attr;
    cfg.numAttrs = 1;
    const int32_t* list = c->d_lists_p + lc.list_off;
-   CU(cudaLaunchKernelEx(&cfg, kernel, c->dp, list, (int)lc.loci.size(), (unsigned)lc.smem));
+   CU(cudaLaunchKernelEx(&cfg, kernel, c->dp, list, (int)lc.loci.size(), (unsigned)lc.smem, XcArgs{nullptr, nullptr, 1, 0, 0}));
+   return SBQ_SUCCESS;
+}
+
+int launch_xc_class(sbq_ctx* c, LaunchClass& lc, cudaStream_t st) {
+   auto kernel = em_cluster_kernel<CL_NT, 0, 1>;
+   int rc = set_kernel_attrs(c, kernel, std::max(lc.smem, lc.fb_smem), true);
+   if (rc) return rc;
+   cudaLaunchConfig_t cfg{};
+   cfg.gridDim = dim3((unsigned)(lc.cs * lc.kc));
+   cfg.blockDim = dim3(CL_NT);
+   cfg.dynamicSmemBytes = lc.smem;
+   cfg.stream = st;
+   cudaLaunchAttribute attr[2];
+   attr[0].id = cudaLaunchAttributeClusterDimension;
+   attr[0].val.clusterDim.x = (unsigned)lc.cs;
+   attr[0].val.clusterDim.y = 1;
+   attr[0].val.clusterDim.z = 1;
+   attr[1].id = cudaLaunchAttributeCooperative;
+   attr[1].val.cooperative = 1;
+   cfg.attrs = attr;
+   cfg.numAttrs = 2;
+   int max_clusters = 0;
+   const size_t n = lc.loci.size();
+   const int w = xc_row_stride(lc.max_iso);
+   const size_t per = cudaOccupancyMaxActiveClusters(&max_clusters, kernel, &cfg) == cudaSuccess ? (size_t)(max_clusters / lc.kc) : 0;
+   lc.fell_back = per == 0;
+   for (size_t s = 0; s < n && !lc.fell_back; s += per) {
+      const size_t m = std::min(per, n - s);
+      char* base = (char*)c->d_xc.p + lc.xc_off;
+      const XcArgs xa{(double*)(base + n * XC_FLAGS * 8) + s * 2 * lc.kc * w, (unsigned long long*)base + s * XC_FLAGS, lc.kc, w, c->xc_epoch};
+      cfg.gridDim = dim3((unsigned)(m * lc.cs * lc.kc));
+      const cudaError_t e = cudaLaunchKernelEx(&cfg, kernel, c->dp, c->d_lists_p + lc.list_off + s, (int)m, (unsigned)lc.smem, xa);
+      if (e != cudaSuccess && s > 0) return fail(c, SBQ_ERR_CUDA, "multi-cluster launch failed: %s", cudaGetErrorString(e));
+      lc.fell_back = e != cudaSuccess;
+   }
+   if (!lc.fell_back) return SBQ_SUCCESS;
+   cudaGetLastError();
+   LaunchClass fb = lc;
+   fb.cs = 16;
+   fb.kc = 1;
+   fb.smem = lc.fb_smem;
+   return launch_cluster_class_nt<CL_NT, 0, 1>(c, fb, st);
+}
+
+int cluster_scratch(sbq_ctx* c, cudaStream_t st) {
+   if (c->classes.empty()) return SBQ_SUCCESS;
+   if (!c->d_csc.reserve(align_up(c->nnz * 4 + 16))) return fail(c, SBQ_ERR_NOMEM, "device allocation failed (transposed-index scratch)");
+   c->dp.csc = (unsigned*)c->d_csc.p;
+   size_t xb = 0;
+   for (auto& lc : c->classes) {
+      if (lc.kc == 1) continue;
+      lc.xc_off = xb;
+      xb += align_up(lc.loci.size() * (XC_FLAGS * 8 + (size_t)2 * lc.kc * xc_row_stride(lc.max_iso) * sizeof(double)));
+   }
+   if (xb) {
+      const size_t cap0 = c->d_xc.cap;
+      if (!c->d_xc.reserve(xb)) return fail(c, SBQ_ERR_NOMEM, "device allocation failed (cross-cluster scratch)");
+      if (c->d_xc.cap != cap0) CU(cudaMemsetAsync(c->d_xc.p, 0, c->d_xc.cap, st));
+   }
    return SBQ_SUCCESS;
 }
 
@@ -690,7 +770,7 @@
    c->h_lists.release();
    c->r_theta.release(); c->r_fpkm.release(); c->r_frac.release(); c->r_tpm.release();
    c->r_locus_fpkm.release(); c->r_keep.release(); c->r_iters.release(); c->r_status.release(); c->r_frags.release(); c->d_frags.release();
-   c->d_in.release(); c->d_out.release(); c->d_lists.release(); c->d_grid_scratch.release(); c->d_col16.release(); c->d_rowrec.release(); c->d_csc.release(); c->d_synth.release(); c->d_pk.release(); c->d_raw.release(); c->d_raw2.release(); c->d_bias.release();
+   c->d_in.release(); c->d_out.release(); c->d_lists.release(); c->d_grid_scratch.release(); c->d_col16.release(); c->d_rowrec.release(); c->d_csc.release(); c->d_xc.release(); c->d_synth.release(); c->d_pk.release(); c->d_raw.release(); c->d_raw2.release(); c->d_bias.release();
    c->d_sgrid_scratch.release(); c->d_srowrec.release(); c->d_spk.release();
    c->h_cov.release(); c->r_beta.release(); c->r_outer.release();
    c->h_wseg.release(); c->h_wn.release(); c->h_wmask.release(); c->h_wpool.release(); c->h_wlen.release(); c->h_wpool_off.release(); c->d_weights.release();
@@ -713,8 +793,9 @@
 int sbq_set_plan(sbq_ctx* c, int force_tier, int force_cluster) {
    if (!c) return SBQ_ERR_INVALID;
    if (force_tier < 0 || force_tier > 3) return fail(c, SBQ_ERR_INVALID, "force_tier must be 0..3");
-   if (force_cluster != 0 && force_cluster != 1 && force_cluster != 2 && force_cluster != 4 && force_cluster != 8 && force_cluster != 16)
-      return fail(c, SBQ_ERR_INVALID, "force_cluster must be 0, 1, 2, 4, 8 or 16");
+   if (force_cluster != 0 && force_cluster != 1 && force_cluster != 2 && force_cluster != 4 && force_cluster != 8 && force_cluster != 16 &&
+       force_cluster != XC_CTAS)
+      return fail(c, SBQ_ERR_INVALID, "force_cluster must be 0, 1, 2, 4, 8, 16 or %d", XC_CTAS);
    if (c->force_tier != force_tier || c->force_cluster != force_cluster) c->resident = c->solved = c->downloaded = false;
    c->force_tier = force_tier;
    c->force_cluster = force_cluster;
@@ -863,6 +944,7 @@
       }
    }
    if (timing) fprintf(stderr, "SBQ_TIMING plan_ms %.3f\n", std::chrono::duration<double, std::milli>(std::chrono::steady_clock::now() - t_plan0).count());
+   if (int rc_s = cluster_scratch(c, st)) return rc_s;
    if (c->h_lists.n) CU(cudaMemcpyAsync(c->d_lists_p, c->h_lists.p, c->h_lists.n * sizeof(int32_t), cudaMemcpyHostToDevice, st));
    const int64_t* lro = loc_row_off(c);
    const int64_t* rp = row_ptr(c);
@@ -905,10 +987,6 @@
       if (i < done.size()) pos = std::max(pos, done[i].second);
    }
    CU(cudaEventRecord(c->ev[1], st));
-   if (!c->classes.empty()) {
-      if (!c->d_csc.reserve(align_up(c->nnz * 4 + 16))) return fail(c, SBQ_ERR_NOMEM, "device allocation failed (transposed-index scratch)");
-      dp.csc = (unsigned*)c->d_csc.p;
-   }
    c->stats.h2d_bytes = 2 * (c->n_loci + 1) * 8 + (c->n_row + 1) * 8 + c->nnz * 12 + c->n_row * 4 + c->n_iso * 4 + (int64_t)c->h_lists.n * 4;
    c->stats.n_loci = c->n_loci; c->stats.n_row = c->n_row; c->stats.n_iso = c->n_iso; c->stats.nnz = c->nnz;
    c->stats.weights_ms = 0.0;
@@ -1119,6 +1197,7 @@
    }
    CU(cudaEventRecord(c->ev[2], st));
    CU(cudaEventRecord(c->ev_fork, st));
+   ++c->xc_epoch;
    int used_side = 0;
    c->stats.grid_em_ms = 0;
    for (auto& t : c->lt) t.used = false;
@@ -1206,7 +1285,7 @@
       for (int i = 0; i < ncls; ++i) {
          const LaunchClass& lc = c->classes[i];
          if (lc.lpr < CL_NT) small.push_back(i);
-         else if (lc.cs >= (order_mode == 3 ? 16 : 8)) big.push_back(i);
+         else if (lc.cs * lc.kc >= (order_mode == 3 ? 16 : 8)) big.push_back(i);
          else rest.push_back(i);
       }
       if (order_mode == 1) { ord = small; ord.insert(ord.end(), big.begin(), big.end()); ord.insert(ord.end(), rest.begin(), rest.end()); warp_pos = 0; }
@@ -1241,14 +1320,15 @@
       }
       if (pos == ncls) break;
       const int i = ord[pos];
-      const LaunchClass& lc = c->classes[i];
+      LaunchClass& lc = c->classes[i];
       cudaStream_t ss = serialize ? st : c->side[i % N_SIDE_STREAMS];
       if (!serialize && i < N_SIDE_STREAMS) CU(cudaStreamWaitEvent(ss, c->ev_fork, 0));
       if (pending) CU(cudaStreamWaitEvent(ss, (i < N_SIDE_STREAMS && c->class_ready[i]) ? c->ev_class_ready[i] : c->ev[1], 0));
       LaunchTimer& t = c->lt[2 + i % N_SIDE_STREAMS];
       CU(cudaEventRecord(t.e0, ss));
-      int rc = lc.lpr == 64 ? launch_cluster_class_nt<64, 0, 8>(c, lc, ss) : lc.lpr == 128 ? launch_cluster_class_nt<128, 0, 4>(c, lc, ss) :
-               lc.lpr == 256 ? launch_cluster_class_nt<256, 0, 2>(c, lc, ss) : launch_cluster_class_nt<CL_NT, 0, 1>(c, lc, ss);
+      int rc = lc.kc > 1 ? launch_xc_class(c, lc, ss) : lc.lpr == 64 ? launch_cluster_class_nt<64, 0, 8>(c, lc, ss) :
+               lc.lpr == 128 ? launch_cluster_class_nt<128, 0, 4>(c, lc, ss) : lc.lpr == 256 ? launch_cluster_class_nt<256, 0, 2>(c, lc, ss) :
+               launch_cluster_class_nt<CL_NT, 0, 1>(c, lc, ss);
       if (rc) return rc;
       CU(cudaEventRecord(t.e1, ss));
       t.used = true;
@@ -1299,7 +1379,9 @@
    for (size_t i = 0; i < c->classes.size(); ++i) {
       LaunchTimer& t = c->lt[2 + i % N_SIDE_STREAMS];
       CU(cudaEventElapsedTime(&ms, t.e0, t.e1));
-      add_stat(2, c->classes[i].cs, c->classes[i].lpr, c->classes[i].loci, ms, t.e0);
+      const LaunchClass& lc = c->classes[i];
+      add_stat(2, lc.fell_back ? 16 : lc.cs * lc.kc, lc.lpr, lc.loci, ms, t.e0);
+      c->launch_stats.back().variant = lc.kc == 1 ? 0 : lc.fell_back ? 2 : 1;
    }
    c->stats.kernel_launches = launches;
    c->solved = true;
@@ -1385,6 +1467,9 @@
 
    c->stats_stale = true;
    c->downloaded = true;
+   for (const LaunchClass& lc : c->classes)
+      for (int32_t l : lc.kc > 1 ? lc.loci : std::vector<int32_t>())
+         if (c->r_status.p[l] == LOCUS_SYNC_TIMEOUT) return fail(c, SBQ_ERR_CUDA, "locus %d: clusters of a multi-cluster locus lost each other (wait timed out)", l);
    return SBQ_SUCCESS;
 }
 
@@ -1755,10 +1840,7 @@
    for (int64_t l = 0; l < L; ++l) c->meta[l] = {nz_off[l + 1] - nz_off[l], c->r_frags.p[l], (int32_t)(cls_off[l + 1] - cls_off[l]), (int32_t)(lio[l + 1] - lio[l])};
    if ((rc = plan(c))) return rc;
    if (c->h_lists.n) CU(cudaMemcpyAsync(c->d_lists_p, c->h_lists.p, c->h_lists.n * sizeof(int32_t), cudaMemcpyHostToDevice, st));
-   if (!c->classes.empty()) {
-      if (!c->d_csc.reserve(align_up(c->nnz * 4 + 16))) return fail(c, SBQ_ERR_NOMEM, "device allocation failed (transposed-index scratch)");
-      dp.csc = (unsigned*)c->d_csc.p;
-   }
+   if (int rc_s = cluster_scratch(c, st)) return rc_s;
    CU(cudaEventRecord(c->ev[1], st));
    CU(cudaStreamSynchronize(st));
    float ms = 0;
@@ -1873,10 +1955,7 @@
       if (rc) { reset_batch(c); return rc; }
    }
    if (c->h_lists.n) CU(cudaMemcpyAsync(c->d_lists_p, c->h_lists.p, c->h_lists.n * sizeof(int32_t), cudaMemcpyHostToDevice, st));
-   if (!c->classes.empty()) {
-      if (!c->d_csc.reserve(align_up(c->nnz * 4 + 16))) return fail(c, SBQ_ERR_NOMEM, "device allocation failed (transposed-index scratch)");
-      dp.csc = (unsigned*)c->d_csc.p;
-   }
+   if (int rc_s = cluster_scratch(c, st)) return rc_s;
    CU(cudaEventRecord(c->ev[1], st));
    CU(cudaStreamSynchronize(st));
    float ms = 0;
diff --git a/strawberry_b200/csrc/sbq_kernels.cuh b/strawberry_b200/csrc/sbq_kernels.cuh
--- a/strawberry_b200/csrc/sbq_kernels.cuh
+++ b/strawberry_b200/csrc/sbq_kernels.cuh
@@ -6,7 +6,7 @@
 namespace sbq {
 namespace cg = cooperative_groups;
 
-enum : int { LOCUS_OK = 0, LOCUS_ITER_CAP = 1, LOCUS_ZERO_DENOM = 2, LOCUS_NO_ROWS = 3 };
+enum : int { LOCUS_OK = 0, LOCUS_ITER_CAP = 1, LOCUS_ZERO_DENOM = 2, LOCUS_NO_ROWS = 3, LOCUS_SYNC_TIMEOUT = 4 };
 
 struct DevParams {
    const int64_t* loc_row_off;
@@ -291,8 +291,27 @@
    const size_t want = fixed + (slice_bytes > stream ? slice_bytes : stream) + 256;
    return want < CL_SMEM_CAP ? want : CL_SMEM_CAP;
 }
-__host__ __device__ inline size_t cluster_slice_estimate(long long nnz, long long R, int T, int cs) {
-   return (size_t)(1.12 * (double)cluster_resident_bytes((size_t)(nnz / cs + 1), (size_t)(R / cs + 1), T)) + 512;
+__host__ __device__ inline size_t cluster_slice_estimate(long long nnz, long long R, int T, int ctas) {
+   return (size_t)(1.12 * (double)cluster_resident_bytes((size_t)(nnz / ctas + 1), (size_t)(R / ctas + 1), T)) + 512;
+}
+__host__ __device__ inline bool cluster_slice_fits(long long nnz, long long R, int T, int ctas, int cs) {
+   const size_t s = cluster_slice_estimate(nnz, R, T, ctas);
+   return cluster_fixed_doubles(T, cs, s) * sizeof(double) + s + 256 <= CL_SMEM_CAP;
+}
+
+struct XcArgs {
+   double* rows;
+   unsigned long long* flags;
+   int kc;
+   int w;
+   unsigned long long epoch;
+};
+constexpr int XC_FLAGS = 16;
+constexpr unsigned XC_ABORT = 0xffffffffu;
+constexpr unsigned long long XC_TIMEOUT_NS = 1000000000ull;
+__host__ __device__ inline int xc_row_stride(int max_iso) { return (max_iso + 3) & ~1; }
+__host__ __device__ inline bool xc_shape_ok(long long nnz, long long R, int T, int kc, int cs) {
+   return cluster_slice_fits(nnz, R, T, kc * cs, cs) && cluster_a2a(T, cs, cluster_slice_estimate(nnz, R, T, kc * cs));
 }
 
 template <int NT>
@@ -720,6 +739,53 @@
 __device__ __forceinline__ void cluster_arrive_relaxed() { asm volatile("barrier.cluster.arrive.relaxed.aligned;" ::: "memory"); }
 __device__ __forceinline__ void cluster_wait() { asm volatile("barrier.cluster.wait.acquire.aligned;" ::: "memory"); }
 
+__device__ __forceinline__ double* xc_row(const XcArgs& x, int item, int u, unsigned cidx) {
+   return x.rows + (((size_t)item * 2 + (size_t)(u & 1)) * x.kc + cidx) * x.w;
+}
+__device__ __forceinline__ bool xc_sync(const XcArgs& x, int item, int u, unsigned cidx, unsigned rank, unsigned CS, unsigned* go,
+                                        cg::cluster_group& cluster) {
+   unsigned long long* fl = x.flags + (size_t)item * XC_FLAGS;
+   const unsigned long long tag = (x.epoch << 32) | (unsigned)(u + 1);
+   __syncthreads();
+   if (rank == 0 && threadIdx.x < 32) {
+      const int lane = threadIdx.x;
+      if (lane == 0) {
+         __threadfence();
+         asm volatile("st.relaxed.gpu.global.u64 [%0], %1;" ::"l"(fl + cidx), "l"(tag) : "memory");
+      }
+      bool ok = true;
+      if (lane < (int)CS) {
+         unsigned long long t0, t;
+         asm volatile("mov.u64 %0, %%globaltimer;" : "=l"(t0));
+         for (int k = 0; k < x.kc && ok; ++k) {
+            for (;;) {
+               unsigned long long v;
+               asm volatile("ld.acquire.gpu.global.u64 %0, [%1];" : "=l"(v) : "l"(fl + k) : "memory");
+               if (v >= tag) break;
+               asm volatile("mov.u64 %0, %%globaltimer;" : "=l"(t));
+               if (t - t0 > XC_TIMEOUT_NS) { ok = false; break; }
+            }
+         }
+      }
+      ok = __all_sync(0xffffffffu, ok);
+      if (lane < (int)CS) {
+         unsigned* dst = cluster.map_shared_rank(go, (unsigned)lane);
+         asm volatile("st.release.cluster.u32 [%0], %1;" ::"l"(dst), "r"(ok ? (unsigned)(u + 1) : XC_ABORT) : "memory");
+      }
+   }
+   if (threadIdx.x == 0) {
+      unsigned g;
+      do { asm volatile("ld.acquire.cluster.u32 %0, [%1];" : "=r"(g) : "l"(go) : "memory"); } while (g < (unsigned)(u + 1));
+   }
+   __syncthreads();
+   return *(volatile unsigned*)go != XC_ABORT;
+}
+__device__ __forceinline__ double xc_sum(const XcArgs& x, int item, int u, int j) {
+   double v = 0.0;
+   for (int k = 0; k < x.kc; ++k) v += __ldcg(xc_row(x, item, u, (unsigned)k) + j);
+   return v;
+}
+
 struct OwnerMap {
    cg::cluster_group* cluster;
    double* stage;
@@ -738,11 +804,14 @@
 
 template <int NT, int NCACHE, int MINB>
 __global__ void __launch_bounds__(NT, MINB)
-em_cluster_kernel(DevParams p, const int32_t* __restrict__ list, int n_list, unsigned smem_launch) {
+em_cluster_kernel(DevParams p, const int32_t* __restrict__ list, int n_list, unsigned smem_launch, XcArgs xc) {
    cg::cluster_group cluster = cg::this_cluster();
    const unsigned CS = cluster.num_blocks();
    const unsigned rank = cluster.block_rank();
-   const int item = blockIdx.x / CS;
+   const unsigned KC = (unsigned)xc.kc;
+   const unsigned cidx = (blockIdx.x / CS) % KC;
+   const unsigned NC = KC * CS, grank = cidx * CS + rank;
+   const int item = blockIdx.x / NC;
    const int l = list[item];
    const int tid = threadIdx.x, lane = tid & 31;
 #ifdef SBQ_TRACE
@@ -761,10 +830,12 @@
    double* sdiv = bufB + T;
    double* part = sdiv + T;
    const int64_t* __restrict__ rp = p.row_ptr + r0;
-   const size_t slice_est = cluster_slice_estimate((long long)(rp[R] - rp[0]), R, T, (int)CS);
+   const size_t slice_est = cluster_slice_estimate((long long)(rp[R] - rp[0]), R, T, (int)NC);
    double* dyn = smem + cluster_fixed_doubles(T, (int)CS, slice_est);
    __shared__ double red[NT / 32];
    __shared__ int s_rows[2];
+   __shared__ unsigned s_go;
+   if (tid == 0) s_go = 0;
    double* cur = bufA;
    double* nxt = bufB;
 
@@ -772,10 +843,10 @@
 
    if (tid < 2) {
       const int64_t base = rp[0], nnz = rp[R] - base;
-      const int64_t target = base + (nnz * (int64_t)(rank + tid)) / CS;
+      const int64_t target = base + (nnz * (int64_t)(grank + tid)) / NC;
       int lo = 0, hi = R;
-      if (rank + tid >= CS) lo = R;
-      else if (rank + tid == 0) hi = 0;
+      if (grank + tid >= NC) lo = R;
+      else if (grank + tid == 0) hi = 0;
       while (lo < hi) {
          const int mid = (lo + hi) >> 1;
          if (rp[mid] < target) lo = mid + 1; else hi = mid;
@@ -824,7 +895,7 @@
    rslot.s = -1; rslot.q = 0; rslot.lanes = 1; rslot.n = 1; rslot.len = 0; rslot.ne = -1;
 
 #ifdef SBQ_PHASE_TIMING
-   long long ph[8] = {0, 0, 0, 0, 0, 0, 0, 0};
+   long long ph[9] = {0, 0, 0, 0, 0, 0, 0, 0, 0};
 #define SBQ_TICK(k) { const long long t_ = clock64(); ph[k] += t_ - t_prev; t_prev = t_; }
 #define SBQ_STICK(k) { const long long t_ = clock64(); st[k] += t_ - t_prev; t_prev = t_; }
    long long st[8] = {0, 0, 0, 0, 0, 0, 0, 0};
@@ -1098,6 +1169,20 @@
       }
       sdiv[j] = sj;
    }
+   bool xc_ok = true;
+   if (KC > 1) {
+      double* xr = xc_row(xc, item, 0, cidx);
+      if (rank == 0) {
+         for (int j = tid; j < T; j += NT) __stcg(xr + j, sdiv[j]);
+         if (tid == 0) { __stcg(xr + T, total); __stcg(xr + T + 1, kept_all); }
+      }
+      xc_ok = xc_sync(xc, item, 0, cidx, rank, CS, &s_go, cluster);
+      if (xc_ok) {
+         total = xc_sum(xc, item, 0, T);
+         kept_all = xc_sum(xc, item, 0, T + 1);
+         for (int j = tid; j < T; j += NT) sdiv[j] = xc_sum(xc, item, 0, j);
+      }
+   }
    const double theta0 = total / (double)T;
    for (int j = tid; j < T; j += NT) { cur[j] = theta0; th[j] = theta0; }
    cluster.sync();
@@ -1119,7 +1204,9 @@
    if (slot.j >= 0) slot.out = own.ptr(slot.j);
    const int nb = max(0, min(B, T - (int)rank * B));
    bool pend_b = false;
-   if (kept_all == 0) {
+   if (!xc_ok) {
+      status = LOCUS_SYNC_TIMEOUT;
+   } else if (kept_all == 0) {
       status = LOCUS_NO_ROWS;
    } else {
       for (int it = 0; it < p.max_iter; ++it) {
@@ -1183,17 +1270,30 @@
             SBQ_TICK(4)
             double zf = 0.0;
             for (unsigned r = 0; r < CS; ++r) zf += flags[r];
+            auto cluster_row_sum = [&](int j) {
+               double a[16];
+#pragma unroll
+               for (int r = 0; r < 16; ++r) a[r] = r < (int)CS ? stage[(size_t)r * Tp + j] : 0.0;
+#pragma unroll
+               for (int o = 8; o > 0; o >>= 1)
+#pragma unroll
+                  for (int r = 0; r < o; ++r) a[r] += a[r + o];
+               return a[0];
+            };
+            if (KC > 1) {
+               double* xr = xc_row(xc, item, it + 1, cidx);
+               if (rank == 0) {
+                  for (int j = tid; j < T; j += NT) __stcg(xr + j, cluster_row_sum(j));
+                  if (tid == 0) __stcg(xr + T, zf);
+               }
+               if (!xc_sync(xc, item, it + 1, cidx, rank, CS, &s_go, cluster)) { status = LOCUS_SYNC_TIMEOUT; break; }
+               zf = xc_sum(xc, item, it + 1, T);
+               SBQ_TICK(8)
+            }
             if (zf != 0.0) { status = LOCUS_ZERO_DENOM; break; }
             double dd = 0.0;
             for (int j = tid; j < T; j += NT) {
-               double a[16];
-#pragma unroll
-               for (int r = 0; r < 16; ++r) a[r] = r < (int)CS ? stage[(size_t)r * Tp + j] : 0.0;
-#pragma unroll
-               for (int o = 8; o > 0; o >>= 1)
-#pragma unroll
-                  for (int r = 0; r < o; ++r) a[r] += a[r + o];
-               const double v = a[0], sj = sdiv[j];
+               const double v = KC > 1 ? xc_sum(xc, item, it + 1, j) : cluster_row_sum(j), sj = sdiv[j];
                nxt[j] = v;
                th[j] = (sj != 0) ? v / sj : 0.0;
                const double diff = v - cur[j];
@@ -1255,17 +1355,17 @@
    if (rank == 0 && (tid == 0 || tid == NT - 32))
       printf("setup: sort %lld jd %lld fill %lld csc %lld rowslots %lld colslots %lld\n", st[0], st[1], st[2], st[3], st[4], st[5]);
    if (rank == 0 && (tid == 0 || tid == NT - 32))
-      printf("locus %d tid %d iters %d resident %d csc_smem %d slots %d/%d lanes %d/%d ncache %d lpr %d lpc %d nrows %d nnz %u setup %lld | E %lld or %lld col %lld csync1 %lld own %lld d2 %lld csync2 %lld chk %lld (cycles/iter)\n", l, tid, iters,
-             (int)resident, (int)csc_in_smem, (int)use_row_slots, (int)use_slots, rslot.lanes, slot.lanes, slot.ncache, lpr, lpc, nrows, nnz_c, t_setup, ph[0] / iters, ph[1] / iters, ph[2] / iters, ph[3] / iters, ph[4] / iters, ph[5] / iters, ph[6] / iters, ph[7] / iters);
+      printf("locus %d cluster %u/%u tid %d iters %d resident %d csc_smem %d slots %d/%d lanes %d/%d ncache %d lpr %d lpc %d nrows %d nnz %u setup %lld | E %lld or %lld col %lld csync1 %lld own %lld d2 %lld csync2 %lld chk %lld xc %lld (cycles/iter)\n", l, cidx, KC, tid, iters,
+             (int)resident, (int)csc_in_smem, (int)use_row_slots, (int)use_slots, rslot.lanes, slot.lanes, slot.ncache, lpr, lpc, nrows, nnz_c, t_setup, ph[0] / iters, ph[1] / iters, ph[2] / iters, ph[3] / iters, ph[4] / iters, ph[5] / iters, ph[6] / iters, ph[7] / iters, ph[8] / iters);
 #endif
    if (pend_b) cluster_wait();
    cluster.sync();
 #ifdef SBQ_TRACE
-   if (tid == 0) trace_emit(CS, NT, l, rank, trace_t0, iters);
+   if (tid == 0) trace_emit(NC, NT, l, grank, trace_t0, iters);
 #endif
 
-   if (rank != 0) return;
-   const bool uniform = status == LOCUS_ZERO_DENOM || status == LOCUS_NO_ROWS;
+   if (grank != 0) return;
+   const bool uniform = status == LOCUS_ZERO_DENOM || status == LOCUS_NO_ROWS || status == LOCUS_SYNC_TIMEOUT;
    double fsum = 0.0;
    for (int j = tid; j < T; j += NT) {
       const double tj = uniform ? theta0 : cur[j];
```

Result: slower. 44.22 billion (median of 6 runs) (-13.6%).
